# IBM/VillanDiffusion

Hardware: AMD Instinct MI355X
Metric: train imgs/sec + 1000-step DDPM sample imgs/sec, CIFAR10 bs128 (higher is better)
Workload: dtype bf16x3/f32

## Files before the change

### include/villan_hip.h

```cpp
#ifndef VILLAN_HIP_H
#define VILLAN_HIP_H

#include <stdint.h>

#ifdef __cplusplus
extern "C" {
#endif

#define VD_ABI_VERSION 12
#define VD_EINVAL (-22)
#define VD_ETIMEDOUT (-110)

int vd_abi_version(void);
const char* vd_last_error(void);
int vd_device_ok(void);
int vd_async_errors(int clear);

enum vd_a_mode { VD_A_ROW = 0,
                 VD_A_COL = 1 };
enum vd_b_mode { VD_B_PLAIN = 0,
                 VD_B_KCONTIG = 1,
                 VD_B_CONV3 = 2,
                 VD_B_CONV3_T = 3,
                 VD_B_CONV3_S2 = 4,
// ... 5 lines not shown
    const float* A;
    const float* B;
    float* D;
    const float* bias;
    const float* rowadd;
    const float* residual;
    int32_t M, N, K;
    int32_t a_mode, b_mode;
    int32_t NP;
    int32_t C, H, W;
    int32_t OH, OW;
    int32_t bias_on_n;
    int32_t d_trans;
    int32_t accumulate;
    int32_t tile;
    int32_t debug;
    float alpha;
    int64_t lda, a_bstride;
    int64_t ldb, b_bstride;
    int64_t ldd, d_bstride;
    int64_t res_bstride, rowadd_bstride;
    float* ws;
    int32_t pad;
    int32_t nb2;
    int64_t a_b2stride, b_b2stride, d_b2stride;
    const float* gn_ss;
    const void* a_packed;
    int32_t a_packed_mpad;
    int32_t math;
    int32_t pool2;
    int32_t kh, kw;
    int32_t conv_stride;
    int32_t pad_h, pad_w;
    int32_t act;
    float* gn_part;
    float* act_out;
    int64_t act_bstride;
    int32_t b_presplit;
    int32_t reserved_;
} vd_gemm_desc;

int vd_gemm(const vd_gemm_desc* desc, void* stream);
int64_t vd_gemm_ws_floats(const vd_gemm_desc* desc);
int vd_gemm_tile(const vd_gemm_desc* desc);
int vd_gemm_kernel_name(const vd_gemm_desc* desc, char* name, int name_len);

typedef struct vd_wgrad_desc {
    const float* dY;
    const float* X;
    float* dW;
    float* ws;
    int32_t M, C, T;
    int32_t nb, NP;
    int32_t H, W, OH, OW;
    int32_t mode, splits, accumulate, tile;
    int64_t dy_bstride, x_bstride;
    int32_t pad;
    int32_t math;
    int32_t presplit;
    int32_t reserved_;
} vd_wgrad_desc;

int vd_conv_wgrad(const vd_wgrad_desc* desc, void* stream);
int64_t vd_conv_wgrad_ws_floats(const vd_wgrad_desc* desc);
int vd_conv_wgrad_plan(const vd_wgrad_desc* desc, int* tile, int* splits);
int vd_conv_wgrad_kernel_name(const vd_wgrad_desc* desc, char* name, int name_len);

int vd_presplit_pack(const float* x, void* y, int B, int C, int HW, int64_t x_bstride, int64_t y_bstride, void* stream);
int vd_presplit_unpack(const void* y, float* x, int B, int C, int HW, int64_t y_bstride, int64_t x_bstride, void* stream);
int vd_groupnorm_fwd_presplit_ok(int C, int HW, int G);
int vd_groupnorm_fwd_presplit(const float* x, const float* gamma, const float* beta, void* y, float* mean, float* rstd, int B, int C, int HW, int G,
                              float eps, int apply_silu, int64_t x_bstride, int64_t y_bstride, void* stream);
int vd_groupnorm_bwd_presplit(const float* dy, const float* x, const float* mean, const float* rstd, const float* gamma, const float* beta,
                              const float* extra, const float* extra2, float* dx, void* dx_ps, float* dgamma_ws, float* dbeta_ws, float* rowsum,
                              int B, int C, int HW, int G, int apply_silu, int64_t dy_bstride, int64_t x_bstride, int64_t extra_bstride,
                              int64_t extra2_bstride, int64_t dx_bstride, int64_t ps_bstride, int64_t rowsum_ld, void* stream);

int vd_conv_wgrad_group_class(const vd_wgrad_desc* desc);
int64_t vd_conv_wgrad_group_job_bytes(void);
int vd_conv_wgrad_group_variant(int cls);
int vd_conv_wgrad_group_plan(const vd_wgrad_desc* descs, int n, void* table_out, int64_t* ws_floats, int* blocks, int* rblocks);
int vd_conv_wgrad_group_rebase(void* dev_table, int n, float* ws, void* stream);
int vd_conv_wgrad_group_launch(const void* dev_table, int n, int cls, int blocks, int rblocks, void* stream);
int vd_conv_wgrad_group_kernel_name(int cls, char* name, int name_len);

int64_t vd_conv3_packed_bytes(int M, int C, int taps);
int vd_conv3_pack_weights(const float* W, void* packed, int M, int C, int taps, int64_t row_stride, int64_t chan_stride, void* stream);
int vd_conv3_pack_weights_multi(const int64_t* table, int n_jobs, int64_t total_blocks, void* stream);
int vd_conv3_pack_weights_f16_multi(const int64_t* table, int n_jobs, int64_t total_blocks, void* stream);

int vd_weight_transpose(const float* W, float* Wt, int M, int C, int T, void* stream);
int vd_sumpool2x2(const float* dU, float* dX, int B, int C, int H, int W, int64_t du_bstride, int64_t dx_bstride,
                  int accumulate, void* stream);
int vd_col2im_s2(const float* G, float* dX, int B, int C, int H, int W, int OH, int OW, int pad, int64_t g_bstride,
                 int64_t dx_bstride, void* stream);
int vd_rowsum(const float* X, float* ws, int B, int M, int P, int64_t x_bstride, int64_t ws_ld, void* stream);
int vd_colsum(const float* ws, float* out, int B, int C, int64_t ld, int accumulate, void* stream);
int vd_colsum_segmented(const int64_t* table, int n_jobs, int B, void* stream);

int64_t vd_groupnorm_ws_floats(int B, int C, int HW, int G);
int vd_groupnorm_fwd(const float* x, const float* gamma, const float* beta, float* y, float* mean, float* rstd,
                     int B, int C, int HW, int G, float eps, int apply_silu, int64_t x_bstride, int64_t y_bstride,
                     float* ws, void* stream);
int vd_groupnorm_stats(const float* x, const float* gamma, const float* beta, float* ss, float* mean, float* rstd,
                       int B, int C, int HW, int G, float eps, int64_t x_bstride, void* stream);
int vd_groupnorm_stats_from_partials(const float* part, int tiles, const float* gamma, const float* beta, float* ss, float* mean,
                                     float* rstd, int B, int C, int HW, int G, float eps, void* stream);
int vd_groupnorm_bwd(const float* dy, const float* x, const float* mean, const float* rstd, const float* gamma,
                     const float* beta, const float* extra, float* dx, float* dgamma_ws, float* dbeta_ws,
                     int B, int C, int HW, int G, int apply_silu, int64_t dy_bstride, int64_t x_bstride,
                     int64_t extra_bstride, int64_t dx_bstride, float* ws, void* stream);
int vd_groupnorm_bwd_fused(const float* dy, const float* x, const float* mean, const float* rstd, const float* gamma,
                           const float* beta, const float* extra, const float* extra2, float* dx, float* dgamma_ws,
                           float* dbeta_ws, float* rowsum, int B, int C, int HW, int G, int apply_silu,
                           int64_t dy_bstride, int64_t x_bstride, int64_t extra_bstride, int64_t extra2_bstride,
                           int64_t dx_bstride, int64_t rowsum_ld, float* ws, void* stream);
int vd_groupnorm_plan(int which, int B, int C, int HW, int G, int aligned, int has_ws, void* stream, char* name, int name_len);

int vd_softmax_col_fwd(float* S, int nb, int N, void* stream);
int vd_softmax_col_bwd(const float* P, float* dP, int nb, int N, float scale, void* stream);
int vd_attn_small_fwd(const float* qkv, float* out, float* P, int B, int C, int N, float scale,
                      int64_t qkv_bstride, int64_t out_bstride, void* stream);
int vd_attn_small_bwd(const float* qkv, const float* P, const float* dout, float* dqkv, int B, int C, int N,
                      float scale, int64_t qkv_bstride, int64_t dout_bstride, int64_t dqkv_bstride, void* stream);

int vd_attn_core_fwd(const float* qkv, float* out, float* P, int B, int heads, int head_dim, int N, float scale, void* stream);
int vd_attn_core_bwd(const float* qkv, const float* P, const float* out, const float* dout, float* dS, float* dqkv, int B, int heads,
                     int head_dim, int N, float scale, void* stream);

int vd_attn_flash_fwd(const float* qkv, float* out, float* lse, int B, int heads, int head_dim, int N, float scale, int64_t qkv_bstride,
                      int64_t out_bstride, void* stream);
int vd_attn_flash_bwd(const float* qkv, const float* out, const float* dout, const float* lse, float* delta, float* dqkv, int B, int heads,
                      int head_dim, int N, float scale, int64_t qkv_bstride, int64_t out_bstride, int64_t dout_bstride,
                      int64_t dqkv_bstride, void* stream);

int vd_timestep_embedding(const float* t, const float* freqs, float* emb, int B, int half, int flip_sin_to_cos,
                          void* stream);
int vd_silu_fwd(const float* x, float* y, int64_t n, void* stream);
int vd_silu_bwd(const float* dy, const float* x, float* dx, int64_t n, int accumulate, void* stream);
int vd_add_strided(float* dst, const float* src, int B, int64_t inner, int64_t dst_bstride, int64_t src_bstride,
                   int accumulate, void* stream);
int vd_scale(float* x, int64_t n, float alpha, void* stream);
int vd_lincomb(float* out, const float* const* srcs, const float* coefs, int n_src, int64_t n, void* stream);

int vd_qsample_backdoor(const float* x0, const float* R, const float* eps, const int64_t* t,
                        const float* tab_a, const float* tab_s, const float* tab_step, const float* tab_coef,
                        float* x_t, float* y, int B, int64_t chw, void* stream);
int vd_mse_fwd_bwd(const float* pred, const float* y, const float* pscale, float* dpred, float* loss,
                   float* partial, int B, int64_t chw, float gscale, void* stream);
#define VD_LOSS_L2 0
#define VD_LOSS_L1 1
#define VD_LOSS_HUBER 2
int vd_loss_fwd_bwd(const float* pred, const float* y, const float* pscale, float* dpred, float* loss,
                    float* partial, int B, int64_t chw, float gscale, int kind, void* stream);
int vd_loss_sample_fwd_bwd(const float* pred, const float* y, const float* pscale, const float* weight, const float* wtab, const int64_t* t,
                           int T, const uint8_t* flags, float poison_weight, float* dpred, float* loss, float* sample_loss, float* stats,
                           float* ws, int B, int64_t chw, float gscale, int kind, void* stream);
int64_t vd_loss_sample_ws_floats(int B, int64_t chw);
int vd_loss_sample_plan(int B, int64_t chw, int* segments, int* blocks);
int vd_trigger_inv_objective(const float* e, const float* tau, float lambda, float* loss, float* dout, float* dtau, float* partial,
                             int B, int64_t chw, int64_t e_bstride, void* stream);
int vd_removal_loss(const float* pred, const float* ref, float w_clean, float w_shift, float gscale, float* dpred, float* terms,
                    float* partial, int B, int64_t chw, int64_t pred_bstride, void* stream);
int vd_image_set_stats(const float* x, int N, int C, int H, int W, int64_t x_bstride, float mul, float add, float lo, float hi,
                       float* mean_img, float* stats, float* partial, void* stream);
int vd_score_inv_objective(const float* s, const float* tau, float sigma, float lambda, float* loss, float* dout, float* dtau,
                           float* partial, int B, int64_t chw, int64_t s_bstride, void* stream);
int vd_image_set_merge(float* mean_a, float* stats_a, int64_t n_a, const float* mean_b, const float* stats_b, int64_t n_b, int64_t chw,
                       float* partial, void* stream);
int vd_neuron_scale(const float* w0, float* w, const int64_t* table, int n_jobs, int64_t total_blocks, const float* mask, const float* delta,
                    const float* xi, void* stream);
int vd_neuron_grad(const float* g, const float* w0, const int64_t* table, int n_jobs, int64_t total_blocks, float* gmask, float* gxi, float scale,
                   int accumulate, void* stream);
int vd_neuron_step(float* x, const float* g, float* buf, int64_t n, float lr, float momentum, float lo, float hi, int use_sign, void* stream);
int vd_lora_merge(const float* w0, float* w, const int64_t* table, int n_jobs, int64_t total_blocks, const float* ab, int r, float s, void* stream);
int vd_lora_grad(const float* g, const int64_t* table, int n_jobs, int64_t total_blocks, const float* ab, float* gab, int r, float s,
                 int accumulate, void* stream);
int64_t vd_lora_act_grad_ws_floats(const int64_t* host_table, int n_rows, int r);
int vd_lora_act_grad(const int64_t* host_table, const int64_t* table, int n_rows, const float* ab, float* gab, int r, float s, int accumulate,
                     float* ws, int64_t ws_floats, void* stream);

int vd_l2norm_sq(const float* g, int64_t n, float* partial, float* out_sq, void* stream);
int vd_adam_step(float* p, const float* g, float* m, float* v, int64_t n, const float* norm_sq, float max_norm,
                 float inv_scale, float lr, float beta1, float beta2, float eps, int step, unsigned* skipped, void* stream);
int vd_adam_ema_step(float* p, const float* g, float* m, float* v, float* ema, int64_t n, const float* norm_sq, float max_norm,
                     float inv_scale, float lr, float beta1, float beta2, float eps, int step, float one_minus_decay, unsigned* skipped,
                     void* stream);
int vd_swap(float* a, float* b, int64_t n, void* stream);

int vd_sched_step(const float* x, const float* eps, const float* z, float* out, float* x0_out, int64_t n,
                  float c_eps, float c_div, float clip, float c_x0, float c_x, float c_e, float c_z,
                  uint64_t seed, uint64_t offset, void* stream);
int vd_batch_l2norm(const float* x, float* out, int B, int64_t inner, void* stream);
int vd_postprocess(const float* x, float* out, int B, int C, int HW, float mul, float add, float lo, float hi,
                   int to_nhwc, void* stream);
int vd_ssim(const float* a, const float* b, const float* win, float* out, int N, int C, int H, int W, int K, float c1, float c2,
            void* stream);
int vd_vq_nearest(const float* z, const float* codebook, float* zq, int64_t* idx, int B, int D, int HW, int n_e,
                  int64_t z_bstride, int64_t q_bstride, void* stream);
int vd_fir_resample2(const float* x, float* out, int64_t planes, int H, int W, int up, float scale, int accumulate, void* stream);
int vd_pyramid_dgrad(const float* g, const float* w, const float* coarse, float* out, int B, int K, int C, int H, int W,
                     int64_t g_bstride, int accumulate, void* stream);
int vd_fourier_embedding(const float* t, const float* W, float* emb, int B, int half, void* stream);
int vd_rowscale(const float* x, const float* s, float* out, int B, int64_t inner, int divide, void* stream);
int vd_randn(float* out, int64_t n, uint64_t seed, uint64_t offset, void* stream);

int vd_poison_batch(const uint8_t* img, const int64_t* idx, const uint8_t* flags, const float* trigger, const float* target,
                    float* pixel_values, float* tgt_out, float* image_out, int B, int C, int H, int W, float vmin,
                    float vmax, int R_trigger_only, void* stream);

int vd_pool3(const float* x, float* y, int B, int C, int H, int W, int stride, int pad, int mode, int64_t x_bstride, int64_t y_bstride,
             void* stream);
int vd_resize_bilinear(const float* x, float* y, int64_t planes, int H, int W, int OH, int OW, float mul, float add, void* stream);

int vd_channel_affine(const float* x, const float* mul, const float* add, float* y, int B, int C, int HW, void* stream);
int vd_lpips_layer(const float* f0, const float* f1, const float* w, float* out, int N, int C, int HW, int accumulate, void* stream);

#ifdef __cplusplus
}
#endif
#endif
```

### villandiffusion_amd/csrc/vd_elem.hip

```cpp
#include "vd_common.h"

namespace {

constexpr int EB = 256;
inline int egrid(int64_t n, int per_thread = 1) {
    int64_t g = (n + (int64_t)EB * per_thread - 1) / ((int64_t)EB * per_thread);
    return (int)(g < 1 ? 1 : (g > 4096 ? 4096 : g));
}
#define GRID_STRIDE(i, n) \
    for (int64_t i = blockIdx.x * (int64_t)blockDim.x + threadIdx.x; i < (n); i += (int64_t)gridDim.x * blockDim.x)

__device__ __forceinline__ float mul_rn(float a, float b) { return __fmul_rn(a, b); }
__device__ __forceinline__ float add_rn(float a, float b) { return __fadd_rn(a, b); }
__device__ __forceinline__ float sub_rn(float a, float b) { return __fsub_rn(a, b); }

__global__ void temb_kernel(const float* __restrict__ t, const float* __restrict__ freqs, float* __restrict__ emb, int B,
                            int half, int flip) {
    GRID_STRIDE(i, (int64_t)B * half) {
        const int b = (int)(i / half), k = (int)(i - (int64_t)b * half);
        const float a = mul_rn(t[b], freqs[k]);
        const float sn = sinf(a), cs = cosf(a);
        float* e = emb + (int64_t)b * 2 * half;
        e[flip ? half + k : k] = sn;
        e[flip ? k : half + k] = cs;
// ... 249 lines not shown
        const uint32_t n2 = (uint32_t)(p0 >> 32) ^ c3 ^ k1, n3 = (uint32_t)p0;
        c0 = n0; c1 = n1; c2 = n2; c3 = n3;
        k0 += 0x9E3779B9u;
        k1 += 0xBB67AE85u;
    }
    out[0] = c0; out[1] = c1; out[2] = c2; out[3] = c3;
}
__device__ __forceinline__ void randn4(uint64_t seed, uint64_t ctr, float (&z)[4]) {
    uint32_t r[4];
    philox4x32_10((uint32_t)ctr, (uint32_t)(ctr >> 32), 0u, 0u, (uint32_t)seed, (uint32_t)(seed >> 32), r);
    const float k = 2.3283064365386963e-10f;
    const float u0 = ((float)r[0] + 0.5f) * k, u1 = ((float)r[1] + 0.5f) * k;
    const float u2 = ((float)r[2] + 0.5f) * k, u3 = ((float)r[3] + 0.5f) * k;
    const float ra = sqrtf(-2.f * __logf(fminf(u0, 0.99999994f) + 1e-12f)), rb = sqrtf(-2.f * __logf(fminf(u2, 0.99999994f) + 1e-12f));
    float s, c;
    __sincosf(6.283185307179586f * u1, &s, &c);
    z[0] = ra * c;
    z[1] = ra * s;
    __sincosf(6.283185307179586f * u3, &s, &c);
    z[2] = rb * c;
    z[3] = rb * s;
}

__global__ void randn_kernel(float* __restrict__ out, int64_t n, uint64_t seed, uint64_t offset) {
    GRID_STRIDE(q, (n + 3) >> 2) {
        float z[4];
        randn4(seed, offset + (uint64_t)q, z);
#pragma unroll
        for (int j = 0; j < 4; ++j)
            if (q * 4 + j < n) out[q * 4 + j] = z[j];
    }
}

struct StepCoef {
    float c_eps, c_div, clip, c_x0, c_x, c_e, c_z;
};
__global__ void sched_step_kernel(const float* __restrict__ x, const float* __restrict__ eps, const float* __restrict__ z,
                                  float* __restrict__ out, float* __restrict__ x0_out, int64_t n, StepCoef k, uint64_t seed,
                                  uint64_t offset) {
    GRID_STRIDE(q, (n + 3) >> 2) {
        float zz[4] = {0.f, 0.f, 0.f, 0.f};
        if (k.c_z != 0.f && !z) randn4(seed, offset + (uint64_t)q, zz);
#pragma unroll
        for (int j = 0; j < 4; ++j) {
            const int64_t i = q * 4 + j;
            if (i >= n) break;
            const float xv = x[i], ev = eps[i];
            float x0 = sub_rn(xv, mul_rn(k.c_eps, ev)) / k.c_div;
            if (k.clip > 0.f) x0 = fminf(fmaxf(x0, -k.clip), k.clip);
            float o = add_rn(mul_rn(k.c_x0, x0), mul_rn(k.c_x, xv));
            if (k.c_e != 0.f) o = add_rn(o, mul_rn(k.c_e, ev));
            if (k.c_z != 0.f) o = add_rn(o, mul_rn(k.c_z, z ? z[i] : zz[j]));
            out[i] = o;
            if (x0_out) x0_out[i] = x0;
        }
    }
}

__global__ __launch_bounds__(256) void batch_l2norm_kernel(const float* __restrict__ x, float* __restrict__ out, int64_t inner) {
    __shared__ float red[4];
    const float* __restrict__ xb = x + (int64_t)blockIdx.x * inner;
    float s = 0.f;
    for (int64_t i = threadIdx.x; i < inner; i += 256) s += xb[i] * xb[i];
    s = block_sum_256(s, red);
    if (threadIdx.x == 0) out[blockIdx.x] = sqrtf(s);
}

__global__ void postprocess_kernel(const float* __restrict__ x, float* __restrict__ out, int B, int C, int HW, float mul,
                                   float add, float lo, float hi, int to_nhwc) {
    GRID_STRIDE(i, (int64_t)B * C * HW) {
        const float v = fminf(fmaxf(add_rn(mul_rn(x[i], mul), add), lo), hi);
        if (to_nhwc) {
            const int p = (int)(i % HW);
            const int64_t bc = i / HW;
            const int c = (int)(bc % C);
            const int64_t b = bc / C;
            out[(b * HW + p) * C + c] = v;
        } else {
            out[i] = v;
        }
    }
}

__global__ void poison_kernel(const uint8_t* __restrict__ img, const int64_t* __restrict__ idx, const uint8_t* __restrict__ flags,
                              const float* __restrict__ trigger, const float* __restrict__ target, float* __restrict__ pv,
                              float* __restrict__ tg, float* __restrict__ image_out, int B, int C, int H, int W, float vmin,
                              float vmax, float denom, int r_trigger_only) {
    const int64_t chw = (int64_t)C * H * W;
    GRID_STRIDE(i, (int64_t)B * chw) {
        const int b = (int)(i / chw);
        const int64_t r = i - (int64_t)b * chw;
        const int xw = (int)(r % W);
        const int64_t cy = r / W;
        const int yh = (int)(cy % H), c = (int)(cy / H);
        const uint8_t f = flags[b];
        const int xs = (f & 2) ? (W - 1 - xw) : xw;
        const int64_t sb = idx ? idx[b] : (int64_t)b;
        const float u = (float)img[((sb * H + yh) * W + xs) * C + c] / 255.0f;
        const float xv = add_rn(mul_rn(sub_rn(u, 0.0f) / denom, sub_rn(vmax, vmin)), vmin);
        if (image_out) image_out[i] = xv;
        if (f & 1) {
            const float tr = trigger[r];
            pv[i] = r_trigger_only ? tr : ((tr > vmin) ? tr : xv);
            tg[i] = target[r];
        } else {
            pv[i] = 0.f;
            tg[i] = xv;
        }
    }
}

}

#define ST ((hipStream_t)stream)

extern "C" int vd_timestep_embedding(const float* t, const float* freqs, float* emb, int B, int half, int flip_sin_to_cos,
                                     void* stream) {
    VD_REQUIRE(t && freqs && emb && B > 0 && half > 0, "vd_timestep_embedding: bad args");
    hipLaunchKernelGGL(temb_kernel, dim3(egrid((int64_t)B * half)), dim3(EB), 0, ST, t, freqs, emb, B, half, flip_sin_to_cos);
    VD_LAUNCH_CHECK("vd_timestep_embedding");
    return 0;
}

extern "C" int vd_silu_fwd(const float* x, float* y, int64_t n, void* stream) {
    VD_REQUIRE(x && y && n > 0, "vd_silu_fwd: bad args");
    hipLaunchKernelGGL(silu_fwd_kernel, dim3(egrid(n)), dim3(EB), 0, ST, x, y, n);
    VD_LAUNCH_CHECK("vd_silu_fwd");
    return 0;
}

extern "C" int vd_silu_bwd(const float* dy, const float* x, float* dx, int64_t n, int accumulate, void* stream) {
    VD_REQUIRE(dy && x && dx && n > 0, "vd_silu_bwd: bad args");
    hipLaunchKernelGGL(silu_bwd_kernel, dim3(egrid(n)), dim3(EB), 0, ST, dy, x, dx, n, accumulate);
    VD_LAUNCH_CHECK("vd_silu_bwd");
    return 0;
}

extern "C" int vd_add_strided(float* dst, const float* src, int B, int64_t inner, int64_t dst_bstride, int64_t src_bstride,
                              int accumulate, void* stream) {
    VD_REQUIRE(dst && src && B > 0 && inner > 0, "vd_add_strided: bad args");
    const bool vec = ((inner & 3) == 0) && ((dst_bstride & 3) == 0) && ((src_bstride & 3) == 0) &&
                     ((((uintptr_t)dst) & 15) == 0) && ((((uintptr_t)src) & 15) == 0);
    if (vec)
        hipLaunchKernelGGL(add_strided_kernel, dim3(egrid((int64_t)B * inner / 4)), dim3(EB), 0, ST, dst, src, B, inner / 4,
                           dst_bstride, src_bstride, accumulate);
    else
        hipLaunchKernelGGL(add_strided_scalar_kernel, dim3(egrid((int64_t)B * inner)), dim3(EB), 0, ST, dst, src, B, inner,
                           dst_bstride, src_bstride, accumulate);
    VD_LAUNCH_CHECK("vd_add_strided");
    return 0;
}

extern "C" int vd_scale(float* x, int64_t n, float alpha, void* stream) {
    VD_REQUIRE(x && n > 0, "vd_scale: bad args");
    hipLaunchKernelGGL(scale_kernel, dim3(egrid(n, 4)), dim3(EB), 0, ST, x, n, alpha);
    VD_LAUNCH_CHECK("vd_scale");
    return 0;
}

extern "C" int vd_lincomb(float* out, const float* const* srcs, const float* coefs, int n_src, int64_t n, void* stream) {
    VD_REQUIRE(out && srcs && coefs && n_src >= 1 && n_src <= 6 && n > 0, "vd_lincomb: bad args (n_src=%d)", n_src);
    LinArgs a;
    for (int i = 0; i < 6; ++i) {
        a.src[i] = i < n_src ? srcs[i] : nullptr;
        a.coef[i] = i < n_src ? coefs[i] : 0.f;
    }
    a.n_src = n_src;
    for (int i = 0; i < n_src; ++i) VD_REQUIRE(a.src[i] != nullptr, "vd_lincomb: null source %d", i);
    hipLaunchKernelGGL(lincomb_kernel, dim3(egrid(n)), dim3(EB), 0, ST, out, a, n);
    VD_LAUNCH_CHECK("vd_lincomb");
    return 0;
}

extern "C" int vd_qsample_backdoor(const float* x0, const float* R, const float* eps, const int64_t* t, const float* tab_a,
                                   const float* tab_s, const float* tab_step, const float* tab_coef, float* x_t, float* y, int B,
                                   int64_t chw, void* stream) {
    VD_REQUIRE(x0 && R && eps && t && tab_s && tab_step && tab_coef && x_t && y, "vd_qsample_backdoor: null pointer");
    VD_REQUIRE(B > 0 && chw > 0, "vd_qsample_backdoor: bad dims");
    hipLaunchKernelGGL(qsample_kernel, dim3(egrid((int64_t)B * chw)), dim3(EB), 0, ST, x0, R, eps, t, tab_a, tab_s, tab_step,
                       tab_coef, x_t, y, B, chw);
    VD_LAUNCH_CHECK("vd_qsample_backdoor");
    return 0;
}

extern "C" int vd_loss_fwd_bwd(const float* pred, const float* y, const float* pscale, float* dpred, float* loss, float* partial,
                               int B, int64_t chw, float gscale, int kind, void* stream) {
    VD_REQUIRE(pred && y && loss && partial && B > 0 && chw > 0, "vd_loss_fwd_bwd: bad args");
    VD_REQUIRE(kind >= VD_LOSS_L2 && kind <= VD_LOSS_HUBER, "vd_loss_fwd_bwd: kind %d (0 = l2, 1 = l1, 2 = huber)", kind);
    const int64_t n = (int64_t)B * chw;
    int grid = egrid(n);
    if (grid > 1024) grid = 1024;
// ... 395 lines not shown
    if (q2 >= items) return;
    const int b2 = (int)(q2 / ipi), pb = (int)(q2 - (int64_t)b2 * ipi) * 4;
    float r[4];
#pragma unroll
    for (int e = 0; e < 4; ++e) r[e] = red[0][li2][c * 4 + e];
    for (int t = 1; t < PD_KS; ++t)
#pragma unroll
        for (int e = 0; e < 4; ++e) r[e] += red[t][li2][c * 4 + e];
    float* __restrict__ op = out + ((int64_t)b2 * C + c) * HW + pb;
    const int CH = H >> 1, CW = W >> 1;
    const float* __restrict__ xp = coarse ? coarse + ((int64_t)b2 * C + c) * CH * CW : nullptr;
#pragma unroll
    for (int e = 0; e < 4; ++e) {
        const int p = pb + e;
        if (p >= HW) break;
        float val = r[e];
        if (xp) {
            const int oy = p / W, ox = p - oy * W;
            const int ay = oy >> 1, ax = ox >> 1;
            const int y0 = (oy & 1) ? ay : ay - 1, y1 = (oy & 1) ? ay + 1 : ay;
            const float wy0 = (oy & 1) ? 0.75f : 0.25f, wy1 = (oy & 1) ? 0.25f : 0.75f;
            const int x0 = (ox & 1) ? ax : ax - 1, x1 = (ox & 1) ? ax + 1 : ax;
            const float wx0 = (ox & 1) ? 0.75f : 0.25f, wx1 = (ox & 1) ? 0.25f : 0.75f;
            auto at = [&](int yy, int xx) -> float {
                return ((unsigned)yy < (unsigned)CH && (unsigned)xx < (unsigned)CW) ? xp[yy * CW + xx] : 0.f;
            };
            const float u = wy0 * (wx0 * at(y0, x0) + wx1 * at(y0, x1)) + wy1 * (wx0 * at(y1, x0) + wx1 * at(y1, x1));
            val += 0.25f * u;
        }
        op[e] = accumulate ? op[e] + val : val;
    }
}

extern "C" int vd_pyramid_dgrad(const float* g, const float* w, const float* coarse, float* out, int B, int K, int C, int H, int W,
                                int64_t g_bstride, int accumulate, void* stream) {
    VD_REQUIRE(g && w && out && B > 0 && K > 0 && H > 0 && W > 0, "vd_pyramid_dgrad: bad args");
    VD_REQUIRE(C >= 1 && C <= 4, "vd_pyramid_dgrad: %d image channels not in [1, 4]", C);
    VD_REQUIRE(g_bstride >= (int64_t)K * H * W, "vd_pyramid_dgrad: batch stride %lld < K*H*W %lld", (long long)g_bstride, (long long)K * H * W);
    VD_REQUIRE(!coarse || (H % 2 == 0 && W % 2 == 0), "vd_pyramid_dgrad: a coarser level needs even dims");
    const int HW = H * W;
    const int64_t items = (int64_t)B * ((HW + 3) >> 2);
    const int64_t grid = (items + PD_IPB - 1) / PD_IPB;
    VD_REQUIRE(grid <= 0x7fffffff, "vd_pyramid_dgrad: too many pixels");
    const int vec = (HW % 4 == 0) && (g_bstride % 4 == 0) && ((((uintptr_t)g) & 15) == 0);
#define PD_LAUNCH(CC) \
    hipLaunchKernelGGL(pyramid_dgrad_kernel<CC>, dim3((unsigned)grid), dim3(256), 0, ST, g, w, coarse, out, B, K, H, W, g_bstride, accumulate, vec)
    switch (C) {
        case 1: PD_LAUNCH(1); break;
        case 2: PD_LAUNCH(2); break;
        case 3: PD_LAUNCH(3); break;
        default: PD_LAUNCH(4); break;
    }
#undef PD_LAUNCH
    VD_LAUNCH_CHECK("vd_pyramid_dgrad");
    return 0;
}

extern "C" int vd_fourier_embedding(const float* t, const float* W, float* emb, int B, int half, void* stream) {
    VD_REQUIRE(t && W && emb && B > 0 && half > 0, "vd_fourier_embedding: bad args");
    hipLaunchKernelGGL(fourier_embedding_kernel, dim3((B * half + 255) / 256), dim3(256), 0, ST, t, W, emb, B, half);
    VD_LAUNCH_CHECK("vd_fourier_embedding");
    return 0;
}

extern "C" int vd_rowscale(const float* x, const float* s, float* out, int B, int64_t inner, int divide, void* stream) {
    VD_REQUIRE(x && s && out && B > 0 && inner > 0, "vd_rowscale: bad args");
    hipLaunchKernelGGL(rowscale_kernel, dim3(egrid((int64_t)B * inner)), dim3(EB), 0, ST, x, s, out, B, inner, divide);
    VD_LAUNCH_CHECK("vd_rowscale");
    return 0;
}

extern "C" int vd_poison_batch(const uint8_t* img, const int64_t* idx, const uint8_t* flags, const float* trigger, const float* target,
                               float* pixel_values, float* tgt_out, float* image_out, int B, int C, int H, int W, float vmin,
                               float vmax, int R_trigger_only, void* stream) {
    VD_REQUIRE(img && flags && trigger && target && pixel_values && tgt_out, "vd_poison_batch: null pointer");
    VD_REQUIRE(B > 0 && C > 0 && H > 0 && W > 0, "vd_poison_batch: bad dims");
    const float denom = (float)(1.0 - 0.0 + 1e-5);
    hipLaunchKernelGGL(poison_kernel, dim3(egrid((int64_t)B * C * H * W)), dim3(EB), 0, ST, img, idx, flags, trigger, target,
                       pixel_values, tgt_out, image_out, B, C, H, W, vmin, vmax, denom, R_trigger_only);
    VD_LAUNCH_CHECK("vd_poison_batch");
    return 0;
}

namespace {

template <int MODE>
__global__ __launch_bounds__(EB) void pool3_kernel(const float* __restrict__ x, float* __restrict__ y, int B, int C, int H, int W, int OH, int OW,
                                                   int stride, int pad, int64_t x_bstride, int64_t y_bstride) {
    const int64_t total = (int64_t)B * C * OH * OW;
    for (int64_t e = (int64_t)blockIdx.x * EB + threadIdx.x; e < total; e += (int64_t)gridDim.x * EB) {
        const int ox = (int)(e % OW);
        int64_t r = e / OW;
        const int oy = (int)(r % OH);
        r /= OH;
        const int c = (int)(r % C), b = (int)(r / C);
        const float* __restrict__ src = x + b * x_bstride + (int64_t)c * H * W;
        float acc = MODE == 0 ? -INFINITY : 0.f;
        int cnt = 0;
#pragma unroll
        for (int dy = 0; dy < 3; ++dy)
#pragma unroll
            for (int dx = 0; dx < 3; ++dx) {
                const int iy = oy * stride + dy - pad, ix = ox * stride + dx - pad;
                const bool ok = (unsigned)iy < (unsigned)H && (unsigned)ix < (unsigned)W;
                const float v = src[ok ? iy * W + ix : 0];
                if (ok) {
                    acc = MODE == 0 ? fmaxf(acc, v) : acc + v;
                    ++cnt;
                }
            }
        y[b * y_bstride + (int64_t)c * OH * OW + (int64_t)oy * OW + ox] = MODE == 0 ? acc : acc / (float)cnt;
    }
}

__global__ __launch_bounds__(EB) void resize_bilinear_kernel(const float* __restrict__ x, float* __restrict__ y, int64_t planes, int H, int W, int OH,
                                                             int OW, float sh, float sw, float mul, float add) {
    const int64_t total = planes * OH * OW;
    for (int64_t e = (int64_t)blockIdx.x * EB + threadIdx.x; e < total; e += (int64_t)gridDim.x * EB) {
        const int ox = (int)(e % OW);
        const int64_t r = e / OW;
        const int oy = (int)(r % OH);
        const int64_t pl = r / OH;
        float fy = sh * ((float)oy + 0.5f) - 0.5f, fx = sw * ((float)ox + 0.5f) - 0.5f;
        fy = fy < 0.f ? 0.f : fy;
        fx = fx < 0.f ? 0.f : fx;
        const int y0 = (int)fy, x0 = (int)fx;
        const int y1 = y0 + (y0 < H - 1 ? 1 : 0), x1 = x0 + (x0 < W - 1 ? 1 : 0);
        const float ly = fy - (float)y0, lx = fx - (float)x0;
        const float* __restrict__ s = x + pl * H * W;
        const float v = (1.f - ly) * ((1.f - lx) * s[y0 * W + x0] + lx * s[y0 * W + x1]) + ly * ((1.f - lx) * s[y1 * W + x0] + lx * s[y1 * W + x1]);
        y[e] = mul * v + add;
    }
}

}

extern "C" int vd_pool3(const float* x, float* y, int B, int C, int H, int W, int stride, int pad, int mode, int64_t x_bstride, int64_t y_bstride,
                        void* stream) {
    VD_REQUIRE(x && y && B > 0 && C > 0 && H >= 3 - 2 * pad && W >= 3 - 2 * pad && (stride == 1 || stride == 2) && (pad == 0 || pad == 1) && (mode == 0 || mode == 1),
               "vd_pool3: bad args (3x3 window, stride 1 | 2, pad 0 | 1, mode 0 max | 1 avg without the padding)");
    const int OH = (H + 2 * pad - 3) / stride + 1, OW = (W + 2 * pad - 3) / stride + 1;
    const int64_t n = (int64_t)B * C * OH * OW;
    if (mode == 0)
        hipLaunchKernelGGL(pool3_kernel<0>, dim3(egrid(n)), dim3(EB), 0, ST, x, y, B, C, H, W, OH, OW, stride, pad, x_bstride, y_bstride);
    else
        hipLaunchKernelGGL(pool3_kernel<1>, dim3(egrid(n)), dim3(EB), 0, ST, x, y, B, C, H, W, OH, OW, stride, pad, x_bstride, y_bstride);
    VD_LAUNCH_CHECK("vd_pool3");
    return 0;
}

extern "C" int vd_resize_bilinear(const float* x, float* y, int64_t planes, int H, int W, int OH, int OW, float mul, float add, void* stream) {
    VD_REQUIRE(x && y && planes > 0 && H > 0 && W > 0 && OH > 0 && OW > 0, "vd_resize_bilinear: bad args");
    hipLaunchKernelGGL(resize_bilinear_kernel, dim3(egrid(planes * OH * OW)), dim3(EB), 0, ST, x, y, planes, H, W, OH, OW, (float)H / (float)OH,
                       (float)W / (float)OW, mul, add);
    VD_LAUNCH_CHECK("vd_resize_bilinear");
    return 0;
}

namespace {

__global__ __launch_bounds__(EB) void channel_affine_kernel(const float* __restrict__ x, const float* __restrict__ mul, const float* __restrict__ add,
                                                            float* __restrict__ y, int64_t total, int C, int HW) {
    for (int64_t e = (int64_t)blockIdx.x * EB + threadIdx.x; e < total; e += (int64_t)gridDim.x * EB) {
        const int c = (int)((e / HW) % C);
        y[e] = x[e] * mul[c] + add[c];
    }
// ... 50 lines not shown
```

### villandiffusion_amd/csrc/vd_gemm.hip

```cpp
#include "vd_common.h"
#include <string.h>
#include <stdlib.h>

bool vd_conv3_k32p_eligible(const vd_gemm_desc& d);
int vd_launch_conv3_k32p(const vd_gemm_desc& d, int mode, hipStream_t st, char* name);
int vd_launch_wgrad_ps_group(const void* jobs, int n, int W, int up, int blocks, hipStream_t st, bool one, char* name);
bool vd_conv3_sm_eligible(const vd_gemm_desc& d);
int vd_launch_conv3_sm(const vd_gemm_desc& d, hipStream_t st, char* name);
bool vd_gemm1x1_k32p_pick(const vd_gemm_desc& d);
int vd_launch_gemm1x1_k32p(const vd_gemm_desc& d, hipStream_t st, char* name);

namespace {

constexpr int NT = 256;
constexpr int BK = 32;
constexpr int KG = BK / 4;

struct Pix {
    int b, oy, ox, p;
    bool valid;
};

__device__ __forceinline__ void kdecomp9(int k, int& c, int& r, int& s) {
    c = k / 9;
// ... 1614 lines not shown

static void wgrad_patch_plan(const vd_wgrad_desc& d, int& splits, int& ks_per) {
    const int kpix = wgrad_patch_kind(d) == 3 ? 64 : 32;
    const int ks_total = (int)(((int64_t)d.nb * d.NP + kpix - 1) / kpix);
    const int base = vd_cdiv(d.M, 128) * vd_cdiv(d.C, 64) * 3;
    splits = d.splits;
    if (splits <= 0) {
        constexpr int target = 768;
        splits = vd_cdiv(target, base);
        const int max_splits = ks_total / 8 > 0 ? ks_total / 8 : 1;
        if (splits > max_splits) splits = max_splits;
        if (splits < 1) splits = 1;
    }
    ks_per = vd_cdiv(ks_total, splits);
    splits = vd_cdiv(ks_total, ks_per);
}

__global__ __launch_bounds__(256) void slab_reduce_kernel(const float* __restrict__ ws, float* __restrict__ out,
                                                          int64_t n4, int splits, int accumulate) {
    const f32x4* __restrict__ w4 = reinterpret_cast<const f32x4*>(ws);
    f32x4* __restrict__ o4 = reinterpret_cast<f32x4*>(out);
    for (int64_t i = blockIdx.x * (int64_t)blockDim.x + threadIdx.x; i < n4; i += (int64_t)gridDim.x * blockDim.x) {
        f32x4 s = w4[i];
        for (int z = 1; z < splits; ++z) s += w4[(int64_t)z * n4 + i];
        if (accumulate) s += o4[i];
        o4[i] = s;
    }
}
__global__ __launch_bounds__(256) void slab_reduce_perm_kernel(const float* __restrict__ ws, float* __restrict__ out, int M,
                                                               int C, int splits, int accumulate) {
    const int64_t n = (int64_t)M * C * 9;
    for (int64_t i = blockIdx.x * (int64_t)blockDim.x + threadIdx.x; i < n; i += (int64_t)gridDim.x * blockDim.x) {
        float s = ws[i];
        for (int z = 1; z < splits; ++z) s += ws[(int64_t)z * n + i];
        const int sx = (int)(i % 3);
        const int64_t t = i / 3;
        const int c = (int)(t % C);
        const int64_t t2 = t / C;
        const int m = (int)(t2 % M), r = (int)(t2 / M);
        const int64_t o = ((int64_t)m * C + c) * 9 + r * 3 + sx;
        out[o] = accumulate ? (out[o] + s) : s;
    }
}

__global__ __launch_bounds__(256) void slab_reduce_scalar_kernel(const float* __restrict__ ws, float* __restrict__ out,
                                                                 int64_t n, int splits, int accumulate) {
    for (int64_t i = blockIdx.x * (int64_t)blockDim.x + threadIdx.x; i < n; i += (int64_t)gridDim.x * blockDim.x) {
        float s = ws[i];
        for (int z = 1; z < splits; ++z) s += ws[(int64_t)z * n + i];
        if (accumulate) s += out[i];
        out[i] = s;
    }
}

__global__ __launch_bounds__(256) void wtranspose_kernel(const float* __restrict__ W, float* __restrict__ Wt, int M, int C,
                                                         int T) {
    const int64_t total = (int64_t)M * C * T;
    for (int64_t i = blockIdx.x * (int64_t)blockDim.x + threadIdx.x; i < total; i += (int64_t)gridDim.x * blockDim.x) {
        const int t = (int)(i % T);
        const int64_t cm = i / T;
        const int m = (int)(cm % M), c = (int)(cm / M);
        Wt[i] = W[((int64_t)m * C + c) * T + t];
    }
}

__global__ __launch_bounds__(256) void sumpool2x2_kernel(const float* __restrict__ dU, float* __restrict__ dX, int B, int C,
                                                         int H, int W, int64_t du_bs, int64_t dx_bs, int accumulate) {
    const int64_t per = (int64_t)C * H * W, total = per * B;
    for (int64_t i = blockIdx.x * (int64_t)blockDim.x + threadIdx.x; i < total; i += (int64_t)gridDim.x * blockDim.x) {
        const int b = (int)(i / per);
        const int64_t r = i - (int64_t)b * per;
        const int x = (int)(r % W);
        const int64_t cy = r / W;
        const int y = (int)(cy % H);
        const int64_t c = cy / H;
        const float* u = dU + (int64_t)b * du_bs + (c * 2 * H + 2 * y) * (2 * W) + 2 * x;
        float s = (u[0] + u[1]) + (u[2 * W] + u[2 * W + 1]);
        float* o = dX + (int64_t)b * dx_bs + r;
        *o = accumulate ? (*o + s) : s;
    }
}

__global__ __launch_bounds__(256) void col2im_s2_kernel(const float* __restrict__ G, float* __restrict__ dX, int B, int C,
                                                        int H, int W, int OH, int OW, int pad, int64_t g_bs, int64_t dx_bs) {
    const int64_t per = (int64_t)C * H * W, total = per * B;
    for (int64_t i = blockIdx.x * (int64_t)blockDim.x + threadIdx.x; i < total; i += (int64_t)gridDim.x * blockDim.x) {
        const int b = (int)(i / per);
        const int64_t q = i - (int64_t)b * per;
        const int x = (int)(q % W);
        const int64_t cy = q / W;
        const int y = (int)(cy % H);
        const int c = (int)(cy / H);
        const float* g = G + (int64_t)b * g_bs + (int64_t)c * 9 * OH * OW;
        const int yp = y + pad, xp = x + pad;
        float acc = 0.f;
        for (int r = yp & 1; r < 3; r += 2) {
            const int iy = (yp - r) >> 1;
            if (yp < r || iy >= OH) continue;
            for (int s = xp & 1; s < 3; s += 2) {
                const int ix = (xp - s) >> 1;
                if (xp < s || ix >= OW) continue;
                acc += g[(r * 3 + s) * OH * OW + iy * OW + ix];
            }
        }
        dX[(int64_t)b * dx_bs + q] = acc;
    }
}

__global__ __launch_bounds__(256) void rowsum_long_kernel(const float* __restrict__ X, float* __restrict__ ws, int M, int P, int64_t x_bs, int64_t ws_ld) {
    __shared__ float part[4];
    const int row = blockIdx.x, b = row / M, m = row - b * M;
    const int lane = threadIdx.x & 63, w = threadIdx.x >> 6;
    const int Q = P >> 4;
    const f32x4* __restrict__ x4 = reinterpret_cast<const f32x4*>(X + (int64_t)b * x_bs + (int64_t)m * P) + (int64_t)w * Q;
    float s0 = 0.f, s1 = 0.f, s2 = 0.f, s3 = 0.f;
    int i = lane;
    for (; i + 192 < Q; i += 256) {
        const f32x4 a = x4[i], c = x4[i + 64], e = x4[i + 128], f = x4[i + 192];
        s0 += (a[0] + a[1]) + (a[2] + a[3]);
        s1 += (c[0] + c[1]) + (c[2] + c[3]);
        s2 += (e[0] + e[1]) + (e[2] + e[3]);
        s3 += (f[0] + f[1]) + (f[2] + f[3]);
    }
    for (; i < Q; i += 64) {
        const f32x4 a = x4[i];
        s0 += (a[0] + a[1]) + (a[2] + a[3]);
    }
    const float s = wave_sum((s0 + s1) + (s2 + s3));
    if (lane == 0) part[w] = s;
    __syncthreads();
    if (threadIdx.x == 0) ws[(int64_t)b * ws_ld + m] = (part[0] + part[1]) + (part[2] + part[3]);
}

__global__ __launch_bounds__(256) void rowsum_kernel(const float* __restrict__ X, float* __restrict__ ws, int B, int M, int P,
                                                     int64_t x_bs, int64_t ws_ld) {
    const int row = blockIdx.x * 4 + (threadIdx.x >> 6);
    if (row >= B * M) return;
    const int b = row / M, m = row - b * M;
    const float* __restrict__ x = X + (int64_t)b * x_bs + (int64_t)m * P;
    const int lane = threadIdx.x & 63;
    float s = 0.f;
    if ((P & 3) == 0 && ((((uintptr_t)x) & 15) == 0)) {
        const f32x4* x4 = reinterpret_cast<const f32x4*>(x);
        const int Q = P >> 2;
        int i = lane;
        for (; i + 192 < Q; i += 256) {
            const f32x4 v0 = x4[i], v1 = x4[i + 64], v2 = x4[i + 128], v3 = x4[i + 192];
            s += (v0[0] + v0[1]) + (v0[2] + v0[3]);
            s += (v1[0] + v1[1]) + (v1[2] + v1[3]);
            s += (v2[0] + v2[1]) + (v2[2] + v2[3]);
            s += (v3[0] + v3[1]) + (v3[2] + v3[3]);
        }
        for (; i < Q; i += 64) {
            f32x4 v = x4[i];
            s += (v[0] + v[1]) + (v[2] + v[3]);
        }
    } else {
        for (int i = lane; i < P; i += 64) s += x[i];
    }
    s = wave_sum(s);
    if (lane == 0) ws[(int64_t)b * ws_ld + m] = s;
}

__global__ __launch_bounds__(256) void colsum_kernel(const float* __restrict__ ws, float* __restrict__ out, int B, int C,
                                                     int64_t ld, int accumulate) {
    __shared__ float part[4][64];
    const int lane = threadIdx.x & 63, w = threadIdx.x >> 6;
    const int c = blockIdx.x * 64 + lane;
    float s = 0.f;
    if (c < C) {
        int b = w;
        for (; b + 28 < B; b += 32) {
            float t[8];
#pragma unroll
            for (int u = 0; u < 8; ++u) t[u] = ws[(int64_t)(b + 4 * u) * ld + c];
#pragma unroll
            for (int u = 0; u < 8; ++u) s += t[u];
        }
        for (; b < B; b += 4) s += ws[(int64_t)b * ld + c];
    }
    part[w][lane] = s;
    __syncthreads();
    if (w == 0 && c < C) {
        const float t = (part[0][lane] + part[1][lane]) + (part[2][lane] + part[3][lane]);
        out[c] = accumulate ? (out[c] + t) : t;
    }
}

template <bool BIG_IS_X>
__global__ __launch_bounds__(256) void wgrad_small_kernel(const vd_wgrad_desc d) {
    constexpr int MAXS = 4, PWM = 34;
    __shared__ float S[MAXS * PWM * PWM];
    const int CB = BIG_IS_X ? d.C : d.M, CS = BIG_IS_X ? d.M : d.C;
    const int H = d.OH, W = d.OW, HW = H * W;
    constexpr int PW = PWM, PHW = PWM * PWM;
    const int cb_blocks = (CB + 31) / 32, tiles_x = (W + 31) / 32, tiles = tiles_x * ((H + 31) / 32);
    int rest = blockIdx.x;
    const int cb0 = (rest % cb_blocks) * 32;
    rest /= cb_blocks;
    const int tile = rest % tiles, b = rest / tiles;
    const int y0 = (tile / tiles_x) * 32, x0 = (tile - (tile / tiles_x) * tiles_x) * 32;
    const int TH = min(32, H - y0), TW = min(32, W - x0);
    const float* __restrict__ big = (BIG_IS_X ? d.X + (int64_t)b * d.x_bstride : d.dY + (int64_t)b * d.dy_bstride);
    const float* __restrict__ sml = (BIG_IS_X ? d.dY + (int64_t)b * d.dy_bstride : d.X + (int64_t)b * d.x_bstride);
    for (int i = threadIdx.x; i < CS * PHW; i += 256) {
        const int cs = i / PHW, rem = i - cs * PHW;
        const int yy = y0 + rem / PW - 1, xx = x0 + rem - (rem / PW) * PW - 1;
        const bool ok = (unsigned)yy < (unsigned)H && (unsigned)xx < (unsigned)W;
        S[i] = ok ? sml[(int64_t)cs * HW + yy * W + xx] : 0.f;
    }
    __syncthreads();
    const int x = threadIdx.x & 31, slot = threadIdx.x >> 5;
    const int Ncols = d.C * 9;
    float* __restrict__ part = d.ws + ((int64_t)b * tiles + tile) * d.M * Ncols;
    float acc[4][MAXS][9];
#pragma unroll
    for (int k = 0; k < 4; ++k)
#pragma unroll
        for (int cs = 0; cs < MAXS; ++cs)
#pragma unroll
            for (int t = 0; t < 9; ++t) acc[k][cs][t] = 0.f;
    if (x < TW) {
        const float* __restrict__ src[4];
        bool live[4];
#pragma unroll
        for (int k = 0; k < 4; ++k) {
            const int cb = cb0 + slot + 8 * k;
            live[k] = cb < CB;
            src[k] = big + (int64_t)(live[k] ? cb : 0) * HW + (int64_t)y0 * W + x0 + x;
        }
        for (int y = 0; y < TH; ++y) {
            float v[4];
#pragma unroll
            for (int k = 0; k < 4; ++k) v[k] = src[k][y * W];
#pragma unroll
            for (int k = 0; k < 4; ++k) v[k] = live[k] ? v[k] : 0.f;
#pragma unroll
            for (int cs = 0; cs < MAXS; ++cs) {
                if (cs < CS) {
                    const float* __restrict__ sp = S + cs * PHW + (y + 1) * PW + (x + 1);
#pragma unroll
                    for (int t = 0; t < 9; ++t) {
                        const int r = t / 3, sx = t - 3 * r;
                        const int dy = BIG_IS_X ? 1 - r : r - 1, dx = BIG_IS_X ? 1 - sx : sx - 1;
// ... 551 lines not shown
        jb.d.ws = reinterpret_cast<float*>((uintptr_t)0);
        if (splits > 1) {
            jb.rblocks = (int)((nel + 255) / 256 < 1024 ? (nel + 255) / 256 : 1024);
            jb.d.ws = reinterpret_cast<float*>((uintptr_t)(off * sizeof(float)));
            off += (int64_t)splits * nel;
            off = (off + 3) / 4 * 4;
        }
        rblk += jb.rblocks;
    }
    *ws_floats = off;
    *blocks = blk;
    *rblocks = rblk;
    return cls;
}

__global__ __launch_bounds__(64) void wgrad_group_rebase_kernel(vd_wgrad_job* __restrict__ jobs, int n, float* ws) {
    const int j = blockIdx.x * 64 + threadIdx.x;
    if (j < n && jobs[j].gy > 1) jobs[j].d.ws = ws + ((uintptr_t)jobs[j].d.ws) / sizeof(float);
}

extern "C" int vd_conv_wgrad_group_rebase(void* dev_table, int n, float* ws, void* stream) {
    VD_REQUIRE(dev_table && n > 0, "vd_conv_wgrad_group_rebase: bad args");
    hipLaunchKernelGGL(wgrad_group_rebase_kernel, dim3(vd_cdiv(n, 64)), dim3(64), 0, (hipStream_t)stream,
                       reinterpret_cast<vd_wgrad_job*>(dev_table), n, ws);
    VD_LAUNCH_CHECK("vd_conv_wgrad_group_rebase");
    return 0;
}

static int wgrad_group_run(const void* dev_table, int n, int cls, int blocks, int rblocks, hipStream_t st, char* name) {
    VD_REQUIRE(name || (dev_table && n > 0 && blocks > 0 && rblocks >= 0), "vd_conv_wgrad_group_launch: bad args");
    const vd_wgrad_job* jobs = reinterpret_cast<const vd_wgrad_job*>(dev_table);
    const dim3 grid(blocks);
    switch (cls) {
        case VD_WG_ONE + 1000: {
            if (!name) {
                static const hipError_t attr1 = hipFuncSetAttribute(reinterpret_cast<const void*>(wgrad1x1_wide_group_kernel<true>),
                                                                    hipFuncAttributeMaxDynamicSharedMemorySize, W1X1_WIDE_LDS);
                VD_REQUIRE(attr1 == hipSuccess, "vd_conv_wgrad_group_launch: cannot reserve %d bytes of LDS", W1X1_WIDE_LDS);
            }
            VD_LAUNCH_OR_NAME(name, wgrad1x1_wide_group_kernel<true>, grid, dim3(512), W1X1_WIDE_LDS, st, jobs, n);
            break;
        }
        case VD_WG_ONE + 4 * 32 + 0: VD_LAUNCH_OR_NAME(name, (wgrad_k32_group_kernel<32, 0, true>), grid, dim3(NT), 0, st, jobs, n); break;
        case VD_WG_ONE + 4 * 32 + 2: VD_LAUNCH_OR_NAME(name, (wgrad_k32_group_kernel<32, 2, true>), grid, dim3(NT), 0, st, jobs, n); break;
        case VD_WG_ONE + 4 * 16 + 0: VD_LAUNCH_OR_NAME(name, (wgrad_k32_group_kernel<16, 0, true>), grid, dim3(NT), 0, st, jobs, n); break;
        case VD_WG_ONE + 4 * 16 + 2: VD_LAUNCH_OR_NAME(name, (wgrad_k32_group_kernel<16, 2, true>), grid, dim3(NT), 0, st, jobs, n); break;
        case VD_WG_ONE + 4 * 8 + 0: VD_LAUNCH_OR_NAME(name, (wgrad_k32_group_kernel<8, 0, true>), grid, dim3(NT), 0, st, jobs, n); break;
        case VD_WG_ONE + 4 * 8 + 2: VD_LAUNCH_OR_NAME(name, (wgrad_k32_group_kernel<8, 2, true>), grid, dim3(NT), 0, st, jobs, n); break;
        case VD_WG_ONE + 3000 + 4 * 32: case VD_WG_ONE + 3000 + 4 * 16: case VD_WG_ONE + 3000 + 4 * 8: case VD_WG_ONE + 3000 + 4 * 32 + 2:
        case VD_WG_ONE + 3000 + 4 * 16 + 2: case VD_WG_ONE + 3000 + 4 * 8 + 2:
            VD_REQUIRE(vd_launch_wgrad_ps_group(dev_table, n, (cls - VD_WG_ONE - 3000) / 4, (cls - VD_WG_ONE - 3000) & 2, blocks, st, true, name) == 0,
                       "vd_conv_wgrad_group_launch: no pre-split kernel for class %d", cls);
            break;
        case 1000: {
            if (!name) {
                static const hipError_t attr = hipFuncSetAttribute(reinterpret_cast<const void*>(wgrad1x1_wide_group_kernel<>),
                                                                   hipFuncAttributeMaxDynamicSharedMemorySize, W1X1_WIDE_LDS);
                VD_REQUIRE(attr == hipSuccess, "vd_conv_wgrad_group_launch: cannot reserve %d bytes of LDS", W1X1_WIDE_LDS);
            }
            VD_LAUNCH_OR_NAME(name, wgrad1x1_wide_group_kernel<>, grid, dim3(512), W1X1_WIDE_LDS, st, jobs, n);
            break;
        }
        case 4 * 32 + 0: VD_LAUNCH_OR_NAME(name, (wgrad_k32_group_kernel<32, 0>), grid, dim3(NT), 0, st, jobs, n); break;
        case 4 * 32 + 2: VD_LAUNCH_OR_NAME(name, (wgrad_k32_group_kernel<32, 2>), grid, dim3(NT), 0, st, jobs, n); break;
        case 4 * 32 + 1: VD_LAUNCH_OR_NAME(name, (wgrad_bx3_group_kernel<32, 0, true>), grid, dim3(NT), 0, st, jobs, n); break;
        case 4 * 32 + 3: VD_LAUNCH_OR_NAME(name, (wgrad_bx3_group_kernel<32, 2, true>), grid, dim3(NT), 0, st, jobs, n); break;
        case 4 * 16 + 0: VD_LAUNCH_OR_NAME(name, (wgrad_k32_group_kernel<16, 0>), grid, dim3(NT), 0, st, jobs, n); break;
        case 4 * 16 + 2: VD_LAUNCH_OR_NAME(name, (wgrad_k32_group_kernel<16, 2>), grid, dim3(NT), 0, st, jobs, n); break;
        case 4 * 8 + 0: VD_LAUNCH_OR_NAME(name, (wgrad_k32_group_kernel<8, 0>), grid, dim3(NT), 0, st, jobs, n); break;
        case 4 * 8 + 2: VD_LAUNCH_OR_NAME(name, (wgrad_k32_group_kernel<8, 2>), grid, dim3(NT), 0, st, jobs, n); break;
        case 4 * 4 + 0: VD_LAUNCH_OR_NAME(name, (wgrad_bx3_group_kernel<4, 0, false>), grid, dim3(NT), 0, st, jobs, n); break;
        case 3000 + 4 * 32: case 3000 + 4 * 16: case 3000 + 4 * 8: case 3000 + 4 * 32 + 2: case 3000 + 4 * 16 + 2: case 3000 + 4 * 8 + 2:
            VD_REQUIRE(vd_launch_wgrad_ps_group(dev_table, n, (cls - 3000) / 4, (cls - 3000) & 2, blocks, st, false, name) == 0,
                       "vd_conv_wgrad_group_launch: no pre-split kernel for class %d", cls);
            break;
        case 2000 + 33: VD_LAUNCH_OR_NAME(name, (wgrad_bx3_group_kernel<32, 4, true>), grid, dim3(NT), 0, st, jobs, n); break;
        case 2000 + 32: VD_LAUNCH_OR_NAME(name, (wgrad_bx3_group_kernel<32, 4, false>), grid, dim3(NT), 0, st, jobs, n); break;
        case 2000 + 16: VD_LAUNCH_OR_NAME(name, (wgrad_bx3_group_kernel<16, 4, false>), grid, dim3(NT), 0, st, jobs, n); break;
        case 2000 + 8: VD_LAUNCH_OR_NAME(name, (wgrad_bx3_group_kernel<8, 4, false>), grid, dim3(NT), 0, st, jobs, n); break;
        default: vd_set_error("vd_conv_wgrad_group_launch: unknown kernel class %d", cls); return VD_EINVAL;
    }
    if (name) return vd_name_append(name, "(+group_reduce)");
    VD_LAUNCH_CHECK("vd_conv_wgrad_group_launch");
    if (rblocks > 0) {
        hipLaunchKernelGGL(wgrad_group_reduce_kernel, dim3(rblocks), dim3(256), 0, st, jobs, n);
        VD_LAUNCH_CHECK("vd_conv_wgrad_group_launch/reduce");
    }
    return 0;
}

extern "C" int vd_conv_wgrad_group_launch(const void* dev_table, int n, int cls, int blocks, int rblocks, void* stream) {
    return wgrad_group_run(dev_table, n, cls, blocks, rblocks, (hipStream_t)stream, nullptr);
}

extern "C" int vd_conv_wgrad_group_kernel_name(int cls, char* name, int name_len) {
    char buf[VD_NAME_LEN] = "";
    return name_out(wgrad_group_run(nullptr, 0, cls, 0, 0, nullptr, buf), buf, name, name_len);
}

extern "C" int64_t vd_conv_wgrad_ws_floats(const vd_wgrad_desc* desc) {
    if (!desc) return 0;
    int tile, splits, kk_per;
    wgrad_plan(*desc, tile, splits, kk_per);
    return splits > 1 ? (int64_t)splits * desc->M * desc->C * desc->T : 0;
}

extern "C" int vd_weight_transpose(const float* W, float* Wt, int M, int C, int T, void* stream) {
    VD_REQUIRE(W && Wt && M > 0 && C > 0 && T > 0, "vd_weight_transpose: bad args");
    const int64_t total = (int64_t)M * C * T;
    const int grid = (int)((total + 255) / 256 < 4096 ? (total + 255) / 256 : 4096);
    hipLaunchKernelGGL(wtranspose_kernel, dim3(grid), dim3(256), 0, (hipStream_t)stream, W, Wt, M, C, T);
    VD_LAUNCH_CHECK("vd_weight_transpose");
    return 0;
}

extern "C" int vd_sumpool2x2(const float* dU, float* dX, int B, int C, int H, int W, int64_t du_bstride, int64_t dx_bstride,
                             int accumulate, void* stream) {
    VD_REQUIRE(dU && dX && B > 0 && C > 0 && H > 0 && W > 0, "vd_sumpool2x2: bad args");
    const int64_t total = (int64_t)B * C * H * W;
    const int grid = (int)((total + 255) / 256 < 8192 ? (total + 255) / 256 : 8192);
    hipLaunchKernelGGL(sumpool2x2_kernel, dim3(grid), dim3(256), 0, (hipStream_t)stream, dU, dX, B, C, H, W, du_bstride,
                       dx_bstride, accumulate);
    VD_LAUNCH_CHECK("vd_sumpool2x2");
    return 0;
}

extern "C" int vd_col2im_s2(const float* G, float* dX, int B, int C, int H, int W, int OH, int OW, int pad, int64_t g_bstride,
                            int64_t dx_bstride, void* stream) {
    VD_REQUIRE(G && dX && B > 0 && C > 0 && H > 0 && W > 0 && OH > 0 && OW > 0 && (pad == 0 || pad == 1), "vd_col2im_s2: bad args");
    const int64_t total = (int64_t)B * C * H * W;
    const int grid = (int)((total + 255) / 256 < 16384 ? (total + 255) / 256 : 16384);
    hipLaunchKernelGGL(col2im_s2_kernel, dim3(grid), dim3(256), 0, (hipStream_t)stream, G, dX, B, C, H, W, OH, OW, pad, g_bstride,
                       dx_bstride);
    VD_LAUNCH_CHECK("vd_col2im_s2");
    return 0;
}

extern "C" int vd_rowsum(const float* X, float* ws, int B, int M, int P, int64_t x_bstride, int64_t ws_ld, void* stream) {
    VD_REQUIRE(X && ws && B > 0 && M > 0 && P > 0 && ws_ld >= M, "vd_rowsum: bad args");
    if (P >= 8192 && (P & 15) == 0 && (x_bstride & 3) == 0 && ((((uintptr_t)X) & 15) == 0))
        hipLaunchKernelGGL(rowsum_long_kernel, dim3(B * M), dim3(256), 0, (hipStream_t)stream, X, ws, M, P, x_bstride, ws_ld);
    else
        hipLaunchKernelGGL(rowsum_kernel, dim3(vd_cdiv((int64_t)B * M, 4)), dim3(256), 0, (hipStream_t)stream, X, ws, B, M, P,
                           x_bstride, ws_ld);
    VD_LAUNCH_CHECK("vd_rowsum");
    return 0;
}

extern "C" int vd_colsum_segmented(const int64_t* table, int n_jobs, int B, void* stream) {
    VD_REQUIRE(table && n_jobs > 0 && B > 0, "vd_colsum_segmented: bad args");
    hipLaunchKernelGGL(colsum_seg_kernel, dim3(n_jobs), dim3(256), 0, (hipStream_t)stream, table, B);
    VD_LAUNCH_CHECK("vd_colsum_segmented");
    return 0;
}

extern "C" int vd_colsum(const float* ws, float* out, int B, int C, int64_t ld, int accumulate, void* stream) {
    VD_REQUIRE(ws && out && B > 0 && C > 0, "vd_colsum: bad args");
    hipLaunchKernelGGL(colsum_kernel, dim3(vd_cdiv(C, 64)), dim3(256), 0, (hipStream_t)stream, ws, out, B, C, ld, accumulate);
    VD_LAUNCH_CHECK("vd_colsum");
    return 0;
}
```

### villandiffusion_amd/csrc/vd_wgrad_bx3.inc

```
typedef __bf16 bf16x2 __attribute__((ext_vector_type(2)));

__device__ __forceinline__ void split_pair(float a, float b, unsigned& hi, unsigned& lo) {
    bf16x2 h, l;
    h[0] = (__bf16)a;
    h[1] = (__bf16)b;
    l[0] = (__bf16)(a - (float)h[0]);
    l[1] = (__bf16)(b - (float)h[1]);
    hi = __builtin_bit_cast(unsigned, h);
    lo = __builtin_bit_cast(unsigned, l);
}

#include "vd_wgrad_job.h"

#ifdef VD_WG_STAMPS
__device__ unsigned long long* g_wg_stamps = nullptr;
#define WG_STAMP(var) const unsigned long long var = __builtin_amdgcn_s_memtime()
#endif

template <int W, int MODE, bool WIDE = false>
__device__ __forceinline__ void wgrad_bx3_body(const vd_wgrad_desc& d, int ksteps_per_split, int gx, int gy, int lin) {
    constexpr int ROWS = 32 / W;
    constexpr int OPR = W >= 8 ? W / 8 : 1;
    constexpr bool W4 = (W == 4);
    constexpr int CT = 64;
// ... 341 lines not shown
                va[j] = aok ? ra[2 * i][j] : 0.f;
                va[4 + j] = aok ? ra[2 * i + 1][j] : 0.f;
                vb[j] = bok ? rb[2 * i][j] : 0.f;
                vb[4 + j] = bok ? rb[2 * i + 1][j] : 0.f;
            }
            u32x4 hi, lo;
            split_bf16x8(va, hi, lo);
            As[so * LD_ + sr + 32 * i] = hi;
            As[(8 + so) * LD_ + sr + 32 * i] = lo;
            split_bf16x8(vb, hi, lo);
            Bs[so * LD_ + sr + 32 * i] = hi;
            Bs[(8 + so) * LD_ + sr + 32 * i] = lo;
        }
    };

    f32x16 acc[2][2];
#pragma unroll
    for (int mi = 0; mi < 2; ++mi)
#pragma unroll
        for (int ni = 0; ni < 2; ++ni)
#pragma unroll
            for (int v = 0; v < 16; ++v) acc[mi][ni][v] = 0.f;

    const int wm = wave >> 1, wc = wave & 1;
    const u32x4* __restrict__ a_base = As + h * LD_ + wm * 64 + l31;
    const u32x4* __restrict__ b_base = Bs + h * LD_ + wc * 64 + l31;

    if (ks_begin < ks_end) {
        load_stage(ks_begin);
        store_stage();
        __syncthreads();
        for (int ks = ks_begin; ks < ks_end; ++ks) {
            const bool more = ks + 1 < ks_end;
            if (more) load_stage(ks + 1);
#pragma unroll
            for (int kk = 0; kk < 4; ++kk) {
                bf16x8 ah[2], al[2];
#pragma unroll
                for (int mi = 0; mi < 2; ++mi) {
                    ah[mi] = __builtin_bit_cast(bf16x8, a_base[(2 * kk) * LD_ + mi * 32]);
                    al[mi] = __builtin_bit_cast(bf16x8, a_base[(8 + 2 * kk) * LD_ + mi * 32]);
                }
#pragma unroll
                for (int ni = 0; ni < 2; ++ni) {
                    const bf16x8 bh = __builtin_bit_cast(bf16x8, b_base[(2 * kk) * LD_ + ni * 32]);
                    const bf16x8 bl = __builtin_bit_cast(bf16x8, b_base[(8 + 2 * kk) * LD_ + ni * 32]);
#pragma unroll
                    for (int mi = 0; mi < 2; ++mi) {
                        acc[mi][ni] = __builtin_amdgcn_mfma_f32_32x32x16_bf16(al[mi], bh, acc[mi][ni], 0, 0, 0);
                        acc[mi][ni] = __builtin_amdgcn_mfma_f32_32x32x16_bf16(ah[mi], bl, acc[mi][ni], 0, 0, 0);
                        acc[mi][ni] = __builtin_amdgcn_mfma_f32_32x32x16_bf16(ah[mi], bh, acc[mi][ni], 0, 0, 0);
                    }
                }
            }
            __syncthreads();
            if (more) store_stage();
            __syncthreads();
        }
    }
    float* __restrict__ out = (gy > 1) ? (d.ws + (int64_t)by * d.M * d.C) : d.dW;
    const bool accum = (gy == 1) && d.accumulate;
#pragma unroll
    for (int ni = 0; ni < 2; ++ni) {
        const int c = c0 + wc * 64 + ni * 32 + l31;
        if (c >= d.C) continue;
#pragma unroll
        for (int mi = 0; mi < 2; ++mi)
#pragma unroll
            for (int v = 0; v < 16; ++v) {
                const int m = m0 + wm * 64 + mi * 32 + (v & 3) + 8 * (v >> 2) + 4 * h;
                if (m >= d.M) continue;
                const int64_t off = (int64_t)m * d.C + c;
                out[off] = accum ? (out[off] + acc[mi][ni][v]) : acc[mi][ni][v];
            }
    }
}

__global__ __launch_bounds__(NT, 2) void wgrad1x1_bx3_kernel(const vd_wgrad_desc d, int ksteps_per_split) {
    wgrad1x1_bx3_body(d, ksteps_per_split, gridDim.x, gridDim.y, blockIdx.x + gridDim.x * blockIdx.y);
}

#include "vd_wgrad1x1_wide.inc"

__global__ __launch_bounds__(256) void wgrad_group_reduce_kernel(const vd_wgrad_job* __restrict__ jobs, int n_jobs) {
    const vd_wgrad_job* __restrict__ jb = jobs + wgrad_find_job(jobs, n_jobs, blockIdx.x, true);
    const int lb = blockIdx.x - jb->first_rblock;
    if (lb >= jb->rblocks || jb->gy <= 1) return;
    const int M = jb->d.M, C = jb->d.C, T = jb->d.T, splits = jb->gy, accumulate = jb->d.accumulate;
    const float* __restrict__ ws = jb->d.ws;
    float* __restrict__ out = jb->d.dW;
    const int64_t n = (int64_t)M * C * T;
    if ((n & 3) == 0 && ((((uintptr_t)ws) & 15) == 0)) {
        const int64_t n4 = n >> 2;
        const f32x4* __restrict__ ws4 = reinterpret_cast<const f32x4*>(ws);
        for (int64_t i4 = lb * 256 + threadIdx.x; i4 < n4; i4 += (int64_t)jb->rblocks * 256) {
            const f32x4* __restrict__ p = ws4 + i4;
            f32x4 s = p[0];
            int z = 1;
            for (; z + 4 <= splits; z += 4) {
                const f32x4 a = p[(int64_t)z * n4], b = p[(int64_t)(z + 1) * n4], c = p[(int64_t)(z + 2) * n4], e = p[(int64_t)(z + 3) * n4];
#pragma unroll
                for (int j = 0; j < 4; ++j) s[j] = (((s[j] + a[j]) + b[j]) + c[j]) + e[j];
            }
            for (; z < splits; ++z) {
                const f32x4 a = p[(int64_t)z * n4];
#pragma unroll
                for (int j = 0; j < 4; ++j) s[j] += a[j];
            }
#pragma unroll
            for (int j = 0; j < 4; ++j) {
                const int64_t i = 4 * i4 + j;
                int64_t o = i;
                if (T == 9) {
                    const int sx = (int)(i % 3);
                    const int64_t t = i / 3;
                    const int c = (int)(t % C);
                    const int64_t t2 = t / C;
                    const int m = (int)(t2 % M), r = (int)(t2 / M);
                    o = ((int64_t)m * C + c) * 9 + r * 3 + sx;
                }
                out[o] = accumulate ? (out[o] + s[j]) : s[j];
            }
        }
        return;
    }
    for (int64_t i = lb * 256 + threadIdx.x; i < n; i += (int64_t)jb->rblocks * 256) {
        float s = ws[i];
        for (int z = 1; z < splits; ++z) s += ws[(int64_t)z * n + i];
        int64_t o = i;
        if (T == 9) {
            const int sx = (int)(i % 3);
            const int64_t t = i / 3;
            const int c = (int)(t % C);
            const int64_t t2 = t / C;
            const int m = (int)(t2 % M), r = (int)(t2 / M);
            o = ((int64_t)m * C + c) * 9 + r * 3 + sx;
        }
        out[o] = accumulate ? (out[o] + s) : s;
    }
}

static bool wgrad1x1_bx3_eligible(const vd_wgrad_desc& d) {
    return d.math == 1 && d.T == 1 && d.mode == VD_B_PLAIN && d.NP % 8 == 0 && d.M >= 64 && d.C >= 64 && d.tile == 0 &&
           (d.x_bstride & 3) == 0 && (d.dy_bstride & 3) == 0 && ((((uintptr_t)d.X) | ((uintptr_t)d.dY)) & 15) == 0;
}

static void wgrad1x1_bx3_plan(const vd_wgrad_desc& d, int& splits, int& ks_per) {
    const int ks_total = (int)(((int64_t)d.nb * (d.NP >> 3) + 7) >> 3);
    const int base = vd_cdiv(d.M, 128) * vd_cdiv(d.C, 128);
    splits = d.splits;
    if (splits <= 0) {
        constexpr int target = 256;
        splits = vd_cdiv(target, base);
        const int max_splits = ks_total / 4 > 0 ? ks_total / 4 : 1;
        if (splits > max_splits) splits = max_splits;
        if (splits < 1) splits = 1;
    }
    ks_per = vd_cdiv(ks_total, splits);
    splits = vd_cdiv(ks_total, ks_per);
}
```

### villandiffusion_amd/dataset.py

```python
from __future__ import annotations

import os
import pickle
from typing import Dict, Iterator, List, Optional, Tuple, Union

import numpy as np
import torch

from . import ops

DEFAULT_VMIN, DEFAULT_VMAX = float(-1.0), float(1.0)
_ASSET_ROOT = os.path.dirname(os.path.dirname(os.path.abspath(__file__)))


def normalize(x, vmin_in=None, vmax_in=None, vmin_out=0, vmax_out=1, eps: float = 1e-5):
    if vmax_out is None and vmin_out is None:
        return x
    lo = x.min() if vmin_in is None else vmin_in
    hi = x.max() if vmax_in is None else vmax_in
    if vmax_out is None:
        vmax_out = hi
    if vmin_out is None:
        vmin_out = lo
    return ((x - lo) / (hi - lo + eps)) * (vmax_out - vmin_out) + vmin_out
# ... 473 lines not shown

    def get_mask(self, trigger: torch.Tensor) -> torch.Tensor:
        return torch.where(trigger > self._vmin, 0, 1)

    def get_poisoned(self, imgs: torch.Tensor) -> torch.Tensor:
        trig = self._trigger.to(imgs.device)
        m = self.get_mask(trig)
        return m * imgs + (1 - m) * trig

    def get_inpainted_by_type(self, imgs: torch.Tensor, inpaint_type: str) -> torch.Tensor:
        half = imgs.shape[-1] // 2
        mask = torch.ones_like(imgs[0])
        if inpaint_type == self.INPAINT_LINE:
            mask[..., 0:2 * half, half - half // 10: half + half // 20] = 0
        elif inpaint_type == self.INPAINT_BOX:
            lo, hi = half - half // 3, half + half // 3
            mask[..., lo:hi, lo:hi] = 0
        else:
            raise NotImplementedError(f"inpaint: {inpaint_type} is not implemented")
        return mask * imgs + (1 - mask) * torch.full_like(imgs, float(imgs.min()))

    def _ensure_device(self):
        if self._dev_images is None:
            self._dev_images = torch.from_numpy(self._images).to(self._dev)
            self._dev_trigger = self._trigger.to(self._dev).contiguous()
            self._dev_target = self._target.to(self._dev).contiguous()
            self._dev_index = torch.from_numpy(np.ascontiguousarray(self._index, dtype=np.int64)).to(self._dev)
            self._dev_flags = torch.from_numpy(np.ascontiguousarray(self._flags, dtype=np.uint8)).to(self._dev)
            self._any_rto = bool((self._flags & 4).any())
            self._flip_gen = torch.Generator(device=self._dev).manual_seed(int(self._seed) + 7919) if self._dev.type == "cuda" else None

    def loader_state(self) -> Dict:
        g = getattr(self, "_flip_gen", None)
        return {"flip_gen": None if g is None else g.get_state().cpu()}

    def load_loader_state(self, st: Optional[Dict]):
        if not st or st.get("flip_gen") is None or self._latent is not None:
            return
        self._ensure_device()
        if self._flip_gen is not None:
            self._flip_gen.set_state(st["flip_gen"].cpu())

    def _h2d(self, t: torch.Tensor) -> torch.Tensor:
        if self._dev.type == "cuda" and os.environ.get("VILLAN_PAGEABLE_H2D", "0") != "1":
            return t.contiguous().pin_memory().to(self._dev, non_blocking=True)
        return t.to(self._dev)

    def make_batch(self, sample_ids: torch.Tensor, flip_bits: Optional[torch.Tensor] = None, full: bool = True) -> Dict[str, torch.Tensor]:
        if self._latent is not None:
            return self._make_latent_batch(sample_ids, full)
        self._ensure_device()
        if sample_ids.device.type == "cuda" and not full and not self._any_rto:
            return self._make_batch_resident(sample_ids, flip_bits)
        pos = sample_ids.cpu().numpy()
        ds_idx = self._h2d(torch.from_numpy(self._index[pos]))
        flags = torch.from_numpy(self._flags[pos].copy())
        B = len(pos)
        if flip_bits is None:
            flip_bits = (torch.rand(B) < 0.5) if self.random_flip else torch.zeros(B, dtype=torch.bool)
        rto = bool((flags & 4).any())
        if rto and not bool(((flags & 1) == 0).logical_or((flags & 4) != 0).all()):
            raise NotImplementedError("mixed R_trigger_only flags inside one batch")
        kflags = self._h2d(((flags & 1) | (flip_bits.to(torch.uint8) << 1)).to(torch.uint8))
        C, S = self._channel, self._image_size
        pv, tg, im = (torch.empty((B, C, S, S), device=self._dev, dtype=torch.float32) for _ in range(3))
        ops.poison_batch(self._dev_images, kflags, self._dev_trigger, self._dev_target, pv, tg, im, self._vmin, self._vmax,
                         R_trigger_only=rto, idx=ds_idx.contiguous())
        batch = {self.PIXEL_VALUES: pv, self.TARGET: tg, self.IMAGE: im}
        if full:
            is_p = self._h2d((flags & 1).bool())
            trig = self._dev_trigger[None].expand(B, C, S, S)
            batch[self.TRIGGER] = trig
            batch[self.PIXEL_VALUES_TRIGGER] = torch.where(is_p[:, None, None, None], trig, torch.zeros((), device=self._dev))
            lab = torch.full((B,), -1.0) if self._labels is None else torch.from_numpy(self._labels[self._index[pos]]).float()
            batch[self.LABEL] = self._h2d(lab)
            batch[self.IS_CLEAN] = ~is_p
        elif self.batch_flags:
            batch[self.IS_CLEAN] = ~self._h2d((flags & 1).bool())
        return batch

    def _make_batch_resident(self, pos: torch.Tensor, flip_bits: Optional[torch.Tensor]) -> Dict[str, torch.Tensor]:
        B = len(pos)
        pos = pos.long()
        ds_idx = self._dev_index.index_select(0, pos)
        fl = self._dev_flags.index_select(0, pos)
        if flip_bits is None:
            flip = (torch.rand(B, device=self._dev, generator=self._flip_gen) < 0.5) if self.random_flip else None
        else:
            flip = flip_bits if flip_bits.device.type == "cuda" else self._h2d(flip_bits)
        kflags = fl & 1
        if flip is not None:
            kflags = kflags | (flip.to(torch.uint8) << 1)
        C, S = self._channel, self._image_size
        pv, tg, im = (torch.empty((B, C, S, S), device=self._dev, dtype=torch.float32) for _ in range(3))
        ops.poison_batch(self._dev_images, kflags.contiguous(), self._dev_trigger, self._dev_target, pv, tg, im, self._vmin, self._vmax,
                         R_trigger_only=False, idx=ds_idx)
        batch = {self.PIXEL_VALUES: pv, self.TARGET: tg, self.IMAGE: im}
        if self.batch_flags:
            batch[self.IS_CLEAN] = (fl & 1) == 0
        return batch

    def get_dataloader(self, batch_size: int = None, shuffle: bool = None, num_workers: int = None, collate_fn=None,
                       rank: int = 0, world: int = 1, epoch: int = 0, full: bool = True):
        bs = batch_size or self._batch_size
        shuffle = self._shuffle if shuffle is None else shuffle
        return _Loader(self, bs, shuffle, rank, world, epoch, full)

    def get_dataset(self):
        return self


class _Loader:
    def __init__(self, dsl: DatasetLoader, bs: int, shuffle: bool, rank: int, world: int, epoch: int, full: bool):
        from .trainer import shard_indices
        self.dsl, self.bs, self.full = dsl, bs, full
        self.ids = shard_indices(len(dsl), epoch, rank, world, seed=dsl._seed, shuffle=shuffle)
        self._ids_dev = self.ids.to(dsl._dev) if (not full and dsl._latent is None and dsl._dev.type == "cuda") else None

    def __len__(self):
        return (len(self.ids) + self.bs - 1) // self.bs

    def __iter__(self) -> Iterator[Dict[str, torch.Tensor]]:
        ids = self.ids if self._ids_dev is None else self._ids_dev
        for s in range(0, len(ids), self.bs):
            yield self.dsl.make_batch(ids[s:s + self.bs], full=self.full)


class LatentDataset(torch.utils.data.Dataset):
    DATA_EXT: str = ".pt"
    TARGET_LATENTS_FILE_NAME: str = "target"
    POISON_LATENTS_FILE_NAME: str = "poison"
    RAW_LATENTS_FILE_NAME: str = "raw"

    def __init__(self, ds_root: str):
        os.makedirs(ds_root, exist_ok=True)
        self._root = ds_root
        self._target = self._poison = self._raw = None
        self._target_name = self._poison_name = self._raw_name = None
        self._poison_rate, self._len, self._vae, self._use_latent = None, None, None, True

    def set_vae(self, vae):
        self._vae = vae
        return self

    @staticmethod
    def add_ext(p: str) -> str:
        return f"{p}.{LatentDataset.DATA_EXT}"

    @staticmethod
    def read_ext(file: str):
        try:
            return torch.load(LatentDataset.add_ext(file))
        except (FileNotFoundError, OSError):
            return None

    @staticmethod
    def save_ext(val, file: str) -> None:
        torch.save(val, LatentDataset.add_ext(file))

    @property
    def targe_latents_path(self) -> str:
        p = os.path.join(self._root, LatentDataset.TARGET_LATENTS_FILE_NAME)
        if not os.path.exists(LatentDataset.add_ext(p)):
            LatentDataset.save_ext({}, p)
        return p

    def _dir(self, data_type: str) -> str:
        p = os.path.join(self._root, data_type)
        os.makedirs(p, exist_ok=True)
        return p

    def _encode(self, x: torch.Tensor) -> torch.Tensor:
        if self._vae is None:
            raise ValueError("Please provide encoder first")
        with torch.no_grad():
            return self._vae.encode(x.to(self._vae.device)).latents.detach().cpu()
# ... 74 lines not shown
```

### villandiffusion_amd/lib.py

```python
from __future__ import annotations

import ctypes as C
import os
import subprocess
from typing import Optional

_HERE = os.path.dirname(os.path.abspath(__file__))
LIB_PATH = os.path.join(_HERE, "libvillan_hip.so")
CSRC = os.path.join(_HERE, "csrc")

A_ROW, A_COL = 0, 1
B_PLAIN, B_KCONTIG, B_CONV3, B_CONV3_T, B_CONV3_S2, B_CONV3_UP, B_CONV3_DIL, B_CONVG = range(8)

_i32, _i64, _f32, _vp = C.c_int32, C.c_int64, C.c_float, C.c_void_p


class GemmDesc(C.Structure):
    _fields_ = [("A", _vp), ("B", _vp), ("D", _vp), ("bias", _vp), ("rowadd", _vp), ("residual", _vp),
                ("M", _i32), ("N", _i32), ("K", _i32), ("a_mode", _i32), ("b_mode", _i32), ("NP", _i32),
                ("C", _i32), ("H", _i32), ("W", _i32), ("OH", _i32), ("OW", _i32),
                ("bias_on_n", _i32), ("d_trans", _i32), ("accumulate", _i32), ("tile", _i32), ("debug", _i32), ("alpha", _f32),
                ("lda", _i64), ("a_bstride", _i64), ("ldb", _i64), ("b_bstride", _i64),
                ("ldd", _i64), ("d_bstride", _i64), ("res_bstride", _i64), ("rowadd_bstride", _i64), ("ws", _vp), ("pad", _i32), ("nb2", _i32),
                ("a_b2stride", _i64), ("b_b2stride", _i64), ("d_b2stride", _i64), ("gn_ss", _vp), ("a_packed", _vp), ("a_packed_mpad", _i32), ("math", _i32), ("pool2", _i32),
                ("kh", _i32), ("kw", _i32), ("conv_stride", _i32), ("pad_h", _i32), ("pad_w", _i32), ("act", _i32),
                ("gn_part", _vp), ("act_out", _vp), ("act_bstride", _i64), ("b_presplit", _i32), ("reserved_", _i32)]


class WgradDesc(C.Structure):
    _fields_ = [("dY", _vp), ("X", _vp), ("dW", _vp), ("ws", _vp),
                ("M", _i32), ("C", _i32), ("T", _i32), ("nb", _i32), ("NP", _i32),
                ("H", _i32), ("W", _i32), ("OH", _i32), ("OW", _i32),
                ("mode", _i32), ("splits", _i32), ("accumulate", _i32), ("tile", _i32),
                ("dy_bstride", _i64), ("x_bstride", _i64), ("pad", _i32), ("math", _i32), ("presplit", _i32), ("reserved_", _i32)]


PROTOTYPES = {
    "vd_abi_version": (_i32, []),
    "vd_last_error": (C.c_char_p, []),
    "vd_async_errors": (_i32, [_i32]),
    "vd_device_ok": (_i32, []),
    "vd_gemm": (_i32, [C.POINTER(GemmDesc), _vp]),
    "vd_gemm_tile": (_i32, [C.POINTER(GemmDesc)]),
    "vd_gemm_ws_floats": (_i64, [C.POINTER(GemmDesc)]),
    "vd_gemm_kernel_name": (_i32, [C.POINTER(GemmDesc), C.c_char_p, _i32]),
    "vd_conv_wgrad": (_i32, [C.POINTER(WgradDesc), _vp]),
    "vd_conv_wgrad_plan": (_i32, [C.POINTER(WgradDesc), C.POINTER(_i32), C.POINTER(_i32)]),
    "vd_conv_wgrad_ws_floats": (_i64, [C.POINTER(WgradDesc)]),
    "vd_conv_wgrad_kernel_name": (_i32, [C.POINTER(WgradDesc), C.c_char_p, _i32]),
    "vd_presplit_pack": (_i32, [_vp, _vp, _i32, _i32, _i32, _i64, _i64, _vp]),
    "vd_presplit_unpack": (_i32, [_vp, _vp, _i32, _i32, _i32, _i64, _i64, _vp]),
    "vd_groupnorm_fwd_presplit_ok": (_i32, [_i32, _i32, _i32]),
    "vd_groupnorm_fwd_presplit": (_i32, [_vp, _vp, _vp, _vp, _vp, _vp, _i32, _i32, _i32, _i32, _f32, _i32, _i64, _i64, _vp]),
    "vd_groupnorm_bwd_presplit": (_i32, [_vp] * 12 + [_vp, _i32, _i32, _i32, _i32, _i32] + [_i64] * 7 + [_vp]),
    "vd_conv_wgrad_group_class": (_i32, [C.POINTER(WgradDesc)]),
    "vd_conv_wgrad_group_job_bytes": (_i64, []),
    "vd_conv_wgrad_group_variant": (_i32, [_i32]),
    "vd_conv_wgrad_group_kernel_name": (_i32, [_i32, C.c_char_p, _i32]),
    "vd_conv_wgrad_group_plan": (_i32, [C.POINTER(WgradDesc), _i32, _vp, C.POINTER(_i64), C.POINTER(_i32), C.POINTER(_i32)]),
    "vd_conv_wgrad_group_rebase": (_i32, [_vp, _i32, _vp, _vp]),
    "vd_conv_wgrad_group_launch": (_i32, [_vp, _i32, _i32, _i32, _i32, _vp]),
    "vd_conv3_packed_bytes": (_i64, [_i32, _i32, _i32]),
    "vd_conv3_pack_weights": (_i32, [_vp, _vp, _i32, _i32, _i32, _i64, _i64, _vp]),
    "vd_conv3_pack_weights_multi": (_i32, [_vp, _i32, _i64, _vp]),
    "vd_conv3_pack_weights_f16_multi": (_i32, [_vp, _i32, _i64, _vp]),
    "vd_weight_transpose": (_i32, [_vp, _vp, _i32, _i32, _i32, _vp]),
    "vd_sumpool2x2": (_i32, [_vp, _vp, _i32, _i32, _i32, _i32, _i64, _i64, _i32, _vp]),
    "vd_col2im_s2": (_i32, [_vp, _vp, _i32, _i32, _i32, _i32, _i32, _i32, _i32, _i64, _i64, _vp]),
    "vd_rowsum": (_i32, [_vp, _vp, _i32, _i32, _i32, _i64, _i64, _vp]),
    "vd_colsum": (_i32, [_vp, _vp, _i32, _i32, _i64, _i32, _vp]),
    "vd_colsum_segmented": (_i32, [_vp, _i32, _i32, _vp]),
    "vd_groupnorm_ws_floats": (_i64, [_i32, _i32, _i32, _i32]),
    "vd_groupnorm_stats": (_i32, [_vp, _vp, _vp, _vp, _vp, _vp, _i32, _i32, _i32, _i32, _f32, _i64, _vp]),
    "vd_groupnorm_fwd": (_i32, [_vp, _vp, _vp, _vp, _vp, _vp, _i32, _i32, _i32, _i32, _f32, _i32, _i64, _i64, _vp, _vp]),
    "vd_groupnorm_bwd": (_i32, [_vp] * 10 + [_i32] * 5 + [_i64] * 4 + [_vp, _vp]),
    "vd_groupnorm_stats_from_partials": (_i32, [_vp, _i32, _vp, _vp, _vp, _vp, _vp, _i32, _i32, _i32, _i32, _f32, _vp]),
    "vd_groupnorm_bwd_fused": (_i32, [_vp] * 12 + [_i32] * 5 + [_i64] * 6 + [_vp, _vp]),
    "vd_groupnorm_plan": (_i32, [_i32] * 7 + [_vp, C.c_char_p, _i32]),
    "vd_softmax_col_fwd": (_i32, [_vp, _i32, _i32, _vp]),
    "vd_softmax_col_bwd": (_i32, [_vp, _vp, _i32, _i32, _f32, _vp]),
    "vd_attn_small_fwd": (_i32, [_vp, _vp, _vp, _i32, _i32, _i32, _f32, _i64, _i64, _vp]),
    "vd_attn_small_bwd": (_i32, [_vp, _vp, _vp, _vp, _i32, _i32, _i32, _f32, _i64, _i64, _i64, _vp]),
    "vd_attn_core_fwd": (_i32, [_vp, _vp, _vp, _i32, _i32, _i32, _i32, _f32, _vp]),
    "vd_attn_core_bwd": (_i32, [_vp, _vp, _vp, _vp, _vp, _vp, _i32, _i32, _i32, _i32, _f32, _vp]),
    "vd_attn_flash_fwd": (_i32, [_vp, _vp, _vp, _i32, _i32, _i32, _i32, _f32, _i64, _i64, _vp]),
    "vd_attn_flash_bwd": (_i32, [_vp, _vp, _vp, _vp, _vp, _vp, _i32, _i32, _i32, _i32, _f32, _i64, _i64, _i64, _i64, _vp]),
    "vd_timestep_embedding": (_i32, [_vp, _vp, _vp, _i32, _i32, _i32, _vp]),
    "vd_silu_fwd": (_i32, [_vp, _vp, _i64, _vp]),
    "vd_silu_bwd": (_i32, [_vp, _vp, _vp, _i64, _i32, _vp]),
    "vd_add_strided": (_i32, [_vp, _vp, _i32, _i64, _i64, _i64, _i32, _vp]),
    "vd_scale": (_i32, [_vp, _i64, _f32, _vp]),
    "vd_lincomb": (_i32, [_vp, C.POINTER(_vp), C.POINTER(_f32), _i32, _i64, _vp]),
    "vd_qsample_backdoor": (_i32, [_vp] * 10 + [_i32, _i64, _vp]),
    "vd_mse_fwd_bwd": (_i32, [_vp] * 6 + [_i32, _i64, _f32, _vp]),
    "vd_loss_fwd_bwd": (_i32, [_vp] * 6 + [_i32, _i64, _f32, _i32, _vp]),
    "vd_loss_sample_fwd_bwd": (_i32, [_vp] * 6 + [_i32, _vp, _f32] + [_vp] * 5 + [_i32, _i64, _f32, _i32, _vp]),
    "vd_loss_sample_ws_floats": (_i64, [_i32, _i64]),
    "vd_loss_sample_plan": (_i32, [_i32, _i64, C.POINTER(_i32), C.POINTER(_i32)]),
    "vd_trigger_inv_objective": (_i32, [_vp, _vp, _f32, _vp, _vp, _vp, _vp, _i32, _i64, _i64, _vp]),
    "vd_removal_loss": (_i32, [_vp, _vp, _f32, _f32, _f32, _vp, _vp, _vp, _i32, _i64, _i64, _vp]),
    "vd_score_inv_objective": (_i32, [_vp, _vp, _f32, _f32, _vp, _vp, _vp, _vp, _i32, _i64, _i64, _vp]),
    "vd_image_set_stats": (_i32, [_vp, _i32, _i32, _i32, _i32, _i64, _f32, _f32, _f32, _f32, _vp, _vp, _vp, _vp]),
    "vd_image_set_merge": (_i32, [_vp, _vp, _i64, _vp, _vp, _i64, _i64, _vp, _vp]),
    "vd_neuron_scale": (_i32, [_vp, _vp, _vp, _i32, _i64, _vp, _vp, _vp, _vp]),
    "vd_neuron_grad": (_i32, [_vp, _vp, _vp, _i32, _i64, _vp, _vp, _f32, _i32, _vp]),
    "vd_neuron_step": (_i32, [_vp, _vp, _vp, _i64, _f32, _f32, _f32, _f32, _i32, _vp]),
    "vd_lora_merge": (_i32, [_vp, _vp, _vp, _i32, _i64, _vp, _i32, _f32, _vp]),
    "vd_lora_grad": (_i32, [_vp, _vp, _i32, _i64, _vp, _vp, _i32, _f32, _i32, _vp]),
    "vd_lora_act_grad_ws_floats": (_i64, [_vp, _i32, _i32]),
    "vd_lora_act_grad": (_i32, [_vp, _vp, _i32, _vp, _vp, _i32, _f32, _i32, _vp, _i64, _vp]),
    "vd_l2norm_sq": (_i32, [_vp, _i64, _vp, _vp, _vp]),
    "vd_adam_step": (_i32, [_vp, _vp, _vp, _vp, _i64, _vp, _f32, _f32, _f32, _f32, _f32, _f32, _i32, _vp, _vp]),
    "vd_adam_ema_step": (_i32, [_vp, _vp, _vp, _vp, _vp, _i64, _vp, _f32, _f32, _f32, _f32, _f32, _f32, _i32, _f32, _vp, _vp]),
    "vd_swap": (_i32, [_vp, _vp, _i64, _vp]),
    "vd_sched_step": (_i32, [_vp] * 5 + [_i64] + [_f32] * 7 + [C.c_uint64, C.c_uint64, _vp]),
    "vd_batch_l2norm": (_i32, [_vp, _vp, _i32, _i64, _vp]),
    "vd_postprocess": (_i32, [_vp, _vp, _i32, _i32, _i32, _f32, _f32, _f32, _f32, _i32, _vp]),
    "vd_ssim": (_i32, [_vp, _vp, _vp, _vp, _i32, _i32, _i32, _i32, _i32, _f32, _f32, _vp]),
    "vd_randn": (_i32, [_vp, _i64, C.c_uint64, C.c_uint64, _vp]),
    "vd_fir_resample2": (_i32, [_vp, _vp, _i64, _i32, _i32, _i32, _f32, _i32, _vp]),
    "vd_pyramid_dgrad": (_i32, [_vp, _vp, _vp, _vp, _i32, _i32, _i32, _i32, _i32, _i64, _i32, _vp]),
    "vd_fourier_embedding": (_i32, [_vp, _vp, _vp, _i32, _i32, _vp]),
    "vd_rowscale": (_i32, [_vp, _vp, _vp, _i32, _i64, _i32, _vp]),
    "vd_vq_nearest": (_i32, [_vp, _vp, _vp, _vp, _i32, _i32, _i32, _i32, _i64, _i64, _vp]),
    "vd_poison_batch": (_i32, [_vp] * 8 + [_i32] * 4 + [_f32, _f32, _i32, _vp]),
    "vd_pool3": (_i32, [_vp, _vp, _i32, _i32, _i32, _i32, _i32, _i32, _i32, _i64, _i64, _vp]),
    "vd_resize_bilinear": (_i32, [_vp, _vp, _i64, _i32, _i32, _i32, _i32, _f32, _f32, _vp]),
    "vd_channel_affine": (_i32, [_vp, _vp, _vp, _vp, _i32, _i32, _i32, _vp]),
    "vd_lpips_layer": (_i32, [_vp, _vp, _vp, _vp, _i32, _i32, _i32, _i32, _vp]),
}

_lib: Optional[C.CDLL] = None


class VillanHipError(RuntimeError):
    pass


def build(verbose: bool = False) -> str:
    out = subprocess.run(["make", "-C", CSRC, "-j4"], capture_output=True, text=True)
    if verbose or out.returncode != 0:
        print(out.stdout[-4000:], out.stderr[-4000:])
    if out.returncode != 0:
        raise VillanHipError("building libvillan_hip.so failed (see output above)")
    return LIB_PATH


def load() -> C.CDLL:
    global _lib
    if _lib is not None:
        return _lib
    import torch
    if not os.path.exists(LIB_PATH):
        raise VillanHipError(
            f"{LIB_PATH} not found: the HIP extension is required (no CPU fallback exists). "
            f"Build it with `make -C {CSRC}` or `python -c 'import __graft_entry__ as g; g.build()'`.")
    lib = C.CDLL(LIB_PATH)
    for name, (res, args) in PROTOTYPES.items():
        fn = getattr(lib, name)
        fn.restype, fn.argtypes = res, args
    if lib.vd_abi_version() != 12:
        raise VillanHipError("libvillan_hip.so ABI version mismatch")
    _lib = lib
    return lib


def last_error() -> str:
    return load().vd_last_error().decode("utf-8", "replace")


_SYNC_DEBUG = bool(os.environ.get("VD_SYNC_DEBUG"))


def check(rc: int, what: str) -> None:
    if rc != 0:
        raise VillanHipError(f"{what} failed (rc={rc}): {last_error()}")
    if _SYNC_DEBUG:
        import sys
        import torch
        print(f"[vd] {what}", file=sys.stderr, flush=True)
        torch.cuda.synchronize()


_device_checked = False


def require_device() -> None:
    global _device_checked
    if _device_checked:
        return
    lib = load()
    rc = lib.vd_device_ok()
    if rc != 0:
        raise VillanHipError(f"MI355X (gfx950) device required: {last_error()}")
    _device_checked = True
```

### villandiffusion_amd/ops.py

```python
from __future__ import annotations

import ctypes as C
import functools
import math
import os
from typing import Optional, Sequence

import torch

from . import lib as L
from .lib import (A_COL, A_ROW, B_CONV3, B_CONV3_DIL, B_CONVG, B_CONV3_S2, B_CONV3_T, B_CONV3_UP, B_KCONTIG, B_PLAIN,
                  GemmDesc, WgradDesc)


def _lib():
    L.require_device()
    return L.load()


_PROF = None


def _kernel_name(query, what) -> str:
    buf = C.create_string_buffer(128)
# ... 575 lines not shown
    if ent is None or ws is None or ent["ws_ptr"] != ws.data_ptr() or ent["ws_floats"] > ws.numel():
        arr = (WgradDesc * n)(*descs)
        jb = int(lib.vd_conv_wgrad_group_job_bytes())
        host = (C.c_uint8 * (n * jb))()
        wsf, blocks, rblocks = C.c_int64(0), C.c_int32(0), C.c_int32(0)
        cls = lib.vd_conv_wgrad_group_plan(arr, n, host, C.byref(wsf), C.byref(blocks), C.byref(rblocks))
        if cls <= 0:
            raise L.VillanHipError(f"vd_conv_wgrad_group_plan: {lib.vd_last_error().decode()}")
        if ws is None or ws.numel() < wsf.value:
            ws = torch.empty(max(int(wsf.value), 1 << 22), device=device, dtype=torch.float32)
            _WG_WS[device] = ws
        ws_ptr = ws.data_ptr()
        table = upload_table(torch.frombuffer(bytearray(host), dtype=torch.uint8), device,
                             after=lambda t: L.check(lib.vd_conv_wgrad_group_rebase(t.data_ptr(), n, ws_ptr, _s()), "vd_conv_wgrad_group_rebase"))
        if len(_WG_CACHE) > 256:
            _WG_CACHE.clear()
        ent = _WG_CACHE[key] = {"table": table, "cls": cls, "blocks": blocks.value, "rblocks": rblocks.value, "ws_ptr": ws.data_ptr(),
                                "ws_floats": int(wsf.value)}
    if _CAPTURE_TABLES is not None:
        _CAPTURE_TABLES.append(ent["table"])
    flops = sum(2.0 * d.M * d.C * d.T * d.nb * d.NP for d in descs)
    nbytes = sum(4.0 * (d.nb * d.M * d.NP + d.nb * d.C * d.H * d.W + d.M * d.C * d.T) for d in descs)
    name = _kernel_name(lib.vd_conv_wgrad_group_kernel_name, ent["cls"]) if _PROF is not None else None
    _timed(name, flops, "mfma", lambda: L.check(
        lib.vd_conv_wgrad_group_launch(ent["table"].data_ptr(), n, ent["cls"], ent["blocks"], ent["rblocks"], _s()), "vd_conv_wgrad_group_launch"),
        nbytes=nbytes)


def conv_wgrad(dy, x, dw2d, mode, ws: Optional[torch.Tensor], accumulate=False, splits=0, tile=0, pad=0, math_mode=0):
    d = wgrad_desc(dy, x, dw2d, mode, ws, accumulate, splits, tile, pad, math_mode)
    Bn, M, OH, OW = dy.shape
    Cc, T = x.shape[1], d.T
    lib = _lib()
    need = lib.vd_conv_wgrad_ws_floats(C.byref(d))
    if need > 0:
        assert ws is not None and ws.numel() >= need, f"wgrad workspace too small: need {need}"
    if _PROF is None:
        L.check(lib.vd_conv_wgrad(C.byref(d), _s()), "vd_conv_wgrad")
        return dw2d
    e0, e1 = torch.cuda.Event(enable_timing=True), torch.cuda.Event(enable_timing=True)
    e0.record()
    L.check(lib.vd_conv_wgrad(C.byref(d), _s()), "vd_conv_wgrad")
    e1.record()
    name = _kernel_name(lib.vd_conv_wgrad_kernel_name, C.byref(d))
    _PROF.append({"name": name, "flops": 2.0 * M * Cc * T * Bn * OH * OW, "bytes": 4.0 * (dy.numel() + x.numel() + M * Cc * T),
                  "e0": e0, "e1": e1, "kind": "mfma"})
    return dw2d


def _wgrad_s2_split(OW) -> bool:
    sel = os.environ.get("VILLAN_WGRAD_S2", "all")
    return sel == "all" or (sel != "none" and OW >= 32)


@functools.lru_cache(maxsize=None)
def _wgrad_split_kernel(M, Cc, OH, OW, mode) -> bool:
    return _wgrad_tile(wgrad_query_desc(M, Cc, OH, OW, mode)) == (5 if mode == B_PLAIN else 4)


def wgrad_bx3_eligible(M, Cc, OH, OW, mode) -> bool:
    return _wgrad_split_kernel(M, Cc, OH, OW, mode) and (mode != B_CONV3_S2 or _wgrad_s2_split(OW))


def wgrad_ws_floats(M, Cc, T, nb, NP, OH=None, OW=None, mode=None, math_mode=0) -> int:
    if OH is None:
        OH = OW = int(round(math.sqrt(NP)))
    d = wgrad_query_desc(M, Cc, OH, OW, (B_PLAIN if T == 1 else B_CONV3) if mode is None else mode, nb, math_mode, NP=NP)
    return int(L.load().vd_conv_wgrad_ws_floats(C.byref(d)))


def weight_transpose(w2d, wt, M, Cc, T):
    L.check(_lib().vd_weight_transpose(_p(w2d), _p(wt), M, Cc, T, _s()), "vd_weight_transpose")
    return wt


def sumpool2x2(dU, dX, accumulate=False):
    Bn, Cc, H, W, xbs = _img(dX)
    ubs = _img(dU)[4]
    assert dU.shape == (Bn, Cc, 2 * H, 2 * W)
    L.check(_lib().vd_sumpool2x2(_p(dU), _p(dX), Bn, Cc, H, W, ubs, xbs, int(accumulate), _s()), "vd_sumpool2x2")
    return dX


def conv3x3_s2_dgrad(dy, w2d, dx, pad=0, a_packed=None):
    Bn, M, OH, OW, dbs = _img(dy)
    Bx, Cc, H, W, xbs = _img(dx)
    assert Bx == Bn and w2d.shape == (M, Cc * 9) and w2d.is_contiguous()
    OHW = OH * OW
    G = torch.empty((Bn, Cc * 9, OHW), device=dy.device, dtype=torch.float32)
    gemm(w2d, dy, G, M=Cc * 9, N=Bn * OHW, K=M, a_mode=A_COL, b_mode=B_PLAIN, NP=OHW, lda=Cc * 9, ldb=OHW, b_bstride=dbs,
         ldd=OHW, d_bstride=Cc * 9 * OHW, a_packed=a_packed)
    L.check(_lib().vd_col2im_s2(_p(G), _p(dx), Bn, Cc, H, W, OH, OW, pad, Cc * 9 * OHW, xbs, _s()), "vd_col2im_s2")
    return dx


def rowsum(x, ws, ws_ld=None):
    Bn, M, H, W, xbs = _img(x)
    ld = M if ws_ld is None else ws_ld
    L.check(_lib().vd_rowsum(_p(x), _p(ws), Bn, M, H * W, xbs, ld, _s()), "vd_rowsum")
    return ws


def colsum(ws, out, Bn, Cc, ld=None, accumulate=False):
    L.check(_lib().vd_colsum(_p(ws), _p(out), Bn, Cc, Cc if ld is None else ld, int(accumulate), _s()), "vd_colsum")
    return out


def colsum_segmented(table, n_jobs, Bn):
    assert table.dtype == torch.int64 and table.is_contiguous() and table.numel() >= 4 * n_jobs
    L.check(_lib().vd_colsum_segmented(_p(table), n_jobs, Bn, _s()), "vd_colsum_segmented")


def _gn_ws(Bn, Cc, HW, G, device):
    need = _lib().vd_groupnorm_ws_floats(Bn, Cc, HW, G)
    return _gemm_ws(need, device) if need > 0 else None


GN_FWD, GN_BWD, GN_STATS = 0, 1, 2


def groupnorm_plan(which, Bn, Cc, HW, G, aligned=True, has_ws=None, stream=None):
    lib = L.load()
    if has_ws is None:
        has_ws = lib.vd_groupnorm_ws_floats(Bn, Cc, HW, G) > 0
    buf = C.create_string_buffer(128)
    S = lib.vd_groupnorm_plan(which, Bn, Cc, HW, G, int(aligned), int(has_ws), stream, buf, len(buf))
    L.check(min(S, 0), "vd_groupnorm_plan")
    return buf.value.decode(), S


def groupnorm_fwd(x, gamma, beta, y, mean, rstd, G, eps, silu):
    Bn, Cc, H, W, xbs = _img(x)
    ybs = _img(y)[4]
    assert y.shape == x.shape and mean.numel() >= Bn * G and rstd.numel() >= Bn * G
    _timed("groupnorm_fwd (gn_fwd_reg_kernel<*> / gn_chunk_*)", 8.0 * x.numel(), "hbm", lambda: L.check(
        _lib().vd_groupnorm_fwd(_p(x), _p(gamma), _p(beta), _p(y), _p(mean), _p(rstd), Bn, Cc, H * W, G, eps,
                                int(silu), xbs, ybs, _p(_gn_ws(Bn, Cc, H * W, G, x.device)), _s()), "vd_groupnorm_fwd"))
    return y


def groupnorm_stats(x, gamma, beta, ss, mean, rstd, G, eps):
    Bn, Cc, H, W, xbs = _img(x)
    assert ss.shape == (Bn, Cc, 2) and ss.is_contiguous()
    L.check(_lib().vd_groupnorm_stats(_p(x), _p(gamma), _p(beta), _p(ss), _p(mean), _p(rstd), Bn, Cc, H * W, G, eps, xbs, _s()),
            "vd_groupnorm_stats")
    return ss


def groupnorm_stats_from_partials(part, tiles, gamma, beta, ss, mean, rstd, HW, G, eps):
    Bn, Cc = ss.shape[0], ss.shape[1]
    assert ss.is_contiguous() and part.is_contiguous() and part.numel() >= Bn * tiles * Cc * 2
    L.check(_lib().vd_groupnorm_stats_from_partials(_p(part), tiles, _p(gamma), _p(beta), _p(ss), _p(mean), _p(rstd), Bn, Cc, HW, G, eps, _s()),
            "vd_groupnorm_stats_from_partials")
    return ss


def gn_fusable(x, cout) -> bool:
    Bn, Cc, H, W = x.shape
    return W in (16, 32) and H == W and Cc % 8 == 0 and Cc <= 1024 and cout >= 64


def groupnorm_bwd(dy, x, mean, rstd, gamma, beta, dx, dgamma_ws, dbeta_ws, G, silu, extra=None, extra2=None, rowsum=None, rowsum_ld=None):
    Bn, Cc, H, W, xbs = _img(x)
    dbs, dxbs = _img(dy)[4], _img(dx)[4]
    ebs = _img(extra)[4] if extra is not None else 0
    e2bs = _img(extra2)[4] if extra2 is not None else 0
    assert dgamma_ws.numel() >= Bn * Cc and dbeta_ws.numel() >= Bn * Cc
    assert extra2 is None or extra2.shape == x.shape
    rld = 0
    if rowsum is not None:
        rld = Cc if rowsum_ld is None else rowsum_ld
        assert rld >= Cc
    nbytes = (12.0 + (4.0 if extra is not None else 0.0) + (4.0 if extra2 is not None else 0.0)) * x.numel()
    _timed("groupnorm_bwd (gn_bwd_reg_kernel<*> / gn_chunk_*)", nbytes, "hbm", lambda: L.check(
        _lib().vd_groupnorm_bwd_fused(_p(dy), _p(x), _p(mean), _p(rstd), _p(gamma), _p(beta), _p(extra), _p(extra2), _p(dx),
                                      _p(dgamma_ws), _p(dbeta_ws), _p(rowsum), Bn, Cc, H * W, G, int(silu), dbs, xbs, ebs, e2bs, dxbs, rld,
                                      _p(_gn_ws(Bn, Cc, H * W, G, x.device)), _s()), "vd_groupnorm_bwd"))
    return dx


def softmax_col_fwd(S, nb, N):
    L.check(_lib().vd_softmax_col_fwd(_p(S), nb, N, _s()), "vd_softmax_col_fwd")
    return S
# ... 374 lines not shown
                                 c_z, seed, offset, _s()), "vd_sched_step")
    return out


def batch_l2norm(x, out):
    Bn = x.shape[0]
    assert x.is_contiguous() and out.numel() >= Bn
    L.check(_lib().vd_batch_l2norm(_p(x), _p(out), Bn, x.numel() // Bn, _s()), "vd_batch_l2norm")
    return out


def ssim(a, b, win, out, c1, c2):
    Bn, Cc, H, W = a.shape
    assert a.is_contiguous() and b.is_contiguous() and win.is_contiguous() and a.shape == b.shape and win.shape[0] == win.shape[1]
    L.check(_lib().vd_ssim(_p(a), _p(b), _p(win), _p(out), Bn, Cc, H, W, win.shape[0], c1, c2, _s()), "vd_ssim")
    return out


def postprocess(x, out, mul, add, lo, hi, to_nhwc):
    Bn, Cc, H, W = x.shape
    assert x.is_contiguous() and out.is_contiguous()
    L.check(_lib().vd_postprocess(_p(x), _p(out), Bn, Cc, H * W, mul, add, lo, hi, int(to_nhwc), _s()), "vd_postprocess")
    return out


def fir_resample2(x, out, up: bool, scale: float = 1.0, accumulate: bool = False):
    Bn, Cc, H, W = x.shape
    assert x.is_contiguous() and out.is_contiguous()
    assert out.shape == ((Bn, Cc, 2 * H, 2 * W) if up else (Bn, Cc, H // 2, W // 2)), (x.shape, out.shape, up)
    L.check(_lib().vd_fir_resample2(_p(x), _p(out), Bn * Cc, H, W, int(up), scale, int(accumulate), _s()), "vd_fir_resample2")
    return out


def pyramid_dgrad(g, w, out, coarse=None, accumulate: bool = False):
    Bn, K, H, W, gbs = _img(g)
    Cc = w.shape[1]
    assert w.is_contiguous() and tuple(w.shape) == (K, Cc) and w.dtype == torch.float32 and 1 <= Cc <= 4
    assert out.is_contiguous() and tuple(out.shape) == (Bn, Cc, H, W) and out.dtype == torch.float32
    assert coarse is None or (coarse.is_contiguous() and tuple(coarse.shape) == (Bn, Cc, H // 2, W // 2) and coarse.dtype == torch.float32
                              and H % 2 == 0 and W % 2 == 0)
    _timed("pyramid_dgrad (pyramid_dgrad_kernel)", 4.0 * (g.numel() + (2 + int(accumulate)) * out.numel()), "hbm", lambda: L.check(
        _lib().vd_pyramid_dgrad(_p(g), _p(w), _p(coarse), _p(out), Bn, K, Cc, H, W, gbs, int(accumulate), _s()), "vd_pyramid_dgrad"))
    return out


def fourier_embedding(t_f32, W, emb):
    Bn, half = t_f32.numel(), W.numel()
    assert emb.shape == (Bn, 2 * half) and emb.is_contiguous()
    L.check(_lib().vd_fourier_embedding(_p(t_f32), _p(W), _p(emb), Bn, half, _s()), "vd_fourier_embedding")
    return emb


def rowscale(x, s, out, divide=False):
    Bn = x.shape[0]
    assert x.is_contiguous() and out.is_contiguous() and s.numel() == Bn
    L.check(_lib().vd_rowscale(_p(x), _p(s), _p(out), Bn, x.numel() // Bn, int(divide), _s()), "vd_rowscale")
    return out


def vq_nearest(z, codebook, zq, idx=None):
    Bn, D, H, W, zbs = _img(z)
    qbs = _img(zq)[4]
    assert zq.shape == z.shape and codebook.is_contiguous() and codebook.shape[1] == D
    assert idx is None or (idx.dtype == torch.int64 and idx.numel() >= Bn * H * W)
    L.check(_lib().vd_vq_nearest(_p(z), _p(codebook), _p(zq), _p(idx), Bn, D, H * W, codebook.shape[0], zbs, qbs, _s()),
            "vd_vq_nearest")
    return zq


def randn(out, seed, offset):
    L.check(_lib().vd_randn(_p(out), out.numel(), seed, offset, _s()), "vd_randn")
    return out


def poison_batch(img_u8, flags_u8, trigger, target, pixel_values, tgt, image_out, vmin, vmax, R_trigger_only=False, idx=None):
    _, H, W, Cc = img_u8.shape
    Bn = flags_u8.numel()
    assert img_u8.dtype == torch.uint8 and flags_u8.dtype == torch.uint8 and img_u8.is_contiguous()
    assert idx is None or (idx.dtype == torch.int64 and idx.numel() == Bn and idx.is_contiguous())
    assert idx is not None or img_u8.shape[0] == Bn
    L.check(_lib().vd_poison_batch(_p(img_u8), _p(idx), _p(flags_u8), _p(trigger), _p(target), _p(pixel_values), _p(tgt),
                                   _p(image_out), Bn, Cc, H, W, vmin, vmax, int(R_trigger_only), _s()), "vd_poison_batch")
    return pixel_values, tgt
```

### villandiffusion_amd/unet.py

```python
from __future__ import annotations

import math
import os
from types import SimpleNamespace
from typing import Dict, List, Optional, Tuple

import torch

from . import ops
from .flatnet import FlatParamNet
from .lib import B_CONV3, B_CONV3_DIL, B_CONV3_S2, B_CONV3_T, B_CONV3_UP, B_PLAIN, A_COL, A_ROW, B_KCONTIG


CONV_MATH_DEFAULT = os.environ.get("VILLAN_CONV_MATH", "bf16x3")
if CONV_MATH_DEFAULT not in ("bf16x3", "f32", "f16", "bf16"):
    raise ValueError(f"VILLAN_CONV_MATH must be 'bf16x3', 'f32', 'f16' or 'bf16', got {CONV_MATH_DEFAULT!r}")


class _PackedConvWeights:

    def __init__(self, net, f16: bool = False):
        self.net = net
        self.f16 = f16
        self.off = {False: {}, True: {}}
        self.jobs = {False: [], True: []}
        self.total = 0
        cands = []
        for name, shape, _ in net._layout:
            if name.endswith(".weight") and len(shape) == 4 and shape[2] == shape[3] and shape[2] in (1, 3):
                cands.append((name[:-7], (lambda n=name: net.P[n]), shape[0], shape[1], shape[2] * shape[3]))
        for prefix, ch in getattr(net, "_qkv", []):
            if prefix + "::qkv_w" in getattr(net, "Pq", {}):
                cands.append((prefix + "::qkv", (lambda k=prefix + "::qkv_w": net.Pq[k]), 3 * ch, ch, 1))
            if prefix + ".to_out.0.weight" in net.P:
                cands.append((prefix + ".to_out.0", (lambda n=prefix + ".to_out.0.weight": net.P[n]), ch, ch, 1))
        plan = []
        for key, get, cout, cin, T in cands:
            for bwd, (M, Cc, rs, cs) in ((False, (cout, cin, cin * T, T)), (True, (cin, cout, T, cin * T))):
                plan.append((key, get, bwd, M, Cc, T, rs, cs))
            if T == 9 and ".downsamplers." in key:
                plan.append((key + "::s2g", get, True, cin * 9, cout, 1, 1, cin * 9))
        for key, get, bwd, M, Cc, T, rs, cs in plan:
            if Cc % 16 == 0 and M >= 64:
                n = (M + 127) // 128 * 128 * Cc * T // (2 if f16 else 1)
                self.off[bwd][key] = (self.total, n)
                self.jobs[bwd].append((key, get, M, Cc, T, rs, cs))
                self.total += n
        self.buf: Optional[torch.Tensor] = None
        self.tables = {}
        self.key = {False: None, True: None}

    def view(self, prefix, bwd):
        ent = self.off[bwd].get(prefix)
        if ent is None:
            return None
        self.refresh(bwd)
        return self.buf[ent[0]:ent[0] + ent[1]]

    def refresh(self, bwd):
        net = self.net
        if not self.jobs[bwd]:
            return
        key = (net.flat_param._version, ops.WEIGHTS_EPOCH)
        if self.key[bwd] != key:
            if self.buf is None:
                self.buf = torch.empty(self.total, device=net.flat_param.device, dtype=torch.int32)
            if bwd not in self.tables:
                rows, blk = [], 0
                for k, get, M, Cc, T, rs, cs in self.jobs[bwd]:
                    o, n = self.off[bwd][k]
                    rows.append([get().data_ptr(), self.buf.data_ptr() + 4 * o, M, Cc, rs, cs, blk, T])
                    blk += ((M + 127) // 128 * 128 * (Cc // 16) * 2 + 255) // 256
                self.tables[bwd] = (torch.tensor(rows, dtype=torch.int64).to(self.buf.device), len(rows), blk)
            tab, nj, blk = self.tables[bwd]
            (ops.conv3_pack_weights_f16_multi if self.f16 else ops.conv3_pack_weights_multi)(tab, nj, blk)
            self.key[bwd] = key


def _split(net) -> bool:
    return getattr(net, "conv_math", "f32") in ("bf16x3", "f16", "bf16")


def _pairs(net) -> bool:
    return getattr(net, "conv_math", "f32") in ("bf16x3", "bf16")


def _with_mixed(net, pk, key, bwd):
    mode = getattr(net, "conv_math", "f32")
    if pk is None or mode not in ("f16", "bf16"):
        return pk
    if mode == "bf16":
        return (pk, pk, 3)
    p16 = getattr(net, "_packed16", None)
    if p16 is None:
        p16 = net._packed16 = _PackedConvWeights(net, f16=True)
    v16 = p16.view(key, bwd)
    return pk if v16 is None else (pk, v16)


def _bx3_packed(net, prefix, bwd, M, Cc, OH, OW, mode):
    if not _split(net) or not ops.bx3_eligible(M, Cc, OH, OW, mode):
        return None
    pk = getattr(net, "_packed", None)
    if pk is None:
        pk = net._packed = _PackedConvWeights(net)
    return _with_mixed(net, pk.view(prefix, bwd), prefix, bwd)


def _bx3_packed_1x1(net, key, bwd, M, K, NP, nb=None):
    if not _split(net) or not ops.gemm_bx3_eligible(M, K, NP, nb):
        return None
    pk = getattr(net, "_packed", None)
    if pk is None:
        pk = net._packed = _PackedConvWeights(net)
    return _with_mixed(net, pk.view(key, bwd), key, bwd)


def _conv1x1_dgrad(net, prefix, cout, cin, dout):
    B, _, H, W = dout.shape
    HW = H * W
    dx = torch.empty((B, cin, H, W), device=dout.device, dtype=torch.float32)
    ops.gemm(net.P[prefix + ".weight"].view(cout, cin), dout, dx, M=cin, N=B * HW, K=cout, a_mode=A_COL, b_mode=B_PLAIN, NP=HW, lda=cin, ldb=HW,
             b_bstride=ops._img(dout)[4], ldd=HW, d_bstride=cin * HW, a_packed=_bx3_packed_1x1(net, prefix, True, cin, cout, HW, B))
    return dx


def _amath(net, M, K, NP) -> int:
    return int(_split(net) and ops.gemm_bx3_act_eligible(M, K, NP))


def _wgrad1x1_math(net, dy, x) -> int:
    ok = _split(net) and ops.wgrad_bx3_eligible(dy.shape[1], x.shape[1], dy.shape[2], dy.shape[3], B_PLAIN) \
        and x.stride(0) % 4 == 0 and dy.stride(0) % 4 == 0
    return int(ok)


class _Conv:

    def __init__(self, net, prefix, cin, cout, mode=B_CONV3, pad=0):
        self.net, self.prefix, self.cin, self.cout, self.mode, self.pad = net, prefix, cin, cout, mode, pad
        net._decl(prefix + ".weight", (cout, cin, 3, 3), fan_in=cin * 9)
        net._decl(prefix + ".bias", (cout,), fan_in=cin * 9, is_bias=True)

    def w2d(self):
        return self.net.P[self.prefix + ".weight"].view(self.cout, self.cin * 9)

    def fwd(self, x, out, rowadd=None, rowadd_bstride=0, residual=None, gn_ss=None, gn_part=None):
        pk = _bx3_packed(self.net, self.prefix, False, self.cout, self.cin, out.shape[2], out.shape[3], self.mode)
        if gn_ss is not None and (out.shape[3] not in (16, 32) or self.mode != B_CONV3):
            pk = None
        return ops.conv3x3(x, self.w2d(), self.net.P[self.prefix + ".bias"], out, mode=self.mode, rowadd=rowadd,
                           rowadd_bstride=rowadd_bstride, residual=residual, pad=self.pad, gn_ss=gn_ss, a_packed=pk, gn_part=gn_part)

    def us_input(self, h, save):
        net = self.net
        B, _, H, W = h.shape
        if (self.mode != B_CONV3_UP or not net.us_fwd_presplit or not getattr(net, "presplit", False) or not _pairs(net) or H != W
                or not ops.conv_presplit_ok(B, self.cin, self.cout, 2 * H, 2 * W, B_CONV3_UP)
                or (save and not (net.group_wgrad and ops.wgrad_presplit_ok(B, self.cin, self.cout, 2 * H, B_CONV3_UP)))):
            return h
        return ops.presplit_pack(h)

    def bwd(self, dout, x, dx, bias_ws=None, skip_bias=False, dout_ps=None):
        net = self.net
        dout_f32 = dout
        gw = net.G[self.prefix + ".weight"].view(self.cout, self.cin * 9)
        want = net.wants_wgrad(gw)
        if isinstance(x, ops.PreSplit):
            if want:
                dy_ps = dout_ps if dout_ps is not None else net.pack_later(dout)
                net.wgrad(dy_ps, x, gw, self.mode, pad=self.pad, math_mode=1)
            if dout_ps is not None:
                dout = dout_ps
        elif (self.mode == B_CONV3_UP and getattr(net, "presplit", False) and _pairs(net) and net.group_wgrad
              and dout.shape[2] == dout.shape[3] and ops.wgrad_presplit_ok(dout.shape[0], self.cin, self.cout, dout.shape[3], B_CONV3_UP)):
            if want:
                dy_ps = dout_ps if dout_ps is not None else net.pack_later(dout)
                net.wgrad(dy_ps, net.pack_later(x), gw, self.mode, pad=self.pad, math_mode=1)
        else:
            assert dout is not None
            bx3 = _split(net) and ops.wgrad_bx3_eligible(self.cout, self.cin, dout.shape[2], dout.shape[3],
                                                                                           self.mode) and x.stride(0) % 4 == 0
            if want:
                net.wgrad(dout, x, gw, self.mode, pad=self.pad, math_mode=int(bx3))
        if not skip_bias:
            B = dout.shape[0]
            ws = bias_ws if bias_ws is not None else net.scratch_bc(B, self.cout)
            if bias_ws is None:
                assert dout_f32 is not None
                net.rowsum(dout_f32, ws)
            net.colsum_later(ws, net.G[self.prefix + ".bias"], B, self.cout, ld=(ws.stride(0) if ws.dim() == 2 else self.cout))
        if dx is None:
            return None
        if self.mode == B_CONV3_S2:
            pk = _bx3_packed_1x1(net, self.prefix + "::s2g", True, self.cin * 9, self.cout, dout.shape[2] * dout.shape[3], dout.shape[0])
            return ops.conv3x3_s2_dgrad(dout, self.w2d(), dx, pad=self.pad, a_packed=pk)
        pk = _bx3_packed(net, self.prefix, True, self.cin, self.cout, dout.shape[2], dout.shape[3], B_CONV3_T) \
            if self.mode in (B_CONV3, B_CONV3_UP) else None
        wt = net.wt_view(self.prefix, self.cout, self.cin, 9, fresh=pk is None)
        if self.mode == B_CONV3:
            ops.conv3x3(dout, wt, None, dx, mode=B_CONV3_T, a_packed=pk)
        elif self.mode == B_CONV3_UP:
            B, _, OH, OW = dout.shape
            if pk is not None and ops.bx3_pool2_eligible(self.cin, self.cout, OH, OW, B):
                src = dout_ps if (dout_ps is not None and net.us_dgrad_presplit and ops.conv_presplit_ok(B, self.cout, self.cin, OH, OW, B_CONV3_T)) else dout
                ops.conv3x3(src, wt, None, dx, mode=B_CONV3_T, a_packed=pk, pool2=True)
            else:
                dU = torch.empty((B, self.cin, OH, OW), device=dout.device, dtype=torch.float32)
                ops.conv3x3(dout, wt, None, dU, mode=B_CONV3_T, a_packed=pk)
                ops.sumpool2x2(dU, dx)
        else:
            raise NotImplementedError(self.mode)
        return dx


class _Norm:
    def __init__(self, net, prefix, ch, silu, groups=None):
        self.net, self.prefix, self.ch, self.silu = net, prefix, ch, silu
        self.groups = net.groups if groups is None else groups
        net._decl(prefix + ".weight", (ch,), ones=True)
        net._decl(prefix + ".bias", (ch,), zeros=True)

    def fwd(self, x, y):
        net = self.net
        B = x.shape[0]
        mean = torch.empty(B * self.groups, device=x.device, dtype=torch.float32)
        rstd = torch.empty_like(mean)
        ops.groupnorm_fwd(x, net.P[self.prefix + ".weight"], net.P[self.prefix + ".bias"], y, mean, rstd, self.groups,
                          net.eps, self.silu)
        return mean, rstd

    def fwd_ps(self, x):
        net = self.net
        B = x.shape[0]
        mean = torch.empty(B * self.groups, device=x.device, dtype=torch.float32)
        rstd = torch.empty_like(mean)
        y = ops.presplit_empty(x.shape, x.device)
        ops.groupnorm_fwd_presplit(x, net.P[self.prefix + ".weight"], net.P[self.prefix + ".bias"], y, mean, rstd, self.groups, net.eps, self.silu)
        return y, mean, rstd

    def ps_ok(self, HW: int) -> bool:
        return ops.groupnorm_presplit_ok(self.ch, HW, self.groups)

    def stats(self, x):
        net = self.net
        B = x.shape[0]
        ss = torch.empty((B, self.ch, 2), device=x.device, dtype=torch.float32)
        mean = torch.empty(B * self.groups, device=x.device, dtype=torch.float32)
        rstd = torch.empty_like(mean)
        ops.groupnorm_stats(x, net.P[self.prefix + ".weight"], net.P[self.prefix + ".bias"], ss, mean, rstd, self.groups, net.eps)
        return ss

    def stats_from_partials(self, part, tiles, B, HW):
        net = self.net
        ss = torch.empty((B, self.ch, 2), device=part.device, dtype=torch.float32)
        mean = torch.empty(B * self.groups, device=part.device, dtype=torch.float32)
        rstd = torch.empty_like(mean)
        ops.groupnorm_stats_from_partials(part, tiles, net.P[self.prefix + ".weight"], net.P[self.prefix + ".bias"], ss, mean, rstd, HW,
                                          self.groups, net.eps)
        return ss

    def bwd(self, dy, x, mean, rstd, dx, extra=None, extra2=None, rowsum=None, dx_ps=None):
        net = self.net
        B = x.shape[0]
        wg, wb = net.scratch_bc(B, self.ch, 1), net.scratch_bc(B, self.ch, 2)
        if dx_ps is not None:
            ops.groupnorm_bwd_presplit(dy, x, mean, rstd, net.P[self.prefix + ".weight"], net.P[self.prefix + ".bias"], dx, dx_ps, wg, wb,
                                       self.groups, self.silu, extra=extra, extra2=extra2, rowsum=rowsum,
                                       rowsum_ld=(rowsum.stride(0) if rowsum is not None else None))
        else:
            ops.groupnorm_bwd(dy, x, mean, rstd, net.P[self.prefix + ".weight"], net.P[self.prefix + ".bias"], dx, wg, wb,
                              self.groups, self.silu, extra=extra, extra2=extra2, rowsum=rowsum,
                              rowsum_ld=(rowsum.stride(0) if rowsum is not None else None))
        net.colsum_later(wg, net.G[self.prefix + ".weight"], B, self.ch)
        net.colsum_later(wb, net.G[self.prefix + ".bias"], B, self.ch)
        return dx


class _Resnet:
# ... 354 lines not shown
        self._begin_declarations(device)
        self._temb: List[Tuple[str, int]] = []
        temb_dim = boc[0] * 4
        self.time_dim0, self.temb_dim = boc[0], temb_dim
        self._decl("time_embedding.linear_1.weight", (temb_dim, boc[0]), fan_in=boc[0])
        self._decl("time_embedding.linear_1.bias", (temb_dim,), fan_in=boc[0], is_bias=True)
        self._decl("time_embedding.linear_2.weight", (temb_dim, temb_dim), fan_in=temb_dim)
        self._decl("time_embedding.linear_2.bias", (temb_dim,), fan_in=temb_dim, is_bias=True)
        self._conv_in = _Conv(self, "conv_in", in_channels, boc[0])

        self.down: List[dict] = []
        ch = boc[0]
        skip_ch = [ch]
        for i, typ in enumerate(down_block_types):
            cin, ch = ch, boc[i]
            blk = {"res": [], "attn": [], "ds": None}
            for j in range(layers_per_block):
                blk["res"].append(_Resnet(self, f"down_blocks.{i}.resnets.{j}", cin if j == 0 else ch, ch))
                if typ == "AttnDownBlock2D":
                    blk["attn"].append(_Attn(self, f"down_blocks.{i}.attentions.{j}", ch, attention_head_dim))
                skip_ch.append(ch)
            if i != len(boc) - 1:
                blk["ds"] = _Conv(self, f"down_blocks.{i}.downsamplers.0.conv", ch, ch, mode=B_CONV3_S2, pad=downsample_padding)
                skip_ch.append(ch)
            self.down.append(blk)
        self.mid_res = [_Resnet(self, "mid_block.resnets.0", ch, ch), _Resnet(self, "mid_block.resnets.1", ch, ch)]
        self.mid_attn = _Attn(self, "mid_block.attentions.0", ch, attention_head_dim)

        rev = boc[::-1]
        self.up: List[dict] = []
        out_ch = rev[0]
        sk = list(skip_ch)
        for i, typ in enumerate(up_block_types):
            prev, out_ch = out_ch, rev[i]
            in_ch = rev[min(i + 1, len(boc) - 1)]
            blk = {"res": [], "attn": [], "us": None, "h_ch": [], "skip_ch": []}
            for j in range(layers_per_block + 1):
                s_ch = sk.pop()
                assert s_ch == (in_ch if j == layers_per_block else out_ch)
                h_ch = prev if j == 0 else out_ch
                blk["res"].append(_Resnet(self, f"up_blocks.{i}.resnets.{j}", h_ch + s_ch, out_ch))
                blk["h_ch"].append(h_ch)
                blk["skip_ch"].append(s_ch)
                if typ == "AttnUpBlock2D":
                    blk["attn"].append(_Attn(self, f"up_blocks.{i}.attentions.{j}", out_ch, attention_head_dim))
            if i != len(boc) - 1:
                blk["us"] = _Conv(self, f"up_blocks.{i}.upsamplers.0.conv", out_ch, out_ch, mode=B_CONV3_UP)
            self.up.append(blk)
        assert not sk
        self.norm_out = _Norm(self, "conv_norm_out", boc[0], True)
        self._conv_out = _Conv(self, "conv_out", boc[0], out_channels)
        self._materialise()

    def _decl_temb(self, prefix, cout) -> int:
        off = sum(c for _, c in self._temb)
        self._temb.append((prefix, cout))
        return off

    def _materialise(self):
        head = [(prefix + ".weight", (cout, self.temb_dim), dict(fan_in=self.temb_dim)) for prefix, cout in self._temb]
        head += [(prefix + ".bias", (cout,), dict(fan_in=self.temb_dim, is_bias=True)) for prefix, cout in self._temb]
        super()._materialise(head, grads=True)
        layout, offs, total, dev = self._layout, self._offs, self.flat_numel, self._dev
        n_t = sum(c for _, c in self._temb)
        o0 = offs[self._temb[0][0] + ".weight"][0]
        ob = offs[self._temb[0][0] + ".bias"][0]
        self.temb_total = n_t
        self.Wt_all = self.flat_param[o0:o0 + n_t * self.temb_dim].view(n_t, self.temb_dim)
        self.bt_all = self.flat_param[ob:ob + n_t]
        self.gWt_all = self.flat_grad[o0:o0 + n_t * self.temb_dim].view(n_t, self.temb_dim)
        self.gbt_all = self.flat_grad[ob:ob + n_t]
        self._wt_offs, wt_total = {}, 0
        for name, shape, _ in layout:
            if name.endswith(".weight") and len(shape) == 4 and shape[2] == 3 and name != "conv_in.weight":
                self._wt_offs[name[:-7]] = wt_total
                wt_total += int(math.prod(shape))
        self._wt_offs["conv_in"] = wt_total
        wt_total += int(math.prod(offs["conv_in.weight"][2]))
        self._wt_total = wt_total
        self._wt_buf: Optional[torch.Tensor] = None
        self.wgrad_ws: Optional[torch.Tensor] = None
        self._cs_pool: Optional[torch.Tensor] = None
        self._cs_tables: Dict[tuple, torch.Tensor] = {}
        self._cs_cols_hint = 4 * sum(int(math.prod(sh)) for _, sh, _ in layout if len(sh) == 1) + 4096
        self._cs_off, self._cs_jobs, self._cs_B, self._cs_retired = 0, [], 0, []
        self._d_temb: Dict[int, torch.Tensor] = {}
        half = self.time_dim0 // 2
        exponent = -math.log(10000) * torch.arange(0, half, dtype=torch.float32)
        exponent = exponent / (half - self.config.freq_shift)
        self.freqs = torch.exp(exponent).to(dev)
        self._anchor = torch.zeros(1, device=dev, requires_grad=True)
        def _late(k):
            return ".time_emb_proj." in k or ".to_q." in k or ".to_k." in k or ".to_v." in k
        o_in = offs["conv_in.weight"][0]
        o_mid = min(v[0] for k, v in offs.items() if k.startswith("mid_block.") and not _late(k))
        o_up = min(v[0] for k, v in offs.items() if k.startswith("up_blocks.") and not _late(k))
        self.grad_buckets = [(o_up, total), (o_mid, o_up), (o_in, o_mid), (0, o_in)]
        self.bucket_ready_hook = None
        self.fuse_gn_inference = None
        self.fused_attention = os.environ.get("VILLAN_FUSED_ATTENTION", "1") != "0"
        self.sampler_graph = os.environ.get("VILLAN_SAMPLER_GRAPH", "1") != "0"
        self.group_wgrad = os.environ.get("VILLAN_GROUP_WGRAD", "1") != "0"
        self._wg_jobs: Dict[int, list] = {}
        self.wgrad_stream = os.environ.get("VILLAN_WGRAD_STREAM", "1") != "0"
        self.wgrad_flush_jobs = int(os.environ.get("VILLAN_WGRAD_FLUSH_JOBS", "24"))
        self._wg_side, self._wg_keep, self._rs_jobs = None, [], []
        self.fuse_gn_bwd = os.environ.get("VILLAN_FUSE_GN_BWD", "1") != "0"
        self.presplit = os.environ.get("VILLAN_PRESPLIT", "1") != "0"
        self.nograd_presplit = os.environ.get("VILLAN_NOGRAD_PRESPLIT", "1") != "0"
        self.us_dgrad_presplit = os.environ.get("VILLAN_US_DGRAD_PRESPLIT", "1") != "0"
        self.us_fwd_presplit = os.environ.get("VILLAN_US_FWD_PRESPLIT", "1") != "0"
        self.sc_stream = os.environ.get("VILLAN_SC_STREAM", "1") != "0"
        self._aux_stream = None
        self.gn_stats_in_epilogue = os.environ.get("VILLAN_GN_STATS_IN_EPILOGUE", "1") != "0"
        self._pk_jobs = []
        self.conv_math = CONV_MATH_DEFAULT
        self._packed: Optional[_PackedConvWeights] = None
        self._packed16: Optional[_PackedConvWeights] = None
        self._wt_fresh = set()

    def zero_grad(self, set_to_none: bool = False):
        ops.scale_(self.flat_grad, 0.0)

    def refresh_packed(self, bwd: bool):
        for pk in (self._packed, self._packed16):
            if pk is not None:
                pk.refresh(bwd)

    def weights_changed(self):
        for pk in (self._packed, self._packed16):
            if pk is not None:
                pk.key = {False: None, True: None}

    def _cs_begin(self, B):
        need = B * self._cs_cols_hint
        if self._cs_pool is None or self._cs_pool.numel() < need:
            self._cs_pool = torch.empty(need, device=self._dev, dtype=torch.float32)
            self._cs_tables = {}
        self._cs_off, self._cs_jobs, self._cs_B = 0, [], B
        self._cs_retired = []

    def scratch_bc(self, B, Cc, slot=0):
        n = (B * Cc + 3) // 4 * 4
        if self._cs_off + n > self._cs_pool.numel():
            self._cs_flush()
            self._cs_retired.append(self._cs_pool)
            self._cs_cols_hint *= 2
            self._cs_pool = torch.empty(B * self._cs_cols_hint, device=self._dev, dtype=torch.float32)
            self._cs_tables, self._cs_off = {}, 0
        t = self._cs_pool[self._cs_off:self._cs_off + B * Cc]
        self._cs_off += n
        return t

    def colsum_later(self, ws, out, B, Cc, ld=None):
        if self._dx_only or self.lora_route is not None:
            return
        ld = Cc if ld is None else ld
        wp, op = ws.data_ptr(), out.data_ptr()
        for c0 in range(0, Cc, 64):
            self._cs_jobs.append((wp + 4 * c0, op + 4 * c0, min(64, Cc - c0), ld))

    def wants_wgrad(self, dw2d) -> bool:
        if self._dx_only:
            return False
        return self.lora_route is None or self.lora_route.wants(self, dw2d)

    def wgrad(self, dy, x, dw2d, mode, pad=0, math_mode=0):
        if self._dx_only:
            return
        route = self.lora_route
        if route is not None and route.take(self, dy, x, dw2d, mode):
            if self.wgrad_stream and self.lora_flush_jobs and len(route.jobs) >= self.lora_flush_jobs:
                self._lora_flush()
            return
        if math_mode == 1 and self.group_wgrad:
            d = ops.wgrad_desc(dy, x, dw2d, mode, None, accumulate=True, pad=pad, math_mode=1)
            if self.conv_math == "bf16":
                d3 = ops.wgrad_desc(dy, x, dw2d, mode, None, accumulate=True, pad=pad, math_mode=3)
                if ops.wgrad_group_class(d3):
                    d = d3
            cls = ops.wgrad_group_class(d)
            if cls:
                self._wg_jobs.setdefault(cls, []).append((d, dy, x))
                if self.wgrad_stream and self.wgrad_flush_jobs and sum(len(v) for v in self._wg_jobs.values()) >= self.wgrad_flush_jobs:
                    self._wg_flush()
                return
        ops.conv_wgrad(dy, x, dw2d, mode, self.wgrad_ws, accumulate=True, pad=pad, math_mode=math_mode)

    def aux_fork(self) -> bool:
        if not self.sc_stream or self._dev.type != "cuda":
            return False
        if self._aux_stream is None:
            self._aux_stream = torch.cuda.Stream(device=self._dev)
        if _split(self) and self._packed is None:
            self._packed = _PackedConvWeights(self)
        if self.conv_math == "f16" and self._packed16 is None:
            self._packed16 = _PackedConvWeights(self, f16=True)
        for pk in (self._packed, self._packed16):
            if pk is not None:
                pk.refresh(False)
                pk.refresh(True)
        self._aux_stream.wait_stream(torch.cuda.current_stream(self._dev))
        return True

    def aux_scope(self):
        import contextlib
        stack = contextlib.ExitStack()
        stack.enter_context(torch.cuda.stream(self._aux_stream))
        stack.enter_context(ops.ws_slot(ops.AUX_WS_SLOT))
        return stack

    def aux_join(self):
        torch.cuda.current_stream(self._dev).wait_stream(self._aux_stream)

    def pack_later(self, t):
        if self._dx_only:
            return None
        out = ops.presplit_empty(t.shape, t.device)
        if self.wgrad_stream and self.group_wgrad:
            self._pk_jobs.append((t, out))
        else:
            ops.presplit_pack(t, out=out)
        return out

    def rowsum(self, x, ws, ws_ld=None):
        if self._dx_only:
            return
        route = self.lora_route
        if route is not None and not (route.temb and self._in_d_temb(ws)):
            return
        if self.wgrad_stream and self.group_wgrad:
            self._rs_jobs.append((x, ws, ws_ld))
        else:
            ops.rowsum(x, ws, ws_ld=ws_ld)

    def _in_d_temb(self, ws) -> bool:
        return any(t.data_ptr() <= ws.data_ptr() < t.data_ptr() + 4 * t.numel() for t in self._d_temb.values())

    def _lora_flush(self):
        if self._wg_side is None:
            self._wg_side = torch.cuda.Stream(device=self._dev)
        self._wg_side.wait_stream(torch.cuda.current_stream(self._dev))
        with torch.cuda.stream(self._wg_side):
            done = self.lora_route.flush(self._dev)
        self._wg_keep.append(("direct", done))

    def _wg_flush(self):
        route = self.lora_route
        direct = route is not None and bool(route.jobs)
        if not any(self._wg_jobs.values()) and not self._rs_jobs and not self._pk_jobs and not direct:
            return
        if self.wgrad_stream:
            if self._wg_side is None:
                self._wg_side = torch.cuda.Stream(device=self._dev)
            main = torch.cuda.current_stream(self._dev)
            self._wg_side.wait_stream(main)
            with torch.cuda.stream(self._wg_side):
                for t, out in self._pk_jobs:
                    ops.presplit_pack(t, out=out)
                for x, ws, ld in self._rs_jobs:
                    ops.rowsum(x, ws, ws_ld=ld)
                for cls, jobs in self._wg_jobs.items():
                    if jobs:
                        ops.conv_wgrad_group([j[0] for j in jobs], self._dev)
                done = route.flush(self._dev) if direct else None
            self._wg_keep.append((self._wg_jobs, self._rs_jobs, self._pk_jobs, done))
            self._rs_jobs, self._pk_jobs = [], []
        else:
            for t, out in self._pk_jobs:
                ops.presplit_pack(t, out=out)
            self._pk_jobs = []
            for cls, jobs in self._wg_jobs.items():
                if jobs:
                    ops.conv_wgrad_group([j[0] for j in jobs], self._dev)
            if direct:
                route.flush(self._dev)
        self._wg_jobs = {}

    def _wg_join(self):
        if self._wg_keep:
            torch.cuda.current_stream(self._dev).wait_stream(self._wg_side)
            self._wg_keep = []

    def _bucket_boundary(self, i: int, hook):
        if not self.wgrad_stream or os.environ.get("VILLAN_BUCKET_JOIN", "0") == "1":
            self._cs_flush()
            hook(i)
            return
        if self._wg_side is None:
            self._wg_side = torch.cuda.Stream(device=self._dev)
        self._wg_flush()
        self._wg_side.wait_stream(torch.cuda.current_stream(self._dev))
        with torch.cuda.stream(self._wg_side):
            self._cs_launch()
            hook(i)
        self._wg_keep.append(("bucket", i))

    def _cs_flush(self):
        self._wg_flush()
        self._wg_join()
        self._cs_launch()

    def _cs_launch(self):
        jobs = self._cs_jobs
        if not jobs:
            return
        key = tuple(jobs)
        tab = self._cs_tables.get(key)
        if tab is None:
            tab = ops.upload_table(torch.tensor(jobs, dtype=torch.int64), self._dev)
            self._cs_tables[key] = tab
        if ops._CAPTURE_TABLES is not None:
            ops._CAPTURE_TABLES.append(tab)
        ops.colsum_segmented(tab, len(jobs), self._cs_B)
        self._cs_jobs = []

    def _d_temb_buffer(self, B):
        t = self._d_temb.get(B)
        if t is None:
            t = torch.zeros((B, self.temb_total), device=self._dev, dtype=torch.float32)
            self._d_temb[B] = t
        else:
            ops.scale_(t, 0.0)
        return t

    def wt_view(self, prefix, M, Cc, T, fresh=True):
        off = self._wt_offs[prefix]
        if fresh and prefix not in self._wt_fresh:
            ops.weight_transpose(self.P[prefix + ".weight"], self._wt_buf[off:off + M * Cc * T], M, Cc, T)
            self._wt_fresh.add(prefix)
        return self._wt_buf[off:off + M * Cc * T].view(Cc, M * T)

    def _prepare_backward(self, B, weights=True):
        if self._wg_keep:
            self._wg_join()
        self._wg_jobs, self._rs_jobs, self._pk_jobs = {}, [], []
        if self.lora_route is not None:
            self.lora_route.jobs = []
        if self._wt_buf is None:
            self._wt_buf = torch.empty(self._wt_total, device=self._dev, dtype=torch.float32)
        self._wt_fresh = set()
        if not weights:
            return
        if self.wgrad_ws is None or getattr(self, "_ws_B", None) != B:
            need = 0
            S = self.sample_size
            for name, shape, _ in self._layout:
                if name.endswith(".weight") and len(shape) == 4:
                    M, Cc, T = shape[0], shape[1], shape[2] * shape[3]
                    for hw in {(S >> k) ** 2 for k in range(len(self.config.block_out_channels))}:
                        for md in ((B_PLAIN,) if T == 1 else (B_CONV3, B_CONV3_UP, B_CONV3_S2)):
                            need = max(need, ops.wgrad_ws_floats(M, Cc, T, B, hw, mode=md))
                        side = int(round(math.sqrt(hw)))
                        for md in (B_CONV3, B_CONV3_UP, B_CONV3_S2):
                            if T == 9 and ops.wgrad_bx3_eligible(M, Cc, side, side, md):
                                need = max(need, ops.wgrad_ws_floats(M, Cc, T, B, hw, mode=md, math_mode=1))
                        if T == 1 and ops.wgrad_bx3_eligible(M, Cc, side, side, B_PLAIN):
                            need = max(need, ops.wgrad_ws_floats(M, Cc, T, B, hw, mode=B_PLAIN, math_mode=1))
            for prefix, ch in self._qkv:
                for hw in {(S >> k) ** 2 for k in range(len(self.config.block_out_channels))}:
                    need = max(need, ops.wgrad_ws_floats(3 * ch, ch, 1, B, hw), ops.wgrad_ws_floats(ch, ch, 1, B, hw))
                    if hw % 8 == 0 and ch >= 64:
                        need = max(need, ops.wgrad_ws_floats(3 * ch, ch, 1, B, hw, mode=B_PLAIN, math_mode=1),
                                   ops.wgrad_ws_floats(ch, ch, 1, B, hw, mode=B_PLAIN, math_mode=1))
            self.wgrad_ws = torch.empty(max(need, 4), device=self._dev, dtype=torch.float32)
            self._ws_B = B

    def forward(self, sample: torch.Tensor, timestep, return_dict: bool = False):
        x = sample
        if x.device != self._dev:
            x = x.to(self._dev)
        x = x.contiguous().float()
        B = x.shape[0]
        t = timestep
        if not torch.is_tensor(t):
            t = torch.tensor([t], device=self._dev)
        t = t.to(self._dev)
        if t.dim() == 0:
            t = t[None]
        t = t.to(torch.float32).expand(B).contiguous()
        if torch.is_grad_enabled() and any(p.requires_grad for p in self.parameters()):
            out = _UNetFn.apply(self, x, t, self._anchor)
        elif torch.is_grad_enabled() and self._input_grad and x.requires_grad:
            out = _UNetFn.apply(self, x, t, None)
        else:
            out, _ = self._run_forward(x, t, save=False)
        if return_dict:
            return SimpleNamespace(sample=out)
        return (out,)

    def _new(self, B, Cc, S):
        return torch.empty((B, Cc, S, S), device=self._dev, dtype=torch.float32)

    def _run_forward(self, x, t, save):
        dev = self._dev
        B, _, S, _ = x.shape
        st = SimpleNamespace(saved=[], B=B)
        sv = st.saved
        st.marks = {}
        emb_sin = torch.empty((B, self.time_dim0), device=dev, dtype=torch.float32)
        ops.timestep_embedding(t, self.freqs, emb_sin, self.config.flip_sin_to_cos)
        e1 = torch.empty((B, self.temb_dim), device=dev, dtype=torch.float32)
        ops.linear(emb_sin, self.P["time_embedding.linear_1.weight"], self.P["time_embedding.linear_1.bias"], e1)
        e1a = ops.silu_fwd(e1, torch.empty_like(e1))
        emb = torch.empty_like(e1)
        ops.linear(e1a, self.P["time_embedding.linear_2.weight"], self.P["time_embedding.linear_2.bias"], emb)
        emb_act = ops.silu_fwd(emb, torch.empty_like(emb))
        st.temb_all = torch.empty((B, self.temb_total), device=dev, dtype=torch.float32)
        ops.linear(emb_act, self.Wt_all, self.bt_all, st.temb_all)
        if save:
            st.temb_saved = (emb_sin, e1, e1a, emb, emb_act)

        up_slots = []
        sp = S >> (len(self.down) - 1)
        for bi, blk in enumerate(self.up):
            for j in range(len(blk["res"])):
                up_slots.append((blk["h_ch"][j], blk["skip_ch"][j], sp))
            if blk["us"] is not None:
                sp *= 2
        n_skip = len(up_slots)
        cats: List[Optional[torch.Tensor]] = [None] * n_skip

        def skip_out(k, ch, spatial):
            h_ch, s_ch, s_sp = up_slots[n_skip - 1 - k]
            assert s_ch == ch and s_sp == spatial, (k, ch, spatial, up_slots[n_skip - 1 - k])
            buf = self._new(B, h_ch + s_ch, spatial)
            cats[n_skip - 1 - k] = buf
            return buf[:, h_ch:]

        k = 0
        h = skip_out(k, self._conv_in.cout, S); k += 1
        self._conv_in.fwd(x, h)
        if save:
            sv.append(("conv_in", x))
        sp = S
        for blk in self.down:
            for j, res in enumerate(blk["res"]):
                if blk["attn"]:
                    tmp = self._new(B, res.cout, sp)
                    s = res.fwd(h, tmp, st, save)
                    out = skip_out(k, res.cout, sp); k += 1
                    s2 = blk["attn"][j].fwd(tmp, out, st, save)
                    if save:
                        sv.append(("res", res, s)); sv.append(("attn", blk["attn"][j], s2))
                else:
                    out = skip_out(k, res.cout, sp); k += 1
                    s = res.fwd(h, out, st, save)
                    if save:
                        sv.append(("res", res, s))
                h = out
            if blk["ds"] is not None:
                sp //= 2
                out = skip_out(k, blk["ds"].cout, sp); k += 1
                blk["ds"].fwd(h, out)
                if save:
                    sv.append(("ds", blk["ds"], h))
                h = out
        assert k == n_skip
        st.marks["down_end"] = len(sv)
        tmp = self._new(B, self.mid_res[0].cout, sp)
        s = self.mid_res[0].fwd(h, tmp, st, save)
        tmp2 = self._new(B, self.mid_res[0].cout, sp)
        s2 = self.mid_attn.fwd(tmp, tmp2, st, save)
        slot = 0
        out = cats[slot][:, :up_slots[slot][0]]
        s3 = self.mid_res[1].fwd(tmp2, out, st, save)
        if save:
            sv.append(("res", self.mid_res[0], s)); sv.append(("attn", self.mid_attn, s2)); sv.append(("res", self.mid_res[1], s3))
        st.marks["mid_end"] = len(sv)
        final = None
        for bi, blk in enumerate(self.up):
            nres = len(blk["res"])
            for j, res in enumerate(blk["res"]):
                xin = cats[slot]
                last_of_net = (slot == n_skip - 1)
                nxt_in_block = j + 1 < nres
                if nxt_in_block:
                    dest = cats[slot + 1][:, :up_slots[slot + 1][0]]
                elif blk["us"] is not None:
# ... 32 lines not shown
        return out, st

    def _run_backward(self, st, dout, want_dx=False, weights=True):
        if not weights:
            if not want_dx:
                return None
            self._dx_only = True
            try:
                return self._backward_tape(st, dout, True, False)
            finally:
                self._dx_only = False
        return self._backward_tape(st, dout, want_dx, True)

    def _backward_tape(self, st, dout, want_dx, weights):
        dev = self._dev
        B = st.B
        self._prepare_backward(B, weights)
        self._cs_begin(B)
        st.d_temb_all = self._d_temb_buffer(B)
        up_slots = st.up_slots
        n_skip = len(up_slots)
        dcats: List[Optional[torch.Tensor]] = [None] * n_skip
        sv = st.saved
        _, final, a, mo, ro = sv.pop()
        da = torch.empty_like(a)
        self._conv_out.bwd(dout, a, da)
        g = torch.empty(final.shape, device=dev, dtype=torch.float32)
        fuse = self.fuse_gn_bwd
        g_rs = self.scratch_bc(B, final.shape[1]).view(B, final.shape[1]) if fuse else None

        def wants_ps(norm, shape):
            if not sv or not norm.ps_ok(shape[2] * shape[3]):
                return None
            nxt = sv[-1]
            if nxt[0] == "res" and isinstance(nxt[2][5], ops.PreSplit):
                return ops.presplit_empty(shape, dev)
            if (nxt[0] == "us" and self.presplit and _pairs(self) and self.group_wgrad
                    and ops.wgrad_presplit_ok(shape[0], nxt[1].cin, nxt[1].cout, shape[3], B_CONV3_UP)):
                return ops.presplit_empty(shape, dev)
            return None

        g_ps = wants_ps(self.norm_out, final.shape)
        self.norm_out.bwd(da, final, mo, ro, g, rowsum=g_rs, dx_ps=g_ps)
        slot = n_skip
        hook = self.bucket_ready_hook if weights else None
        dx_in = None
        while sv:
            if hook is not None:
                if len(sv) == st.marks["mid_end"]:
                    self._bucket_boundary(0, hook)
                elif len(sv) == st.marks["down_end"]:
                    self._bucket_boundary(1, hook)
            rec = sv.pop()
            kind = rec[0]
            if kind in ("res", "attn"):
                layer, saved = rec[1], rec[2]
                x = saved[0]
                is_cat_input = kind == "res" and any(x.data_ptr() == c.data_ptr() and x.shape == c.shape for c in st.cats)
                dx = torch.empty(x.shape, device=dev, dtype=torch.float32)
                rs = self.scratch_bc(B, x.shape[1]).view(B, x.shape[1]) if fuse else None
                dxp = wants_ps(layer.norm1 if kind == "res" else layer.norm, x.shape) if fuse else None
                if is_cat_input:
                    slot -= 1
                    dcats[slot] = dx
                    layer.bwd(saved, g, dx, st, dout_rs=g_rs, dx_rs=rs, dout_ps=g_ps, dx_ps=dxp)
                    g = dx[:, :up_slots[slot][0]]
                    g_rs = rs[:, :up_slots[slot][0]] if fuse else None
                    g_ps = dxp.channels(0, up_slots[slot][0]) if dxp is not None and up_slots[slot][0] % 8 == 0 else None
                elif fuse:
                    layer.bwd(saved, g, dx, st, dout_rs=g_rs, extra2=self._skip_grad(x, st, dcats), dx_rs=rs, dout_ps=g_ps, dx_ps=dxp)
                    g, g_rs, g_ps = dx, rs, dxp
                else:
                    layer.bwd(saved, g, dx, st, dout_ps=g_ps)
                    g, g_ps = dx, None
                    g = self._add_skip_grad(g, x, st, dcats)
            elif kind == "us":
                layer, x = rec[1], rec[2]
                dx = torch.empty(x.shape, device=dev, dtype=torch.float32)
                layer.bwd(g, x, dx, bias_ws=g_rs, dout_ps=g_ps)
                g, g_rs, g_ps = dx, None, None
            elif kind == "ds":
                layer, x = rec[1], rec[2]
                dx = torch.empty(x.shape, device=dev, dtype=torch.float32)
                layer.bwd(g, x, dx, bias_ws=g_rs)
                g, g_rs, g_ps = self._add_skip_grad(dx, x, st, dcats), None, None
            elif kind == "conv_in":
                if want_dx:
                    dx_in = torch.empty(rec[1].shape, device=dev, dtype=torch.float32)
                self._conv_in.bwd(g, rec[1], dx_in, bias_ws=g_rs)
            else:
                raise RuntimeError(kind)
        if not weights:
            return dx_in
        self._cs_flush()
        if hook is not None:
            hook(2)
        if self.lora_route is not None and not self.lora_route.temb:
            if hook is not None:
                hook(3)
            return dx_in
        emb_sin, e1, e1a, emb, emb_act = st.temb_saved
        d = st.d_temb_all
        ops.linear_wgrad(d, emb_act, self.gWt_all, accumulate=True)
        self.colsum_later(d, self.gbt_all, B, self.temb_total)
        d_act = torch.empty_like(emb_act)
        ops.linear_dgrad(d, self.Wt_all, d_act)
        d_emb = ops.silu_bwd(d_act, emb, torch.empty_like(emb))
        ops.linear_wgrad(d_emb, e1a, self.G["time_embedding.linear_2.weight"], accumulate=True)
        ops.colsum(d_emb, self.G["time_embedding.linear_2.bias"], B, self.temb_dim, accumulate=True)
        d_e1a = torch.empty_like(e1a)
        ops.linear_dgrad(d_emb, self.P["time_embedding.linear_2.weight"], d_e1a)
        d_e1 = ops.silu_bwd(d_e1a, e1, torch.empty_like(e1))
        ops.linear_wgrad(d_e1, emb_sin, self.G["time_embedding.linear_1.weight"], accumulate=True)
        ops.colsum(d_e1, self.G["time_embedding.linear_1.bias"], B, self.temb_dim, accumulate=True)
        self._cs_flush()
        if hook is not None:
            hook(3)
        return dx_in

    def _skip_grad(self, x, st, dcats):
        for k, c in enumerate(st.cats):
            h_ch = st.up_slots[k][0]
            if x.shape[1:] == c[:, h_ch:].shape[1:] and x.data_ptr() == c[:, h_ch:].data_ptr():
                return dcats[k][:, h_ch:]
        return None

    def _add_skip_grad(self, g, x, st, dcats):
        sg = self._skip_grad(x, st, dcats)
        if sg is not None:
            ops.add_strided(g, sg, accumulate=True)
        return g
```

Before: 7618.

## Batch rowsums, fuse s2 dgrad skip-add, coalesce wgrad reduce, merge weight packing

Several independent changes. Per-layer rowsum launches are grouped into one segmented kernel driven by a cached job table. The stride-2 dgrad col2im now adds the skip gradient in the same pass instead of a separate add. The wgrad split reduce gets a coalesced vector path that stages results through LDS. Forward and backward packed-weight refreshes are merged into a single multi-pack launch, and a GPU-resident poisoning kernel is added. The goal is fewer kernel launches and memory passes, at the cost of extra table management and new code paths that could be wrong.

```diff
diff --git a/include/villan_hip.h b/include/villan_hip.h
--- a/include/villan_hip.h
+++ b/include/villan_hip.h
@@ -111,6 +111,7 @@
 int vd_conv_wgrad_group_plan(const vd_wgrad_desc* descs, int n, void* table_out, int64_t* ws_floats, int* blocks, int* rblocks);
 int vd_conv_wgrad_group_rebase(void* dev_table, int n, float* ws, void* stream);
 int vd_conv_wgrad_group_launch(const void* dev_table, int n, int cls, int blocks, int rblocks, void* stream);
+int vd_conv_wgrad_group_reduce(const void* dev_table, int n, int rblocks, void* stream);
 int vd_conv_wgrad_group_kernel_name(int cls, char* name, int name_len);
 
 int64_t vd_conv3_packed_bytes(int M, int C, int taps);
@@ -123,7 +124,10 @@
                   int accumulate, void* stream);
 int vd_col2im_s2(const float* G, float* dX, int B, int C, int H, int W, int OH, int OW, int pad, int64_t g_bstride,
                  int64_t dx_bstride, void* stream);
+int vd_col2im_s2_add(const float* G, float* dX, const float* add, int B, int C, int H, int W, int OH, int OW, int pad,
+                     int64_t g_bstride, int64_t dx_bstride, int64_t add_bstride, void* stream);
 int vd_rowsum(const float* X, float* ws, int B, int M, int P, int64_t x_bstride, int64_t ws_ld, void* stream);
+int vd_rowsum_segmented(const int64_t* table, int n_jobs, int B, int blocks, void* stream);
 int vd_colsum(const float* ws, float* out, int B, int C, int64_t ld, int accumulate, void* stream);
 int vd_colsum_segmented(const int64_t* table, int n_jobs, int B, void* stream);
 
@@ -237,6 +241,9 @@
 int vd_poison_batch(const uint8_t* img, const int64_t* idx, const uint8_t* flags, const float* trigger, const float* target,
                     float* pixel_values, float* tgt_out, float* image_out, int B, int C, int H, int W, float vmin,
                     float vmax, int R_trigger_only, void* stream);
+int vd_poison_batch_resident(const uint8_t* img, const int64_t* pos, const int64_t* index, const uint8_t* flags, const float* u,
+                             const float* trigger, const float* target, float* pixel_values, float* tgt_out, float* image_out,
+                             uint8_t* is_clean, int B, int C, int H, int W, float vmin, float vmax, void* stream);
 
 int vd_pool3(const float* x, float* y, int B, int C, int H, int W, int stride, int pad, int mode, int64_t x_bstride, int64_t y_bstride,
              void* stream);
diff --git a/villandiffusion_amd/csrc/vd_elem.hip b/villandiffusion_amd/csrc/vd_elem.hip
--- a/villandiffusion_amd/csrc/vd_elem.hip
+++ b/villandiffusion_amd/csrc/vd_elem.hip
@@ -355,6 +355,24 @@
     }
 }
 
+__device__ __forceinline__ void poison_pixel(const uint8_t* __restrict__ img, int64_t sb, uint8_t f, const float* __restrict__ trigger,
+                                             const float* __restrict__ target, float* __restrict__ pv, float* __restrict__ tg,
+                                             float* __restrict__ image_out, int64_t i, int64_t r, int c, int yh, int xw, int C, int H, int W,
+                                             float vmin, float vmax, float denom, int r_trigger_only) {
+    const int xs = (f & 2) ? (W - 1 - xw) : xw;
+    const float u = (float)img[((sb * H + yh) * W + xs) * C + c] / 255.0f;
+    const float xv = add_rn(mul_rn(sub_rn(u, 0.0f) / denom, sub_rn(vmax, vmin)), vmin);
+    if (image_out) image_out[i] = xv;
+    if (f & 1) {
+        const float tr = trigger[r];
+        pv[i] = r_trigger_only ? tr : ((tr > vmin) ? tr : xv);
+        tg[i] = target[r];
+    } else {
+        pv[i] = 0.f;
+        tg[i] = xv;
+    }
+}
+
 __global__ void poison_kernel(const uint8_t* __restrict__ img, const int64_t* __restrict__ idx, const uint8_t* __restrict__ flags,
                               const float* __restrict__ trigger, const float* __restrict__ target, float* __restrict__ pv,
                               float* __restrict__ tg, float* __restrict__ image_out, int B, int C, int H, int W, float vmin,
@@ -366,20 +384,28 @@
         const int xw = (int)(r % W);
         const int64_t cy = r / W;
         const int yh = (int)(cy % H), c = (int)(cy / H);
-        const uint8_t f = flags[b];
-        const int xs = (f & 2) ? (W - 1 - xw) : xw;
-        const int64_t sb = idx ? idx[b] : (int64_t)b;
-        const float u = (float)img[((sb * H + yh) * W + xs) * C + c] / 255.0f;
-        const float xv = add_rn(mul_rn(sub_rn(u, 0.0f) / denom, sub_rn(vmax, vmin)), vmin);
-        if (image_out) image_out[i] = xv;
-        if (f & 1) {
-            const float tr = trigger[r];
-            pv[i] = r_trigger_only ? tr : ((tr > vmin) ? tr : xv);
-            tg[i] = target[r];
-        } else {
-            pv[i] = 0.f;
-            tg[i] = xv;
-        }
+        poison_pixel(img, idx ? idx[b] : (int64_t)b, flags[b], trigger, target, pv, tg, image_out, i, r, c, yh, xw, C, H, W, vmin, vmax, denom,
+                     r_trigger_only);
+    }
+}
+
+__global__ void poison_resident_kernel(const uint8_t* __restrict__ img, const int64_t* __restrict__ pos, const int64_t* __restrict__ index,
+                                       const uint8_t* __restrict__ flags, const float* __restrict__ u, const float* __restrict__ trigger,
+                                       const float* __restrict__ target, float* __restrict__ pv, float* __restrict__ tg,
+                                       float* __restrict__ image_out, uint8_t* __restrict__ is_clean, int B, int C, int H, int W, float vmin,
+                                       float vmax, float denom) {
+    const int64_t chw = (int64_t)C * H * W;
+    GRID_STRIDE(i, (int64_t)B * chw) {
+        const int b = (int)(i / chw);
+        const int64_t r = i - (int64_t)b * chw;
+        const int xw = (int)(r % W);
+        const int64_t cy = r / W;
+        const int yh = (int)(cy % H), c = (int)(cy / H);
+        const int64_t p = pos[b];
+        const uint8_t fl = flags[p];
+        const uint8_t f = (uint8_t)((fl & 1) | ((u && u[b] < 0.5f) ? 2 : 0));
+        poison_pixel(img, index[p], f, trigger, target, pv, tg, image_out, i, r, c, yh, xw, C, H, W, vmin, vmax, denom, 0);
+        if (is_clean && r == 0) is_clean[b] = (fl & 1) == 0;
     }
 }
 
@@ -941,6 +967,18 @@
     return 0;
 }
 
+extern "C" int vd_poison_batch_resident(const uint8_t* img, const int64_t* pos, const int64_t* index, const uint8_t* flags, const float* u,
+                                        const float* trigger, const float* target, float* pixel_values, float* tgt_out, float* image_out,
+                                        uint8_t* is_clean, int B, int C, int H, int W, float vmin, float vmax, void* stream) {
+    VD_REQUIRE(img && pos && index && flags && trigger && target && pixel_values && tgt_out, "vd_poison_batch_resident: null pointer");
+    VD_REQUIRE(B > 0 && C > 0 && H > 0 && W > 0, "vd_poison_batch_resident: bad dims");
+    const float denom = (float)(1.0 - 0.0 + 1e-5);
+    hipLaunchKernelGGL(poison_resident_kernel, dim3(egrid((int64_t)B * C * H * W)), dim3(EB), 0, ST, img, pos, index, flags, u, trigger,
+                       target, pixel_values, tgt_out, image_out, is_clean, B, C, H, W, vmin, vmax, denom);
+    VD_LAUNCH_CHECK("vd_poison_batch_resident");
+    return 0;
+}
+
 namespace {
 
 template <int MODE>
diff --git a/villandiffusion_amd/csrc/vd_gemm.hip b/villandiffusion_amd/csrc/vd_gemm.hip
--- a/villandiffusion_amd/csrc/vd_gemm.hip
+++ b/villandiffusion_amd/csrc/vd_gemm.hip
@@ -1720,7 +1720,8 @@
 }
 
 __global__ __launch_bounds__(256) void col2im_s2_kernel(const float* __restrict__ G, float* __restrict__ dX, int B, int C,
-                                                        int H, int W, int OH, int OW, int pad, int64_t g_bs, int64_t dx_bs) {
+                                                        int H, int W, int OH, int OW, int pad, int64_t g_bs, int64_t dx_bs,
+                                                        const float* __restrict__ add, int64_t add_bs) {
     const int64_t per = (int64_t)C * H * W, total = per * B;
     for (int64_t i = blockIdx.x * (int64_t)blockDim.x + threadIdx.x; i < total; i += (int64_t)gridDim.x * blockDim.x) {
         const int b = (int)(i / per);
@@ -1741,7 +1742,7 @@
                 acc += g[(r * 3 + s) * OH * OW + iy * OW + ix];
             }
         }
-        dX[(int64_t)b * dx_bs + q] = acc;
+        dX[(int64_t)b * dx_bs + q] = add ? (acc + add[(int64_t)b * add_bs + q]) : acc;
     }
 }
 
@@ -1770,9 +1771,8 @@
     if (threadIdx.x == 0) ws[(int64_t)b * ws_ld + m] = (part[0] + part[1]) + (part[2] + part[3]);
 }
 
-__global__ __launch_bounds__(256) void rowsum_kernel(const float* __restrict__ X, float* __restrict__ ws, int B, int M, int P,
-                                                     int64_t x_bs, int64_t ws_ld) {
-    const int row = blockIdx.x * 4 + (threadIdx.x >> 6);
+__device__ __forceinline__ void rowsum_row(const float* __restrict__ X, float* __restrict__ ws, int B, int M, int P, int64_t x_bs,
+                                           int64_t ws_ld, int row) {
     if (row >= B * M) return;
     const int b = row / M, m = row - b * M;
     const float* __restrict__ x = X + (int64_t)b * x_bs + (int64_t)m * P;
@@ -1798,6 +1798,24 @@
     }
     s = wave_sum(s);
     if (lane == 0) ws[(int64_t)b * ws_ld + m] = s;
+}
+
+__global__ __launch_bounds__(256) void rowsum_kernel(const float* __restrict__ X, float* __restrict__ ws, int B, int M, int P,
+                                                     int64_t x_bs, int64_t ws_ld) {
+    rowsum_row(X, ws, B, M, P, x_bs, ws_ld, blockIdx.x * 4 + (threadIdx.x >> 6));
+}
+
+constexpr int RS_SEG_FIELDS = 7;
+__global__ __launch_bounds__(256) void rowsum_seg_kernel(const int64_t* __restrict__ table, int n_jobs, int B) {
+    int lo = 0, hi = n_jobs - 1;
+    while (lo < hi) {
+        const int mid = (lo + hi + 1) >> 1;
+        if (table[(int64_t)mid * RS_SEG_FIELDS + 6] <= (int64_t)blockIdx.x) lo = mid;
+        else hi = mid - 1;
+    }
+    const int64_t* __restrict__ t = table + (int64_t)lo * RS_SEG_FIELDS;
+    rowsum_row(reinterpret_cast<const float*>(t[0]), reinterpret_cast<float*>(t[1]), B, (int)t[2], (int)t[3], t[4], t[5],
+               ((int)blockIdx.x - (int)t[6]) * 4 + (threadIdx.x >> 6));
 }
 
 __global__ __launch_bounds__(256) void colsum_kernel(const float* __restrict__ ws, float* __restrict__ out, int B, int C,
@@ -2515,10 +2533,17 @@
     }
     if (name) return vd_name_append(name, "(+group_reduce)");
     VD_LAUNCH_CHECK("vd_conv_wgrad_group_launch");
-    if (rblocks > 0) {
-        hipLaunchKernelGGL(wgrad_group_reduce_kernel, dim3(rblocks), dim3(256), 0, st, jobs, n);
-        VD_LAUNCH_CHECK("vd_conv_wgrad_group_launch/reduce");
-    }
+    if (rblocks > 0) return vd_conv_wgrad_group_reduce(dev_table, n, rblocks, st);
+    return 0;
+}
+
+extern "C" int vd_conv_wgrad_group_reduce(const void* dev_table, int n, int rblocks, void* stream) {
+    VD_REQUIRE(dev_table && n > 0 && rblocks > 0, "vd_conv_wgrad_group_reduce: bad args");
+    const char* rc_env = getenv("VILLAN_REDUCE_COALESCED");
+    const int lines = !(rc_env && rc_env[0] == '0' && rc_env[1] == 0);
+    hipLaunchKernelGGL(wgrad_group_reduce_kernel, dim3(rblocks), dim3(256), 0, (hipStream_t)stream,
+                       reinterpret_cast<const vd_wgrad_job*>(dev_table), n, lines);
+    VD_LAUNCH_CHECK("vd_conv_wgrad_group_reduce");
     return 0;
 }
 
@@ -2564,8 +2589,19 @@
     const int64_t total = (int64_t)B * C * H * W;
     const int grid = (int)((total + 255) / 256 < 16384 ? (total + 255) / 256 : 16384);
     hipLaunchKernelGGL(col2im_s2_kernel, dim3(grid), dim3(256), 0, (hipStream_t)stream, G, dX, B, C, H, W, OH, OW, pad, g_bstride,
-                       dx_bstride);
+                       dx_bstride, (const float*)nullptr, (int64_t)0);
     VD_LAUNCH_CHECK("vd_col2im_s2");
+    return 0;
+}
+
+extern "C" int vd_col2im_s2_add(const float* G, float* dX, const float* add, int B, int C, int H, int W, int OH, int OW, int pad,
+                                int64_t g_bstride, int64_t dx_bstride, int64_t add_bstride, void* stream) {
+    VD_REQUIRE(G && dX && B > 0 && C > 0 && H > 0 && W > 0 && OH > 0 && OW > 0 && (pad == 0 || pad == 1), "vd_col2im_s2_add: bad args");
+    const int64_t total = (int64_t)B * C * H * W;
+    const int grid = (int)((total + 255) / 256 < 16384 ? (total + 255) / 256 : 16384);
+    hipLaunchKernelGGL(col2im_s2_kernel, dim3(grid), dim3(256), 0, (hipStream_t)stream, G, dX, B, C, H, W, OH, OW, pad, g_bstride,
+                       dx_bstride, add, add_bstride);
+    VD_LAUNCH_CHECK("vd_col2im_s2_add");
     return 0;
 }
 
@@ -2580,6 +2616,13 @@
     return 0;
 }
 
+extern "C" int vd_rowsum_segmented(const int64_t* table, int n_jobs, int B, int blocks, void* stream) {
+    VD_REQUIRE(table && n_jobs > 0 && B > 0 && blocks > 0, "vd_rowsum_segmented: bad args");
+    hipLaunchKernelGGL(rowsum_seg_kernel, dim3(blocks), dim3(256), 0, (hipStream_t)stream, table, n_jobs, B);
+    VD_LAUNCH_CHECK("vd_rowsum_segmented");
+    return 0;
+}
+
 extern "C" int vd_colsum_segmented(const int64_t* table, int n_jobs, int B, void* stream) {
     VD_REQUIRE(table && n_jobs > 0 && B > 0, "vd_colsum_segmented: bad args");
     hipLaunchKernelGGL(colsum_seg_kernel, dim3(n_jobs), dim3(256), 0, (hipStream_t)stream, table, B);
diff --git a/villandiffusion_amd/csrc/vd_wgrad_bx3.inc b/villandiffusion_amd/csrc/vd_wgrad_bx3.inc
--- a/villandiffusion_amd/csrc/vd_wgrad_bx3.inc
+++ b/villandiffusion_amd/csrc/vd_wgrad_bx3.inc
@@ -447,10 +447,7 @@
 
 #include "vd_wgrad1x1_wide.inc"
 
-__global__ __launch_bounds__(256) void wgrad_group_reduce_kernel(const vd_wgrad_job* __restrict__ jobs, int n_jobs) {
-    const vd_wgrad_job* __restrict__ jb = jobs + wgrad_find_job(jobs, n_jobs, blockIdx.x, true);
-    const int lb = blockIdx.x - jb->first_rblock;
-    if (lb >= jb->rblocks || jb->gy <= 1) return;
+__device__ __forceinline__ void wgrad_reduce_strided(const vd_wgrad_job* __restrict__ jb, int lb) {
     const int M = jb->d.M, C = jb->d.C, T = jb->d.T, splits = jb->gy, accumulate = jb->d.accumulate;
     const float* __restrict__ ws = jb->d.ws;
     float* __restrict__ out = jb->d.dW;
@@ -505,6 +502,80 @@
     }
 }
 
+constexpr int RL_CH = 64;
+__device__ __forceinline__ void wgrad_reduce_lines(const vd_wgrad_job* __restrict__ jb, int lb, float* __restrict__ lds) {
+    const int M = jb->d.M, C = jb->d.C, splits = jb->gy, accumulate = jb->d.accumulate;
+    const f32x4* __restrict__ ws4 = reinterpret_cast<const f32x4*>(jb->d.ws);
+    float* __restrict__ out = jb->d.dW;
+    const int64_t n4 = ((int64_t)M * C * 9) >> 2;
+    const int runs = (C + RL_CH - 1) / RL_CH;
+    const int units = M * runs;
+    const int t = threadIdx.x;
+    for (int u = lb; u < units; u += jb->rblocks) {
+        const int m = u / runs, c0 = (u - m * runs) * RL_CH;
+        const int cl = min(RL_CH, C - c0);
+        const int q_per = (cl * 3) >> 2;
+        const int r = t / q_per, q = t - r * q_per;
+        const bool live = t < 3 * q_per;
+        if (live) {
+            const f32x4* __restrict__ p = ws4 + ((((int64_t)r * M + m) * C + c0) * 3 >> 2) + q;
+            f32x4 s = p[0];
+            int z = 1;
+            for (; z + 8 <= splits; z += 8) {
+                f32x4 v[8];
+#pragma unroll
+                for (int k = 0; k < 8; ++k) v[k] = p[(int64_t)(z + k) * n4];
+#pragma unroll
+                for (int k = 0; k < 8; ++k)
+#pragma unroll
+                    for (int j = 0; j < 4; ++j) s[j] = s[j] + v[k][j];
+            }
+            for (; z + 4 <= splits; z += 4) {
+                const f32x4 a = p[(int64_t)z * n4], b = p[(int64_t)(z + 1) * n4], c = p[(int64_t)(z + 2) * n4], e = p[(int64_t)(z + 3) * n4];
+#pragma unroll
+                for (int j = 0; j < 4; ++j) s[j] = (((s[j] + a[j]) + b[j]) + c[j]) + e[j];
+            }
+            for (; z < splits; ++z) {
+                const f32x4 a = p[(int64_t)z * n4];
+#pragma unroll
+                for (int j = 0; j < 4; ++j) s[j] += a[j];
+            }
+#pragma unroll
+            for (int j = 0; j < 4; ++j) {
+                const int e = 4 * q + j;
+                const int c = e / 3, sx = e - 3 * c;
+                lds[c * 9 + r * 3 + sx] = s[j];
+            }
+        }
+        __syncthreads();
+        if (live) {
+            const f32x4 s = *reinterpret_cast<const f32x4*>(lds + 4 * t);
+            f32x4* __restrict__ o = reinterpret_cast<f32x4*>(out + ((int64_t)m * C + c0) * 9) + t;
+            if (accumulate) {
+                const f32x4 old = *o;
+                f32x4 w;
+#pragma unroll
+                for (int j = 0; j < 4; ++j) w[j] = old[j] + s[j];
+                *o = w;
+            } else {
+                *o = s;
+            }
+        }
+        __syncthreads();
+    }
+}
+
+__global__ __launch_bounds__(256) void wgrad_group_reduce_kernel(const vd_wgrad_job* __restrict__ jobs, int n_jobs, int lines) {
+    __shared__ __attribute__((aligned(16))) float lds[RL_CH * 9];
+    const vd_wgrad_job* __restrict__ jb = jobs + wgrad_find_job(jobs, n_jobs, blockIdx.x, true);
+    const int lb = blockIdx.x - jb->first_rblock;
+    if (lb >= jb->rblocks || jb->gy <= 1) return;
+    if (lines && jb->d.T == 9 && (jb->d.C & 3) == 0 && (((uintptr_t)jb->d.ws | (uintptr_t)jb->d.dW) & 15) == 0)
+        wgrad_reduce_lines(jb, lb, lds);
+    else
+        wgrad_reduce_strided(jb, lb);
+}
+
 static bool wgrad1x1_bx3_eligible(const vd_wgrad_desc& d) {
     return d.math == 1 && d.T == 1 && d.mode == VD_B_PLAIN && d.NP % 8 == 0 && d.M >= 64 && d.C >= 64 && d.tile == 0 &&
            (d.x_bstride & 3) == 0 && (d.dy_bstride & 3) == 0 && ((((uintptr_t)d.X) | ((uintptr_t)d.dY)) & 15) == 0;
diff --git a/villandiffusion_amd/dataset.py b/villandiffusion_amd/dataset.py
--- a/villandiffusion_amd/dataset.py
+++ b/villandiffusion_amd/dataset.py
@@ -579,6 +579,17 @@
     def _make_batch_resident(self, pos: torch.Tensor, flip_bits: Optional[torch.Tensor]) -> Dict[str, torch.Tensor]:
         B = len(pos)
         pos = pos.long()
+        C, S = self._channel, self._image_size
+        if flip_bits is None and os.environ.get("VILLAN_BATCH_FUSED", "1") != "0":
+            u = torch.rand(B, device=self._dev, generator=self._flip_gen) if self.random_flip else None
+            pv, tg, im = (torch.empty((B, C, S, S), device=self._dev, dtype=torch.float32) for _ in range(3))
+            clean = torch.empty(B, device=self._dev, dtype=torch.bool) if self.batch_flags else None
+            ops.poison_batch_resident(self._dev_images, pos.contiguous(), self._dev_index, self._dev_flags, u, self._dev_trigger, self._dev_target,
+                                      pv, tg, im, clean, self._vmin, self._vmax)
+            batch = {self.PIXEL_VALUES: pv, self.TARGET: tg, self.IMAGE: im}
+            if clean is not None:
+                batch[self.IS_CLEAN] = clean
+            return batch
         ds_idx = self._dev_index.index_select(0, pos)
         fl = self._dev_flags.index_select(0, pos)
         if flip_bits is None:
@@ -588,7 +599,6 @@
         kflags = fl & 1
         if flip is not None:
             kflags = kflags | (flip.to(torch.uint8) << 1)
-        C, S = self._channel, self._image_size
         pv, tg, im = (torch.empty((B, C, S, S), device=self._dev, dtype=torch.float32) for _ in range(3))
         ops.poison_batch(self._dev_images, kflags.contiguous(), self._dev_trigger, self._dev_target, pv, tg, im, self._vmin, self._vmax,
                          R_trigger_only=False, idx=ds_idx)
diff --git a/villandiffusion_amd/lib.py b/villandiffusion_amd/lib.py
--- a/villandiffusion_amd/lib.py
+++ b/villandiffusion_amd/lib.py
@@ -60,6 +60,7 @@
     "vd_conv_wgrad_group_plan": (_i32, [C.POINTER(WgradDesc), _i32, _vp, C.POINTER(_i64), C.POINTER(_i32), C.POINTER(_i32)]),
     "vd_conv_wgrad_group_rebase": (_i32, [_vp, _i32, _vp, _vp]),
     "vd_conv_wgrad_group_launch": (_i32, [_vp, _i32, _i32, _i32, _i32, _vp]),
+    "vd_conv_wgrad_group_reduce": (_i32, [_vp, _i32, _i32, _vp]),
     "vd_conv3_packed_bytes": (_i64, [_i32, _i32, _i32]),
     "vd_conv3_pack_weights": (_i32, [_vp, _vp, _i32, _i32, _i32, _i64, _i64, _vp]),
     "vd_conv3_pack_weights_multi": (_i32, [_vp, _i32, _i64, _vp]),
@@ -67,7 +68,9 @@
     "vd_weight_transpose": (_i32, [_vp, _vp, _i32, _i32, _i32, _vp]),
     "vd_sumpool2x2": (_i32, [_vp, _vp, _i32, _i32, _i32, _i32, _i64, _i64, _i32, _vp]),
     "vd_col2im_s2": (_i32, [_vp, _vp, _i32, _i32, _i32, _i32, _i32, _i32, _i32, _i64, _i64, _vp]),
+    "vd_col2im_s2_add": (_i32, [_vp, _vp, _vp, _i32, _i32, _i32, _i32, _i32, _i32, _i32, _i64, _i64, _i64, _vp]),
     "vd_rowsum": (_i32, [_vp, _vp, _i32, _i32, _i32, _i64, _i64, _vp]),
+    "vd_rowsum_segmented": (_i32, [_vp, _i32, _i32, _i32, _vp]),
     "vd_colsum": (_i32, [_vp, _vp, _i32, _i32, _i64, _i32, _vp]),
     "vd_colsum_segmented": (_i32, [_vp, _i32, _i32, _vp]),
     "vd_groupnorm_ws_floats": (_i64, [_i32, _i32, _i32, _i32]),
@@ -124,6 +127,7 @@
     "vd_rowscale": (_i32, [_vp, _vp, _vp, _i32, _i64, _i32, _vp]),
     "vd_vq_nearest": (_i32, [_vp, _vp, _vp, _vp, _i32, _i32, _i32, _i32, _i64, _i64, _vp]),
     "vd_poison_batch": (_i32, [_vp] * 8 + [_i32] * 4 + [_f32, _f32, _i32, _vp]),
+    "vd_poison_batch_resident": (_i32, [_vp] * 11 + [_i32] * 4 + [_f32, _f32, _vp]),
     "vd_pool3": (_i32, [_vp, _vp, _i32, _i32, _i32, _i32, _i32, _i32, _i32, _i64, _i64, _vp]),
     "vd_resize_bilinear": (_i32, [_vp, _vp, _i64, _i32, _i32, _i32, _i32, _f32, _f32, _vp]),
     "vd_channel_affine": (_i32, [_vp, _vp, _vp, _vp, _i32, _i32, _i32, _vp]),
diff --git a/villandiffusion_amd/ops.py b/villandiffusion_amd/ops.py
--- a/villandiffusion_amd/ops.py
+++ b/villandiffusion_amd/ops.py
@@ -681,7 +681,11 @@
     return dX
 
 
-def conv3x3_s2_dgrad(dy, w2d, dx, pad=0, a_packed=None):
+def s2_dgrad_add_enabled() -> bool:
+    return os.environ.get("VILLAN_S2_DGRAD_ADD", "1") != "0"
+
+
+def conv3x3_s2_dgrad(dy, w2d, dx, pad=0, a_packed=None, add=None):
     Bn, M, OH, OW, dbs = _img(dy)
     Bx, Cc, H, W, xbs = _img(dx)
     assert Bx == Bn and w2d.shape == (M, Cc * 9) and w2d.is_contiguous()
@@ -689,7 +693,12 @@
     G = torch.empty((Bn, Cc * 9, OHW), device=dy.device, dtype=torch.float32)
     gemm(w2d, dy, G, M=Cc * 9, N=Bn * OHW, K=M, a_mode=A_COL, b_mode=B_PLAIN, NP=OHW, lda=Cc * 9, ldb=OHW, b_bstride=dbs,
          ldd=OHW, d_bstride=Cc * 9 * OHW, a_packed=a_packed)
-    L.check(_lib().vd_col2im_s2(_p(G), _p(dx), Bn, Cc, H, W, OH, OW, pad, Cc * 9 * OHW, xbs, _s()), "vd_col2im_s2")
+    if add is None:
+        L.check(_lib().vd_col2im_s2(_p(G), _p(dx), Bn, Cc, H, W, OH, OW, pad, Cc * 9 * OHW, xbs, _s()), "vd_col2im_s2")
+    else:
+        assert add.shape == dx.shape and add.dtype == torch.float32
+        L.check(_lib().vd_col2im_s2_add(_p(G), _p(dx), _p(add), Bn, Cc, H, W, OH, OW, pad, Cc * 9 * OHW, xbs, _img(add)[4], _s()),
+                "vd_col2im_s2_add")
     return dx
 
 
@@ -698,6 +707,32 @@
     ld = M if ws_ld is None else ws_ld
     L.check(_lib().vd_rowsum(_p(x), _p(ws), Bn, M, H * W, xbs, ld, _s()), "vd_rowsum")
     return ws
+
+
+ROWSUM_LONG_P = 8192
+
+
+def rowsum_grouped_enabled() -> bool:
+    return os.environ.get("VILLAN_ROWSUM_GROUPED", "1") != "0"
+
+
+def rowsum_job(x, ws, ws_ld=None):
+    Bn, M, H, W, xbs = _img(x)
+    return (x.data_ptr(), ws.data_ptr(), M, H * W, xbs, M if ws_ld is None else ws_ld)
+
+
+def rowsum_table(jobs, Bn):
+    rows, blk = [], 0
+    for j in jobs:
+        assert j[3] < ROWSUM_LONG_P and j[5] >= j[2]
+        rows.append(list(j) + [blk])
+        blk += (Bn * j[2] + 3) // 4
+    return torch.tensor(rows, dtype=torch.int64), blk
+
+
+def rowsum_segmented(table, n_jobs, Bn, blocks):
+    assert table.dtype == torch.int64 and table.is_contiguous() and table.numel() >= 7 * n_jobs
+    L.check(_lib().vd_rowsum_segmented(_p(table), n_jobs, Bn, blocks, _s()), "vd_rowsum_segmented")
 
 
 def colsum(ws, out, Bn, Cc, ld=None, accumulate=False):
@@ -1238,3 +1273,15 @@
     L.check(_lib().vd_poison_batch(_p(img_u8), _p(idx), _p(flags_u8), _p(trigger), _p(target), _p(pixel_values), _p(tgt),
                                    _p(image_out), Bn, Cc, H, W, vmin, vmax, int(R_trigger_only), _s()), "vd_poison_batch")
     return pixel_values, tgt
+
+
+def poison_batch_resident(img_u8, pos, index, flags_u8, u, trigger, target, pixel_values, tgt, image_out, is_clean, vmin, vmax):
+    _, H, W, Cc = img_u8.shape
+    Bn = pos.numel()
+    assert img_u8.dtype == torch.uint8 and img_u8.is_contiguous() and pos.dtype == torch.int64 and pos.is_contiguous()
+    assert index.dtype == torch.int64 and flags_u8.dtype == torch.uint8 and index.is_contiguous() and flags_u8.is_contiguous()
+    assert u is None or (u.dtype == torch.float32 and u.numel() == Bn and u.is_contiguous())
+    assert is_clean is None or (is_clean.dtype == torch.bool and is_clean.numel() == Bn and is_clean.is_contiguous())
+    L.check(_lib().vd_poison_batch_resident(_p(img_u8), _p(pos), _p(index), _p(flags_u8), _p(u), _p(trigger), _p(target), _p(pixel_values),
+                                            _p(tgt), _p(image_out), _p(is_clean), Bn, Cc, H, W, vmin, vmax, _s()), "vd_poison_batch_resident")
+    return pixel_values, tgt
diff --git a/villandiffusion_amd/unet.py b/villandiffusion_amd/unet.py
--- a/villandiffusion_amd/unet.py
+++ b/villandiffusion_amd/unet.py
@@ -63,6 +63,8 @@
             return
         key = (net.flat_param._version, ops.WEIGHTS_EPOCH)
         if self.key[bwd] != key:
+            if getattr(net, "_fwd_saves", False) and self.jobs[not bwd] and self.key[not bwd] != key:
+                return self.refresh_both()
             if self.buf is None:
                 self.buf = torch.empty(self.total, device=net.flat_param.device, dtype=torch.int32)
             if bwd not in self.tables:
@@ -76,6 +78,27 @@
             (ops.conv3_pack_weights_f16_multi if self.f16 else ops.conv3_pack_weights_multi)(tab, nj, blk)
             self.key[bwd] = key
 
+    def refresh_both(self):
+        net = self.net
+        key = (net.flat_param._version, ops.WEIGHTS_EPOCH)
+        if not (self.jobs[False] and self.jobs[True] and self.key[False] != key and self.key[True] != key):
+            self.refresh(False)
+            self.refresh(True)
+            return
+        if self.buf is None:
+            self.buf = torch.empty(self.total, device=net.flat_param.device, dtype=torch.int32)
+        if "both" not in self.tables:
+            rows, blk = [], 0
+            for bwd in (False, True):
+                for k, get, M, Cc, T, rs, cs in self.jobs[bwd]:
+                    o, n = self.off[bwd][k]
+                    rows.append([get().data_ptr(), self.buf.data_ptr() + 4 * o, M, Cc, rs, cs, blk, T])
+                    blk += ((M + 127) // 128 * 128 * (Cc // 16) * 2 + 255) // 256
+            self.tables["both"] = (torch.tensor(rows, dtype=torch.int64).to(self.buf.device), len(rows), blk)
+        tab, nj, blk = self.tables["both"]
+        (ops.conv3_pack_weights_f16_multi if self.f16 else ops.conv3_pack_weights_multi)(tab, nj, blk)
+        self.key[False] = self.key[True] = key
+
 
 def _split(net) -> bool:
     return getattr(net, "conv_math", "f32") in ("bf16x3", "f16", "bf16")
@@ -161,7 +184,7 @@
             return h
         return ops.presplit_pack(h)
 
-    def bwd(self, dout, x, dx, bias_ws=None, skip_bias=False, dout_ps=None):
+    def bwd(self, dout, x, dx, bias_ws=None, skip_bias=False, dout_ps=None, dx_add=None):
         net = self.net
         dout_f32 = dout
         gw = net.G[self.prefix + ".weight"].view(self.cout, self.cin * 9)
@@ -192,9 +215,10 @@
             net.colsum_later(ws, net.G[self.prefix + ".bias"], B, self.cout, ld=(ws.stride(0) if ws.dim() == 2 else self.cout))
         if dx is None:
             return None
+        assert dx_add is None or self.mode == B_CONV3_S2
         if self.mode == B_CONV3_S2:
             pk = _bx3_packed_1x1(net, self.prefix + "::s2g", True, self.cin * 9, self.cout, dout.shape[2] * dout.shape[3], dout.shape[0])
-            return ops.conv3x3_s2_dgrad(dout, self.w2d(), dx, pad=self.pad, a_packed=pk)
+            return ops.conv3x3_s2_dgrad(dout, self.w2d(), dx, pad=self.pad, a_packed=pk, add=dx_add)
         pk = _bx3_packed(net, self.prefix, True, self.cin, self.cout, dout.shape[2], dout.shape[3], B_CONV3_T) \
             if self.mode in (B_CONV3, B_CONV3_UP) else None
         wt = net.wt_view(self.prefix, self.cout, self.cin, 9, fresh=pk is None)
@@ -715,6 +739,7 @@
         self.wgrad_ws: Optional[torch.Tensor] = None
         self._cs_pool: Optional[torch.Tensor] = None
         self._cs_tables: Dict[tuple, torch.Tensor] = {}
+        self._rs_tables: Dict[tuple, tuple] = {}
         self._cs_cols_hint = 4 * sum(int(math.prod(sh)) for _, sh, _ in layout if len(sh) == 1) + 4096
         self._cs_off, self._cs_jobs, self._cs_B, self._cs_retired = 0, [], 0, []
         self._d_temb: Dict[int, torch.Tensor] = {}
@@ -831,8 +856,7 @@
             self._packed16 = _PackedConvWeights(self, f16=True)
         for pk in (self._packed, self._packed16):
             if pk is not None:
-                pk.refresh(False)
-                pk.refresh(True)
+                pk.refresh_both()
         self._aux_stream.wait_stream(torch.cuda.current_stream(self._dev))
         return True
 
@@ -891,8 +915,7 @@
             with torch.cuda.stream(self._wg_side):
                 for t, out in self._pk_jobs:
                     ops.presplit_pack(t, out=out)
-                for x, ws, ld in self._rs_jobs:
-                    ops.rowsum(x, ws, ws_ld=ld)
+                self._rs_launch()
                 for cls, jobs in self._wg_jobs.items():
                     if jobs:
                         ops.conv_wgrad_group([j[0] for j in jobs], self._dev)
@@ -909,6 +932,28 @@
             if direct:
                 route.flush(self._dev)
         self._wg_jobs = {}
+
+    def _rs_launch(self):
+        jobs = self._rs_jobs
+        if not jobs:
+            return
+        seg = {}
+        for x, ws, ld in jobs:
+            if ops.rowsum_grouped_enabled() and x.shape[2] * x.shape[3] < ops.ROWSUM_LONG_P:
+                seg.setdefault(x.shape[0], []).append(ops.rowsum_job(x, ws, ld))
+            else:
+                ops.rowsum(x, ws, ws_ld=ld)
+        for Bn, js in seg.items():
+            key = (Bn, tuple(js))
+            ent = self._rs_tables.get(key)
+            if ent is None:
+                if len(self._rs_tables) >= 64:
+                    self._rs_tables = {}
+                host, blocks = ops.rowsum_table(js, Bn)
+                ent = self._rs_tables[key] = (ops.upload_table(host, self._dev), blocks)
+            if ops._CAPTURE_TABLES is not None:
+                ops._CAPTURE_TABLES.append(ent[0])
+            ops.rowsum_segmented(ent[0], len(js), Bn, ent[1])
 
     def _wg_join(self):
         if self._wg_keep:
@@ -1028,6 +1073,7 @@
     def _run_forward(self, x, t, save):
         dev = self._dev
         B, _, S, _ = x.shape
+        self._fwd_saves = bool(save)
         st = SimpleNamespace(saved=[], B=B)
         sv = st.saved
         st.marks = {}
@@ -1226,8 +1272,12 @@
             elif kind == "ds":
                 layer, x = rec[1], rec[2]
                 dx = torch.empty(x.shape, device=dev, dtype=torch.float32)
-                layer.bwd(g, x, dx, bias_ws=g_rs)
-                g, g_rs, g_ps = self._add_skip_grad(dx, x, st, dcats), None, None
+                if ops.s2_dgrad_add_enabled():
+                    layer.bwd(g, x, dx, bias_ws=g_rs, dx_add=self._skip_grad(x, st, dcats))
+                    g, g_rs, g_ps = dx, None, None
+                else:
+                    layer.bwd(g, x, dx, bias_ws=g_rs)
+                    g, g_rs, g_ps = self._add_skip_grad(dx, x, st, dcats), None, None
             elif kind == "conv_in":
                 if want_dx:
                     dx_in = torch.empty(rec[1].shape, device=dev, dtype=torch.float32)
```

Result: no change. 7587 (-0.4%).
